# sloisel/MultiGridBarrier.jl

Measured on AMD Instinct MI355X. Metric: Newton iters/sec + wall-clock to converge, 2D P2 p-Laplace L=9, higher is better.
Workload: dtype f64

## Files before the change

include/mgbhip.h:

```cpp
#ifndef MGBHIP_H
#define MGBHIP_H

#include <stdint.h>

#ifdef __cplusplus
extern "C" {
#endif

#define MGBHIP_OK 0
#define MGBHIP_ERR_INVALID 1
#define MGBHIP_ERR_HIP 2
#define MGBHIP_ERR_NOT_SPD 3
#define MGBHIP_ERR_NONFINITE 4
#define MGBHIP_ERR_CONVERGENCE 5

#define MGBHIP_MAX_PIECES 4
#define MGBHIP_MAX_IDX 10
#define MGBHIP_MAX_LIN 4
#define MGBHIP_MAX_ND 13
#define MGBHIP_MAX_NU 4
#define MGBHIP_MAX_OPS 8

#define MGBHIP_KIND_EP 1
#define MGBHIP_KIND_LINEAR 2
// ... 74 lines not shown
    int64_t newton_iterations;
    int64_t f0_evals, f1_evals, f2_evals, factorizations;
    int32_t cap_steps;
    int64_t* its;
    double* ts;
    double* kappas;
    double* times;
    double* c_dot_Dz;
} mgbhip_core_result;

int mgbhip_create(mgbhip_ctx** ctx, int device_id, void* hip_stream );
int mgbhip_destroy(mgbhip_ctx* ctx);
const char* mgbhip_last_error(void);
const char* mgbhip_version(void);

int mgbhip_problem_create(mgbhip_ctx* ctx, const mgbhip_problem_desc* desc,
                          mgbhip_problem* share, mgbhip_problem** out);
int mgbhip_problem_destroy(mgbhip_problem* prob);
int mgbhip_problem_set_box(mgbhip_problem* prob, double b, double R);
int mgbhip_problem_set_barrier_weights(mgbhip_problem* prob, const double* bw );
int64_t mgbhip_level_size(const mgbhip_problem* prob, int32_t level);

int mgbhip_f0(mgbhip_problem* prob, int32_t level, const double* s, const double* c,
              const double* z0, double* value);
int mgbhip_f1(mgbhip_problem* prob, int32_t level, const double* s, const double* c,
              const double* z0, double* grad );
int mgbhip_f2(mgbhip_problem* prob, int32_t level, const double* s, const double* c,
              const double* z0, double* values );
int mgbhip_hessian_pattern(mgbhip_problem* prob, int32_t level, int64_t* nnz,
                           const int32_t** rowptr, const int32_t** colidx);
int mgbhip_solve(mgbhip_problem* prob, int32_t level, const double* g, double* x);
int mgbhip_set_hessian(mgbhip_problem* prob, int32_t level, const double* values );
int mgbhip_solve_newton(mgbhip_problem* prob, int32_t level, const double* g, double* x, double* lambda2);
typedef int (*mgbhip_allreduce_fn)(void* user, double* buf, int64_t count, int32_t op, int32_t on_device);
int mgbhip_problem_set_sharding(mgbhip_problem* prob, int32_t level, int64_t n_iface,
                                const int32_t* iface_cols, const double* own_mask );
int mgbhip_problem_set_collective(mgbhip_problem* prob, mgbhip_allreduce_fn allreduce, void* user,
                                  int32_t accepts_device_ptr);
int mgbhip_newton_direction(mgbhip_problem* prob, int32_t level, const double* s, const double* c,
                            const double* z0, double* x, double* lambda2, int32_t* condensed);
int mgbhip_node_barrier(mgbhip_problem* prob, const double* z, double* F , double* Dz );
int mgbhip_node_slack(mgbhip_problem* prob, const double* z, double* slack );

int mgbhip_mgb_core(mgbhip_problem* prob, double* z , const double* c ,
                    const mgbhip_options* opt, mgbhip_core_result* res);
int mgbhip_matched_t(mgbhip_problem* prob, const double* z, const double* c, double t_default,
                     double* t_out);
void mgbhip_default_options(mgbhip_options* opt, int64_t n_nodes);

typedef struct mgbhip_vec mgbhip_vec;
int mgbhip_vec_alloc(mgbhip_ctx* ctx, int64_t len, mgbhip_vec** out);
int mgbhip_vec_free(mgbhip_vec* v);
int64_t mgbhip_vec_len(const mgbhip_vec* v);
int mgbhip_vec_upload(mgbhip_vec* v, const double* host, int64_t len);
int mgbhip_vec_download(const mgbhip_vec* v, double* host, int64_t len);
int mgbhip_vec_fill(mgbhip_vec* v, double value);
int mgbhip_vec_copy(mgbhip_vec* dst, const mgbhip_vec* src);
int mgbhip_vec_axpy(double alpha, const mgbhip_vec* x, mgbhip_vec* y);
int mgbhip_vec_scale(double alpha, mgbhip_vec* x);
int mgbhip_vec_dot(const mgbhip_vec* a, const mgbhip_vec* b, double* out);
int mgbhip_vec_norm(const mgbhip_vec* a, double* out);
int mgbhip_vec_isfinite(const mgbhip_vec* a, int32_t* all_finite);
int mgbhip_f0_d(mgbhip_problem* prob, int32_t level, const mgbhip_vec* s, const mgbhip_vec* c,
                const mgbhip_vec* z0, double* value);
int mgbhip_f1_d(mgbhip_problem* prob, int32_t level, const mgbhip_vec* s, const mgbhip_vec* c,
                const mgbhip_vec* z0, mgbhip_vec* grad);
int mgbhip_f2_d(mgbhip_problem* prob, int32_t level, const mgbhip_vec* s, const mgbhip_vec* c,
                const mgbhip_vec* z0);
int mgbhip_solve_d(mgbhip_problem* prob, int32_t level, const mgbhip_vec* g, mgbhip_vec* x);
int mgbhip_prolong_add(mgbhip_problem* prob, int32_t level, const mgbhip_vec* s, mgbhip_vec* z);

int mgbhip_stage_ms(mgbhip_problem* prob, const char* stage, double* total_ms, int64_t* launches);
int mgbhip_reset_stage_timers(mgbhip_problem* prob, int enable);
int mgbhip_solver_stats(mgbhip_problem* prob, int32_t level, double* out8);
int mgbhip_solver_chain(mgbhip_problem* prob, int32_t level, double* out8);
enum { MGBHIP_PROJ_NONE = 0, MGBHIP_PROJ_LOOP = 1, MGBHIP_PROJ_STAGED = 2, MGBHIP_PROJ_MFMA = 3, MGBHIP_PROJ_ACCUMULATE = 4 };
int mgbhip_level_plan(mgbhip_problem* prob, int32_t level, int32_t* out16);
enum { MGBHIP_ELEM_F0 = 0, MGBHIP_ELEM_F1 = 1, MGBHIP_ELEM_F2 = 2, MGBHIP_ELEM_NODE_F = 3, MGBHIP_ELEM_NODE_SLACK = 4, MGBHIP_ELEM_F01 = 5 };
enum { MGBHIP_ELEM_KIND_DENSE = 0, MGBHIP_ELEM_KIND_WIDE = 1, MGBHIP_ELEM_KIND_FAST_DEFAULT = 2, MGBHIP_ELEM_KIND_FAST_RUNTIME = 3,
       MGBHIP_ELEM_KIND_CONDENSE = 4, MGBHIP_ELEM_KIND_GENERIC = 5 };
int mgbhip_elem_plan(mgbhip_problem* prob, int32_t mode, int32_t* out16);
int mgbhip_trial_values(mgbhip_problem* prob, int32_t level, const double* x, const double* dir, double step, const double* c,
                        const double* z0, double* y, double* g, double* xn, int32_t* moved, int32_t* finite, int32_t* path);
enum { MGBHIP_LAUNCH_ROW = 16 };
enum { MGBHIP_ASM_NONE = 0, MGBHIP_ASM_GATHER = 1, MGBHIP_ASM_COLUMNS = 2 };
enum { MGBHIP_B0_NA = 0, MGBHIP_B0_GATHER = 1, MGBHIP_B0_DIAG0 = 2, MGBHIP_B0_STEP0 = 3 };
enum { MGBHIP_BWD_NA = 0, MGBHIP_BWD_K8 = 1, MGBHIP_BWD_K16 = 2, MGBHIP_BWD_GENERAL = 3 };
int64_t mgbhip_solver_launches(mgbhip_problem* prob, int32_t level, int32_t* out, int64_t cap);

#define MGBHIP_INTERP_FEM1D 1
#define MGBHIP_INTERP_QK 2
#define MGBHIP_INTERP_P1 3
#define MGBHIP_INTERP_P2 4
#define MGBHIP_INTERP_SPECTRAL1D 5
#define MGBHIP_INTERP_SPECTRAL2D 6
#define MGBHIP_INTERP_P2C 7
int mgbhip_interpolate(mgbhip_ctx* ctx, int32_t family, int32_t d, int32_t k, int32_t p, int64_t N,
                       const double* x, const double* table, int32_t ncomp, const double* z, int64_t M,
                       const double* pts, double* out, int32_t* elem);
int mgbhip_interpolate_grad(mgbhip_ctx* ctx, int32_t family, int32_t d, int32_t k, int32_t p, int64_t N,
                            const double* x, const double* table, int32_t ncomp, const double* z, int64_t M,
                            const double* pts, double* out ,
                            double* grad , int32_t* elem );

typedef struct mgbhip_locator mgbhip_locator;
int mgbhip_locator_create(mgbhip_ctx* ctx, int32_t family, int32_t d, int32_t k, int32_t p, int64_t N,
                          const double* x, const double* table, int64_t M, const double* pts,
                          mgbhip_locator** out);
int mgbhip_locator_elements(const mgbhip_locator* loc, int32_t* elem );
int mgbhip_locator_evaluate(mgbhip_locator* loc, int32_t ncomp, const double* z ,
                            double* out ,
                            double* grad );
int mgbhip_locator_destroy(mgbhip_locator* loc);

typedef struct mgbhip_closest mgbhip_closest;
int mgbhip_closest_create(mgbhip_ctx* ctx, int32_t d, int32_t e, int32_t k, int64_t N, const double* x,
                          const double* nodes, int64_t M, const double* pts, double max_distance,
                          mgbhip_closest** out);
int mgbhip_closest_fetch(const mgbhip_closest* cp, int32_t* elem , double* xi ,
                         double* foot , double* dist , int32_t* flag );
int mgbhip_closest_evaluate(mgbhip_closest* cp, int32_t ncomp, const double* z ,
                            double* out ,
                            double* grad );
int mgbhip_closest_destroy(mgbhip_closest* cp);

enum { MGBHIP_QUAD_VALUE = 0, MGBHIP_QUAD_LP = 1, MGBHIP_QUAD_W1P = 2, MGBHIP_QUAD_ENERGY = 3 };
typedef struct mgbhip_quadrature mgbhip_quadrature;
int mgbhip_quadrature_create(mgbhip_ctx* ctx, int32_t d, int32_t e, int32_t p, int64_t N, const double* x, int32_t Q,
                             const double* wref, const double* phi, const double* dphi, mgbhip_quadrature** out);
int mgbhip_quadrature_points(mgbhip_quadrature* quad, double* points );
int mgbhip_quadrature_weights(mgbhip_quadrature* quad, double* weights );
int mgbhip_quadrature_integrate(mgbhip_quadrature* quad, int32_t kind, double pexp, int32_t ncol,
                                const double* z , const double* minus ,
                                const double* source ,
                                double* per_element , double* totals );
int mgbhip_quadrature_max(mgbhip_quadrature* quad, int32_t kind, int32_t ncol, const double* z ,
                          const double* minus , double* maxima );
int mgbhip_quadrature_plan(int32_t d, int32_t e, int32_t p, int32_t Q, int64_t N, int32_t* out16);
int mgbhip_quadrature_times(const mgbhip_quadrature* quad, double* ms2);
int mgbhip_quadrature_destroy(mgbhip_quadrature* quad);

typedef struct mgbhip_residual mgbhip_residual;
int mgbhip_residual_create(mgbhip_ctx* ctx, int32_t d, int32_t p, int64_t N, const double* x, int32_t Q, const double* wref,
                           const double* phi, const double* dphi, const double* d2phi, mgbhip_residual** out);
int mgbhip_residual_geometry(mgbhip_residual* res, double* points , double* weights ,
                             double* sizes );
int mgbhip_residual_pointwise(mgbhip_residual* res, double pexp, int32_t ncol, const double* z ,
                              const double* source , int32_t at_points, double* r );
int mgbhip_residual_integrate(mgbhip_residual* res, double pexp, int32_t ncol, const double* z ,
                              const double* source , int32_t at_points,
                              double* per_element , double* totals );
int mgbhip_residual_plan(int32_t d, int32_t p, int32_t Q, int64_t N, int32_t* out16);
int mgbhip_residual_times(const mgbhip_residual* res, double* ms2);
int mgbhip_residual_destroy(mgbhip_residual* res);

enum { MGBHIP_FACE_VALUE = 0, MGBHIP_FACE_FLUX = 1 };
typedef struct mgbhip_faces mgbhip_faces;
int mgbhip_faces_create(mgbhip_ctx* ctx, int32_t d, int32_t p, int64_t N, const double* x, const int32_t* t, int32_t F,
                        int32_t Qf, const double* wf, const double* phi, const double* dphi, const double* tangents,
                        const double* normals, const int32_t* corners, int32_t ncode, const int32_t* perm,
                        mgbhip_faces** out, int64_t* nboundary, int64_t* ninterior);
int mgbhip_faces_topology(const mgbhip_faces* faces, int32_t* boundary, int32_t* interior, int32_t* orientation,
                          int32_t* element_faces);
int mgbhip_faces_geometry(mgbhip_faces* faces, int32_t which, double* points, double* normals, double* measures);
int mgbhip_faces_sizes(const mgbhip_faces* faces, double* sizes );
int mgbhip_faces_integrate(mgbhip_faces* faces, int32_t kind, double pexp, int32_t ncol, const double* z ,
// ... 128 lines not shown
```

multigridbarrier.jl_amd/csrc/api.cpp:

```cpp
#include <chrono>
#include <cmath>
#include <cstring>
#include <algorithm>
#include <limits>
#include <memory>
#include <string>

#include "closest.hpp"
#include "contour.hpp"
#include "faces.hpp"
#include "figure.hpp"
#include "interpolate.hpp"
#include "polyline.hpp"
#include "problem.hpp"
#include "quadrature.hpp"
#include "residual.hpp"
#include "raycast.hpp"
#include "stream.hpp"
#include "surface.hpp"
#include "tubes.hpp"
#include "weld.hpp"

using namespace mgbhip;

mgbhip_problem* problem_create(mgbhip_ctx* ctx, const mgbhip_problem_desc* d, mgbhip_problem* share);
int core_run(mgbhip_problem* P, double* z, const double* c, const mgbhip_options* opt, mgbhip_core_result* res);
int matched_t_run(mgbhip_problem* P, const double* z, const double* c, double t_default, double* t_out);
void trial_values_run(mgbhip_problem* P, int level, double step, double* y, int32_t* moved, int32_t* finite, int32_t* path);

#ifdef MGB_STEP_PROBE
namespace mgbhip { void mf_debug_probe(long long* out64); }
#endif

static thread_local std::string g_last_error;

struct DeviceGuard {
    int prev = -1, dev = -1;
    explicit DeviceGuard(int d) : dev(d) {
        if (dev < 0) return;
        if (hipGetDevice(&prev) != hipSuccess) prev = -1;
        if (prev != dev) MGB_HIP_CHECK(hipSetDevice(dev));
    }
    ~DeviceGuard() {
        if (dev >= 0 && prev >= 0 && prev != dev) (void)hipSetDevice(prev);
    }
};
static int dev_of(const mgbhip_ctx* c) { return c ? c->device : -1; }
template <class H>
static int dev_of(const H* h) { return (h && h->ctx) ? h->ctx->device : -1; }

template <class T>
struct Handle {
    mgbhip_ctx* ctx = nullptr;
    T obj;
};
struct mgbhip_locator : Handle<Locator> {};
struct mgbhip_closest : Handle<Closest> {};
struct mgbhip_quadrature : Handle<Quadrature> {};
struct mgbhip_faces : Handle<Faces> {};
struct mgbhip_residual : Handle<Residual> {};
struct mgbhip_contour : Handle<Contour> {};
struct mgbhip_tessellation : Handle<Tessellation> {};
struct mgbhip_weld : Handle<Weld> {};
struct mgbhip_polyline : Handle<Polyline> {};
struct mgbhip_raycast : Handle<RayCaster> {};
struct mgbhip_surface : Handle<Surface> {};
struct mgbhip_tubes : Handle<Tubes> {};
struct mgbhip_stream : Handle<StreamTracer> {};
struct mgbhip_figure : Handle<Figure> {};

#define MGB_API_BEGIN try {
#define MGB_API_BEGIN_ON(h) try { DeviceGuard _guard(dev_of(h));
#define MGB_API_END                                   \
    }                                                 \
    catch (const InvalidArgument& e) {                \
        g_last_error = e.what();                      \
        return MGBHIP_ERR_INVALID;                    \
    }                                                 \
    catch (const HipError& e) {                       \
        g_last_error = e.what();                      \
        return MGBHIP_ERR_HIP;                        \
    }                                                 \
    catch (const std::exception& e) {                 \
        g_last_error = e.what();                      \
        return MGBHIP_ERR_INVALID;                    \
    }

template <class H, class Build>
static void create_handle(mgbhip_ctx* ctx, H** out, Build build) {
    std::unique_ptr<H> h(new H());
    h->ctx = ctx;
    build(h->obj);
    *out = h.release();
}

template <class H>
static int destroy_handle(H* h) {
    MGB_API_BEGIN_ON(h)
    if (!h) return MGBHIP_OK;
    (void)hipStreamSynchronize(h->ctx->stream);
    delete h;
    return MGBHIP_OK;
    MGB_API_END
}

static void check_window(const std::string& who, double t_min, double t_max) {
    MGB_REQUIRE(std::isfinite(t_min) && t_max > t_min, who + ": t_min must be finite and t_max > t_min");
}

static void check_rays(const std::string& who, int64_t R, int dim, const double* origin, const double* dir) {
    for (int64_t i = 0; i < R * dim; ++i)
// ... 273 lines not shown
        for (size_t i = 0; i < m; ++i) acc += g[i] * x[i];
        *lambda2 = acc;
    }
    if (status != MGBHIP_OK) g_last_error = "Cholesky met a non-positive pivot";
    return status;
    MGB_API_END
}

int mgbhip_problem_set_sharding(mgbhip_problem* P, int32_t level, int64_t n_iface, const int32_t* iface_cols, const double* own_mask) {
    MGB_API_BEGIN_ON(P)
    check_level(P, level);
    mgbhip::Level& L = P->levels[level];
    MGB_REQUIRE(!L.solver.analyzed, "sharding must be set before the first solve of the level");
    MGB_REQUIRE(own_mask != nullptr && n_iface >= 0 && n_iface <= L.m && (n_iface == 0 || iface_cols), "bad sharding arguments");
    L.h_iface.assign(iface_cols, iface_cols + n_iface);
    for (int64_t i = 0; i < n_iface; ++i) {
        MGB_REQUIRE(L.h_iface[i] >= 0 && L.h_iface[i] < L.m, "interface column out of range");
        MGB_REQUIRE(i == 0 || L.h_iface[i] > L.h_iface[i - 1], "interface columns must be strictly increasing");
    }
    L.d_iface.upload(L.h_iface, P->stream());
    L.own.upload(own_mask, (size_t)L.m, P->stream());
    MGB_HIP_CHECK(hipStreamSynchronize(P->stream()));
    L.sharded = true;
    return MGBHIP_OK;
    MGB_API_END
}

int mgbhip_problem_set_collective(mgbhip_problem* P, mgbhip_allreduce_fn fn, void* user, int32_t accepts_device_ptr) {
    MGB_API_BEGIN_ON(P)
    P->coll_fn = fn;
    P->coll_user = user;
    P->coll_device = accepts_device_ptr != 0;
    return MGBHIP_OK;
    MGB_API_END
}

int mgbhip_newton_direction(mgbhip_problem* P, int32_t level, const double* s, const double* c, const double* z0, double* x,
                            double* lambda2, int32_t* condensed) {
    MGB_API_BEGIN_ON(P)
    check_level(P, level);
    MGB_REQUIRE(s && c && z0 && x, "null argument");
    hipStream_t st = P->stream();
    const size_t m = (size_t)P->levels[level].m;
    stage_inputs(P, level, s, c, z0);
    P->eval_f1(level, P->d_x.p, P->d_z0.p, P->d_c.p, P->d_g.p);
    P->eval_f2(level, P->d_x.p, P->d_z0.p, P->d_c.p, false, P->d_g.p);
    if (condensed) *condensed = P->levels[level].H.condensed() ? 1 : 0;
    P->factor(level, P->d_g.p, P->d_nv.p);
    P->trisolve_carried(level, P->d_nv.p);
    const int status = P->levels[level].solver.status(st);
    P->d_nv.download(x, m, st);
    if (lambda2) {
        std::vector<double> g(m);
        P->d_g.download(g.data(), m, st);
        MGB_HIP_CHECK(hipStreamSynchronize(st));
        double acc = 0.0;
        for (size_t i = 0; i < m; ++i) acc += g[i] * x[i];
        *lambda2 = acc;
    }
    MGB_HIP_CHECK(hipStreamSynchronize(st));
    if (status != MGBHIP_OK) g_last_error = "Cholesky met a non-positive pivot";
    return status;
    MGB_API_END
}

int mgbhip_trial_values(mgbhip_problem* P, int32_t level, const double* x, const double* dir, double step, const double* c,
                        const double* z0, double* y, double* g, double* xn, int32_t* moved, int32_t* finite, int32_t* path) {
    MGB_API_BEGIN_ON(P)
    check_level(P, level);
    MGB_REQUIRE(x && dir && c && z0 && y && g && xn && moved && finite && path, "null argument");
    MGB_REQUIRE(!P->sharded(), "trial_values: not for sharded problems");
    hipStream_t st = P->stream();
    const size_t m = (size_t)P->levels[level].m;
    stage_inputs(P, level, x, c, z0);
    P->d_nv.upload(dir, m, st);
    trial_values_run(P, level, step, y, moved, finite, path);
    P->d_gn.download(g, m, st);
    P->d_xn.download(xn, m, st);
    MGB_HIP_CHECK(hipStreamSynchronize(st));
    return MGBHIP_OK;
    MGB_API_END
}


static double* vec_scratch(mgbhip_ctx* c, int64_t len) {
    c->vscratch.ensure((size_t)reduce_scratch_doubles(len));
    c->vscal.ensure(8);
    return c->vscratch.p;
}
static void same_ctx(const mgbhip_vec* a, const mgbhip_vec* b) {
    MGB_REQUIRE(a && b, "null vector");
    MGB_REQUIRE(a->ctx == b->ctx, "vectors belong to different contexts");
}

int mgbhip_vec_alloc(mgbhip_ctx* ctx, int64_t len, mgbhip_vec** out) {
    MGB_API_BEGIN_ON(ctx)
    MGB_REQUIRE(ctx && out && len >= 0, "bad argument");
    std::unique_ptr<mgbhip_vec> v(new mgbhip_vec());
    v->ctx = ctx;
    v->len = len;
    v->buf.alloc((size_t)std::max<int64_t>(len, 1));
    v->buf.zero(ctx->stream);
    *out = v.release();
    return MGBHIP_OK;
    MGB_API_END
}

int mgbhip_vec_free(mgbhip_vec* v) {
    MGB_API_BEGIN_ON(v)
    if (!v) return MGBHIP_OK;
    (void)hipStreamSynchronize(v->ctx->stream);
    delete v;
    return MGBHIP_OK;
    MGB_API_END
}

int64_t mgbhip_vec_len(const mgbhip_vec* v) { return v ? v->len : -1; }

int mgbhip_vec_upload(mgbhip_vec* v, const double* host, int64_t len) {
    MGB_API_BEGIN_ON(v)
    MGB_REQUIRE(v && host && len == v->len, "upload: length mismatch");
    v->buf.upload(host, (size_t)len, v->ctx->stream);
    MGB_HIP_CHECK(hipStreamSynchronize(v->ctx->stream));
    return MGBHIP_OK;
    MGB_API_END
}

int mgbhip_vec_download(const mgbhip_vec* v, double* host, int64_t len) {
    MGB_API_BEGIN_ON(v)
    MGB_REQUIRE(v && host && len == v->len, "download: length mismatch");
    v->buf.download(host, (size_t)len, v->ctx->stream);
    MGB_HIP_CHECK(hipStreamSynchronize(v->ctx->stream));
    return MGBHIP_OK;
    MGB_API_END
}

int mgbhip_vec_fill(mgbhip_vec* v, double value) {
    MGB_API_BEGIN_ON(v)
    MGB_REQUIRE(v, "null vector");
    launch_fill(value, v->buf.p, v->len, v->ctx->stream);
    return MGBHIP_OK;
    MGB_API_END
}

int mgbhip_vec_copy(mgbhip_vec* dst, const mgbhip_vec* src) {
    MGB_API_BEGIN_ON(dst)
    same_ctx(dst, src);
    MGB_REQUIRE(dst->len == src->len, "copy: length mismatch");
    if (dst->len) MGB_HIP_CHECK(hipMemcpyAsync(dst->buf.p, src->buf.p, (size_t)dst->len * sizeof(double),
                                               hipMemcpyDeviceToDevice, dst->ctx->stream));
    return MGBHIP_OK;
    MGB_API_END
}

int mgbhip_vec_axpy(double alpha, const mgbhip_vec* x, mgbhip_vec* y) {
    MGB_API_BEGIN_ON(y)
    same_ctx(x, y);
    MGB_REQUIRE(x->len == y->len, "axpy: length mismatch");
    if (y->len) launch_axpy(alpha, x->buf.p, y->buf.p, y->len, y->ctx->stream);
    return MGBHIP_OK;
    MGB_API_END
}

int mgbhip_vec_scale(double alpha, mgbhip_vec* x) {
    MGB_API_BEGIN_ON(x)
    MGB_REQUIRE(x, "null vector");
// ... 1273 lines not shown
```

multigridbarrier.jl_amd/csrc/common.hpp:

```cpp
#pragma once
#include <hip/hip_runtime.h>

#include <cstdint>
#include <cstdio>
#include <map>
#include <stdexcept>
#include <string>
#include <vector>

#include "host_util.hpp"
#include "readback.hpp"

namespace mgbhip {

struct HipError : std::runtime_error {
    using std::runtime_error::runtime_error;
};

#define MGB_HIP_CHECK(expr)                                                                  \
    do {                                                                                     \
        hipError_t _e = (expr);                                                              \
        if (_e != hipSuccess) {                                                              \
            char _buf[512];                                                                  \
            snprintf(_buf, sizeof(_buf), "%s failed: %s (%s:%d)", #expr, hipGetErrorString(_e), \
                     __FILE__, __LINE__);                                                    \
            throw ::mgbhip::HipError(_buf);                                                  \
        }                                                                                    \
    } while (0)

template <typename T>
struct DevBuf {
    T* p = nullptr;
    size_t n = 0;
    DevBuf() = default;
    DevBuf(const DevBuf&) = delete;
    DevBuf& operator=(const DevBuf&) = delete;
    DevBuf(DevBuf&& o) noexcept : p(o.p), n(o.n) { o.p = nullptr; o.n = 0; }
    DevBuf& operator=(DevBuf&& o) noexcept {
        if (this != &o) { release(); p = o.p; n = o.n; o.p = nullptr; o.n = 0; }
        return *this;
    }
    ~DevBuf() { release(); }
    void release() {
        if (p) (void)hipFree(p);
        p = nullptr;
        n = 0;
    }
    void alloc(size_t count) {
        if (count == n && p) return;
        release();
        if (count) MGB_HIP_CHECK(hipMalloc((void**)&p, count * sizeof(T)));
        n = count;
    }
    void ensure(size_t count) {
        if (count > n) alloc(count);
    }
    void upload(const T* h, size_t count, hipStream_t st) {
        ensure(count);
        if (count) MGB_HIP_CHECK(hipMemcpyAsync(p, h, count * sizeof(T), hipMemcpyHostToDevice, st));
    }
    void upload(const std::vector<T>& h, hipStream_t st) { upload(h.data(), h.size(), st); }
    void download(T* h, size_t count, hipStream_t st) const {
        if (count) MGB_HIP_CHECK(hipMemcpyAsync(h, p, count * sizeof(T), hipMemcpyDeviceToHost, st));
    }
    void zero(hipStream_t st, size_t count = (size_t)-1) {
        if (count == (size_t)-1) count = n;
        if (count) MGB_HIP_CHECK(hipMemsetAsync(p, 0, count * sizeof(T), st));
    }
};

struct PinnedBuf {
    double* d = nullptr;
    double* dev = nullptr;
    PinnedBuf() {
        void* p = nullptr;
        if (hipHostMalloc(&p, RB_SLOTS * sizeof(double), hipHostMallocDefault) != hipSuccess)
            throw HipError("hipHostMalloc failed for the scalar read-back block");
        d = static_cast<double*>(p);
        void* dp = nullptr;
        if (hipHostGetDevicePointer(&dp, p, 0) != hipSuccess || dp == nullptr)
            throw HipError("hipHostGetDevicePointer failed for the scalar read-back block");
        dev = static_cast<double*>(dp);
    }
    ~PinnedBuf() { if (d) (void)hipHostFree(d); }
    PinnedBuf(const PinnedBuf&) = delete;
    PinnedBuf& operator=(const PinnedBuf&) = delete;
};

struct StageTimers {
    struct Rec { double ms = 0; int64_t launches = 0; };
    bool enabled = false;
    hipStream_t stream = nullptr;
    std::map<std::string, Rec> recs;
    struct Pending { std::string name; hipEvent_t a, b; };
    std::vector<Pending> pending;
    std::vector<hipEvent_t> pool;

    hipEvent_t get() {
        if (!pool.empty()) { hipEvent_t e = pool.back(); pool.pop_back(); return e; }
        hipEvent_t e;
        MGB_HIP_CHECK(hipEventCreate(&e));
        return e;
    }
    std::vector<size_t> open;
    void begin(const char* name) {
        if (!enabled) return;
        Pending p{name, get(), get()};
        MGB_HIP_CHECK(hipEventRecord(p.a, stream));
        pending.push_back(p);
        open.push_back(pending.size() - 1);
    }
    void end() {
        if (!enabled || open.empty()) return;
        MGB_HIP_CHECK(hipEventRecord(pending[open.back()].b, stream));
        open.pop_back();
        if (open.empty() && pending.size() > 4096) collect();
    }
    void collect() {
        if (!open.empty()) return;
        for (auto& p : pending) {
            MGB_HIP_CHECK(hipEventSynchronize(p.b));
            float ms = 0;
            MGB_HIP_CHECK(hipEventElapsedTime(&ms, p.a, p.b));
            auto& r = recs[p.name];
            r.ms += ms;
            r.launches += 1;
            pool.push_back(p.a);
            pool.push_back(p.b);
        }
        pending.clear();
    }
    void reset(bool en) {
        collect();
        recs.clear();
        enabled = en;
    }
    ~StageTimers() {
        for (auto& p : pending) { (void)hipEventDestroy(p.a); (void)hipEventDestroy(p.b); }
        for (auto e : pool) (void)hipEventDestroy(e);
    }
};

template <int N>
struct CallEvents {
    hipEvent_t ev[N] = {};
    bool timed = false;
    CallEvents() = default;
    CallEvents(const CallEvents&) = delete;
    CallEvents& operator=(const CallEvents&) = delete;
    ~CallEvents() {
        for (hipEvent_t e : ev)
            if (e) (void)hipEventDestroy(e);
    }
    void mark(int i, hipStream_t st) {
        if (!ev[i]) MGB_HIP_CHECK(hipEventCreate(&ev[i]));
        MGB_HIP_CHECK(hipEventRecord(ev[i], st));
    }
    void begin(hipStream_t st) {
        timed = false;
        mark(0, st);
    }
// ... 17 lines not shown
```

multigridbarrier.jl_amd/csrc/driver.cpp:

```cpp
#include <chrono>
#include <cstdio>
#include <cstdlib>
#include <cmath>
#include <cstring>
#include <functional>
#include <limits>

#include "problem.hpp"

using namespace mgbhip;

namespace {

constexpr double EPS = std::numeric_limits<double>::epsilon();

bool debug_on() {
    static const bool on = env_on("MGBHIP_DEBUG");
    return on;
}
#define DBG(...) do { if (debug_on()) { fprintf(stderr, __VA_ARGS__); } } while (0)

struct Stop {
    double lambda_tol;
    double theta;
    int (*fn)(double, double, double, double, double, double, void*) = nullptr;
    void* user = nullptr;
    bool operator()(double ymin, double ynext, double gmin, double gnorm_next, double ndecmin, double ndec) const {
        if (fn) return fn(ymin, ynext, gmin, gnorm_next, ndecmin, ndec, user) != 0;
        const bool exact = (ynext >= ymin) && (gnorm_next >= theta * gmin);
        if (lambda_tol >= 0) return (ndec < lambda_tol) || exact;
        return exact;
    }
};

struct NewtonResult {
    int k = 0;
    bool converged = false;
    double y = 0;
};

struct VecStats { double sumsq, bad; };

VecStats vec_stats(mgbhip_problem* P, int level, const double* d_v, int64_t len) {
    launch_vec_stats(d_v, len, P->d_scratch.p, P->d_scal.p, RB_SUMSQ, P->stream(), P->own_mask(level));
    const double* r = P->read_scalars(RB_SUMSQ, 2);
    return VecStats{r[0], r[1]};
}

double dev_dot(mgbhip_problem* P, int level, const double* a, const double* b, int64_t len) {
    launch_dot(a, b, len, P->d_scratch.p, P->d_scal.p, RB_GDOTV, P->stream(), P->own_mask(level));
    return *P->read_scalars(RB_GDOTV, 1);
}

struct NewtonCtx {
    mgbhip_problem* P;
    int level;
    const double* d_zJ;
    const double* d_c;
    int64_t m;
    double F0(const double* d_s) { return P->eval_f0(level, d_s, d_zJ, d_c); }
    void F1(const double* d_s, double* d_out, double* d_part) { P->eval_f1(level, d_s, d_zJ, d_c, d_out, P->sharded() ? d_part : nullptr); }
    const double* rhs_of_g() const { return P->sharded() ? P->d_gpart.p : P->d_g.p; }
    void F2(const double* d_s) { P->eval_f2(level, d_s, d_zJ, d_c, false, rhs_of_g()); }
};

bool trial_values(NewtonCtx& C, double& ynext, double& gnorm_next, int32_t* moved = nullptr, const double* step = nullptr,
                  bool* restrict_fused_out = nullptr) {
    mgbhip_problem* P = C.P;
    hipStream_t st = P->stream();
    const bool onfly = step && P->can_fuse_step(C.level);
    if (step) {
        ++P->step_stamp;
        if (!onfly) launch_step(P->d_x.p, P->d_nv.p, *step, P->d_xn.p, C.m, P->d_flag.p, P->step_stamp, st);
        P->touch();
    }
    const bool fused = !P->dense;
    static const bool fuse_restrict = !env_on("MGBHIP_NO_FUSED_RESTRICT");
    TrialRestrict fuse;
    TrialPoint point{};
    if (onfly) {
        point = TrialPoint{P->d_x.p, P->d_nv.p, *step};
        fuse = TrialRestrict{P->d_x.p, P->d_nv.p, *step, P->d_xn.p, P->d_flag.p, P->step_stamp};
    }
    const bool restrict_fused = P->eval_f01_launch(C.level, P->d_xn.p, C.d_zJ, C.d_c, P->d_gn.p, P->sharded() ? P->d_gnpart.p : nullptr, fused,
                                                   onfly ? &point : nullptr, (fused && fuse_restrict) ? &fuse : nullptr);
    if (restrict_fused_out) *restrict_fused_out = restrict_fused;
    if (onfly && !restrict_fused) launch_step(P->d_x.p, P->d_nv.p, *step, P->d_xn.p, C.m, P->d_flag.p, P->step_stamp, st);
    const TrialReadback r = P->finish_trial(C.level, P->d_gn.p, fused, restrict_fused);
    if (moved) *moved = r.moved ? 1 : 0;
    ynext = r.value;
    if (!std::isfinite(ynext)) return false;
    if (r.bad != 0.0 || !std::isfinite(r.sumsq)) return false;
    gnorm_next = std::sqrt(r.sumsq);
    return true;
}

bool linesearch_backtracking(NewtonCtx& C, const mgbhip_options& opt, double y, double inc, double& ynext,
                             double& gnorm_next) {
    double s = 1.0;
    bool have = false;
    while (s > 0.0) {
        double yn, gn;
        int32_t moved = 0;
        if (trial_values(C, yn, gn, &moved, &s)) {
            have = true;
            ynext = yn;
            gnorm_next = gn;
            const bool stalled = (moved == 0);
            if (stalled || yn <= y - opt.ls_c1 * inc * s) return true;
        }
        s *= opt.ls_beta;
    }
    return have;
}

bool linesearch_illinois(NewtonCtx& C, const mgbhip_options& opt, double inc, double& ynext, double& gnorm_next) {
    mgbhip_problem* P = C.P;
    hipStream_t st = P->stream();
    struct Reject {};
    auto phi = [&](double sigma) -> double {
        launch_step(P->d_x.p, P->d_nv.p, sigma, P->d_xn.p, C.m, P->d_flag.p, ++P->step_stamp, st);
        P->touch();
        const double f = C.F0(P->d_xn.p);
        if (!std::isfinite(f)) throw Reject();
        C.F1(P->d_xn.p, P->d_gn.p, P->d_gnpart.p);
        const double v = dev_dot(P, C.level, P->d_gn.p, P->d_nv.p, C.m);
        if (!std::isfinite(v)) throw Reject();
        return v;
    };
    double s = 1.0;
    while (s > 0.0) {
        try {
            double a = 0.0, b = s, fa = inc, fb = phi(s), root = b;
            bool done = false;
            if (fa == 0) { root = a; done = true; }
            else if (fa * fb >= 0) { root = b; done = true; }
            for (int it = 0; it < 10000 && !done; ++it) {
                const double c = (a * fb - b * fa) / (fb - fa);
                const double fc = phi(c);
                if (c <= std::fmin(a, b) || c >= std::fmax(a, b) || fc * fa == 0 || fc * fb == 0) { root = c; done = true; break; }
                if (fb * fc < 0) { a = b; fa = fb; } else { fa /= 2; }
                b = c; fb = fc;
            }
            if (!done) throw Reject();
            launch_step(P->d_x.p, P->d_nv.p, root, P->d_xn.p, C.m, P->d_flag.p, ++P->step_stamp, st);
        P->touch();
            double yn, gn;
            if (!trial_values(C, yn, gn)) throw Reject();
            ynext = yn;
            gnorm_next = gn;
            return true;
        } catch (Reject&) {
        }
        s *= opt.ls_beta;
    }
    return false;
}

NewtonResult newton(NewtonCtx& C, const mgbhip_options& opt, const Stop& stop, int maxit) {
    mgbhip_problem* P = C.P;
    hipStream_t st = P->stream();
    NewtonResult R;
    P->d_x.zero(st, (size_t)C.m);
    P->touch();
    static const bool split_start = env_on("MGBHIP_SPLIT_START");
    double y;
    VecStats gs;
    if (!split_start && !P->dense && !P->sharded() && opt.line_search != 1) {
        P->eval_f01_launch(C.level, P->d_x.p, C.d_zJ, C.d_c, P->d_g.p, nullptr, true);
        const TrialReadback r = P->finish_trial(C.level, P->d_g.p, true, false);
        y = r.value;
        if (!std::isfinite(y)) throw InvalidArgument("newton: initial objective value is not finite");
        gs = VecStats{r.sumsq, r.bad};
    } else {
        y = C.F0(P->d_x.p);
        if (!std::isfinite(y)) throw InvalidArgument("newton: initial objective value is not finite");
        if (P->sharded()) { P->d_gpart.ensure((size_t)C.m); P->d_gnpart.ensure((size_t)C.m); }
        C.F1(P->d_x.p, P->d_g.p, P->d_gpart.p);
        gs = vec_stats(P, C.level, P->d_g.p, C.m);
    }
    double ymin = y;
// ... 76 lines not shown

struct StepResult {
    bool converged;
    std::vector<int64_t> its;
};

StepResult mgb_step(mgbhip_problem* P, const double* d_c, const mgbhip_options& opt, bool finalize_now,
                    bool initial_step) {
    const int L = (int)P->levels.size();
    StepResult out;
    out.its.assign(L, 0);
    hipStream_t st = P->stream();
    const Stop sc{opt.stop_lambda_tol, opt.stop_theta, opt.stopping_criterion, opt.user};
    const Stop fin{-1.0, opt.finalize_theta};
    const size_t zn = (size_t)P->nu * P->n;
    auto eta = [&](int j, int J, const Stop& stop, int maxit) -> bool {
        (void)j;
        const int lev = J - 1;
        static const bool snapshot = env_on("MGBHIP_Z_SNAPSHOT");
        if (snapshot) MGB_HIP_CHECK(hipMemcpyAsync(P->d_z0.p, P->d_z.p, zn * sizeof(double), hipMemcpyDeviceToDevice, st));
        NewtonCtx C{P, lev, snapshot ? P->d_z0.p : P->d_z.p, d_c, P->levels[lev].m};
        NewtonResult r = newton(C, opt, stop, maxit);
        out.its[lev] += r.k;
        if (r.converged) {
            const Level& Lv = P->levels[lev];
            StageScope scp(P->ctx->timers, "prolong");
            launch_csr_matvec(Lv.rows, Lv.Rptr.p, Lv.Rcol.p, Lv.Rval.p, P->d_x.p, P->d_z.p, true, false, st);
        }
        return r.converged;
    };
    std::function<bool(int, int)> dac = [&](int j, int J) -> bool {
        const int mn = (initial_step && J - j == 1) ? opt.maxit : opt.max_newton;
        if (eta(j, J, sc, mn)) return true;
        const int jmid = (j + J) / 2;
        if (jmid == j || jmid == J) return false;
        return dac(j, jmid) && dac(jmid, J);
    };
    bool converged = dac(0, L);
    if (finalize_now) {
        const bool foo = eta(L - 1, L, fin, opt.maxit);
        converged = converged && foo;
    }
    out.converged = converged;
    return out;
}

double c_dot_Dz(mgbhip_problem* P, const double* d_c) {
    hipStream_t st = P->stream();
    ElemParams E = P->elem_params(d_c);
    E.z0 = P->d_z.p;
    E.invn = 0.0;
    E.bw = nullptr;
    launch_elem(E, MODE_F0, st);
    launch_reduce_partials(P->d_partials.p, elem_grid(P->p, P->N), P->d_scal.p, st);
    double v;
    P->d_scal.download(&v, 1, st);
    MGB_HIP_CHECK(hipStreamSynchronize(st));
    if (P->sharded()) P->allreduce_host(&v, 1, 0);
    return v;
}

bool slack_feasible(mgbhip_problem* P, std::vector<double>& hbuf) {
    hipStream_t st = P->stream();
    hbuf.resize((size_t)P->n);
    MGB_HIP_CHECK(hipMemcpyAsync(hbuf.data(), P->d_z.p + (size_t)(P->nu - 1) * P->n, (size_t)P->n * sizeof(double),
                                 hipMemcpyDeviceToHost, st));
    MGB_HIP_CHECK(hipStreamSynchronize(st));
    double mx = -INFINITY;
    for (double v : hbuf) mx = std::fmax(mx, v);
    if (P->sharded()) P->allreduce_host(&mx, 1, 1);
    return mx < 0;
}

}

void trial_values_run(mgbhip_problem* P, int level, double step, double* y, int32_t* moved, int32_t* finite, int32_t* path) {
    NewtonCtx C{P, level, P->d_z0.p, P->d_c.p, P->levels[level].m};
    double yn = 0.0, gn = 0.0;
    const bool onfly = P->can_fuse_step(level);
    bool restrict_fused = false;
    *finite = trial_values(C, yn, gn, moved, &step, &restrict_fused) ? 1 : 0;
    *y = yn;
    *path = (onfly ? 1 : 0) | (restrict_fused ? 2 : 0);
}

int core_run(mgbhip_problem* P, double* z, const double* c, const mgbhip_options* optp, mgbhip_core_result* res) {
    const mgbhip_options opt = *optp;
    hipStream_t st = P->stream();
    const size_t zn = (size_t)P->nu * P->n;
    const size_t cn = (size_t)P->n * P->nD;
    const int L = (int)P->levels.size();
    P->prepare_all();
    P->d_z.upload(z, zn, st);
    P->d_c0.upload(c, cn, st);
    P->cnt = Counters();
    auto tb = std::chrono::steady_clock::now();
    auto now = [&] { return std::chrono::duration<double>(std::chrono::steady_clock::now() - tb).count(); };
    double t = opt.t;
    const double target = 1.0 / opt.tol;
    double kappa = opt.kappa;
    const double kappa0 = kappa;
    int k = 1;
    std::vector<double> hbuf;
    double t_first = INFINITY;
    std::vector<double> zhost;
    auto early = [&](double tt) -> bool {
        if (opt.early_stop_fn) {
            zhost.resize(zn);
            P->d_z.download(zhost.data(), zn, st);
            MGB_HIP_CHECK(hipStreamSynchronize(st));
            if (opt.early_stop_fn(zhost.data(), tt, opt.user) != 0) return true;
        }
        if (opt.early_stop != 1) return false;
        if (!slack_feasible(P, hbuf)) return false;
        t_first = std::fmin(t_first, tt);
        return tt >= 2 * t_first;
    };
    auto record = [&](int kk, const std::vector<int64_t>& its, bool add) {
        if (kk - 1 < res->cap_steps && res->its) {
            for (int l = 0; l < L; ++l) {
                if (add) res->its[(size_t)(kk - 1) * L + l] += its[l];
                else res->its[(size_t)(kk - 1) * L + l] = its[l];
            }
        }
    };
    auto setc = [&](double tt) { launch_scale_copy(P->d_c0.p, tt, P->d_c.p, (int64_t)cn, st); };
    res->failure_code = 0;
    res->L = L;
    if (res->times && res->cap_steps > 0) res->times[0] = now();
    setc(t);
    StepResult S = mgb_step(P, P->d_c.p, opt, opt.finalize && t >= target, true);
    if (!S.converged) {
        res->failure_code = 1;
        res->k = 1;
        res->t_final = t;
        res->t_elapsed = now();
        return MGBHIP_ERR_CONVERGENCE;
    }
    record(1, S.its, false);
    auto diag = [&](int kk) {
        if (kk - 1 < res->cap_steps) {
            if (res->ts) res->ts[kk - 1] = t;
            if (res->kappas) res->kappas[kk - 1] = kappa;
            if (res->c_dot_Dz) res->c_dot_Dz[kk - 1] = c_dot_Dz(P, P->d_c0.p);
        }
    };
    diag(1);
    bool stopped_early = false;
    while (t < target && kappa > 1 && k < opt.maxit) {
        if (early(t)) { stopped_early = true; break; }
        ++k;
        if (k - 1 < res->cap_steps && res->its)
            for (int l = 0; l < L; ++l) res->its[(size_t)(k - 1) * L + l] = 0;
        if (res->times && k - 1 < res->cap_steps) res->times[k - 1] = now();
        while (kappa > 1) {
            const double t1 = kappa * t;
            setc(t1);
            P->d_tmp.ensure(zn);
            MGB_HIP_CHECK(hipMemcpyAsync(P->d_tmp.p, P->d_z.p, zn * sizeof(double), hipMemcpyDeviceToDevice, st));
            S = mgb_step(P, P->d_c.p, opt, opt.finalize && t1 >= target, false);
            record(k, S.its, true);
            if (S.converged) {
                int64_t mx = 0;
                for (int64_t v : S.its) mx = std::max(mx, v);
                if ((double)mx <= opt.max_newton * 0.5) kappa = std::fmin(kappa0, kappa * kappa);
                t = t1;
// ... 74 lines not shown
```

multigridbarrier.jl_amd/csrc/elem_kernels.hpp:

```cpp
#pragma once
#include <mutex>
#include <utility>

#include "dense.hpp"
#include "elem_device.hpp"

namespace mgbhip {

namespace {

template <int NY, int MODE>
__global__ __launch_bounds__(256) void elem_kernel(const ElemParams P, const int lgG) {
    extern __shared__ double sh[];
    const int tid = threadIdx.x;
    const int G = 1 << lgG;
    const int EPB = 256 >> lgG;
    const int el = tid >> lgG;
    const int r = tid & (G - 1);
    const int p = P.p;
    const int pp = p * p;
    const int nu = P.nu;
    const int64_t e = (int64_t)blockIdx.x * EPB + el;
    const bool active = (e < P.N) && (r < p);
    const int64_t n = P.n;
    const int64_t node = e * p + r;

    double* zl = sh;
    double* opL = zl + elem_lds_z(256, nu);
    double* YL = opL + elem_lds_ops(P.nstage, EPB, pp);

    {
        const int64_t e0 = (int64_t)blockIdx.x * EPB;
        int64_t lim = (P.N - e0) * pp;
        if (lim > (int64_t)EPB * pp) lim = (int64_t)EPB * pp;
        for (int o = 0; o < P.nstage; ++o) {
            const double* src = P.stage_ptr[o] + e0 * pp;
            double* dst = opL + (size_t)o * EPB * pp;
            for (int i = tid; i < lim; i += 256) dst[i] = src[i];
        }
    }
    if (active) stage_z(P, zl, el, nu, G, r, n, node);
    __syncthreads();

    auto OP = [&](int k, int rr, int cc) -> double {
        const int so = P.D_stage[k];
        if (so >= 0) return opL[((size_t)so * EPB + el) * pp + cc * p + rr];
        return P.ops[P.D_op[k]][e * pp + cc * p + rr];
    };

    double y[NY];
#pragma unroll
    for (int k = 0; k < NY; ++k) {
        double v = 0.0;
        if (active) {
            const int a = P.D_state[k];
            if (P.D_stage[k] == -1) {
                v = zl[(el * nu + a) * G + r];
            } else {
                for (int cc = 0; cc < p; ++cc) v += OP(k, r, cc) * zl[(el * nu + a) * G + cc];
            }
        }
        y[k] = v;
    }

    double F = 0.0;
    double g[NY];
    double H[NY * NY];
    (void)g;
    (void)H;

    if (MODE == MODE_F0 || MODE == MODE_NODE_F) {
        if (active) cone_eval<NY, 0>(P.cone, node, n, y, F, g, H);
        if (MODE == MODE_NODE_F) {
            if (active) {
                P.out_F[node] = F;
                if (P.out_Dz != nullptr) {
#pragma unroll
                    for (int k = 0; k < NY; ++k) P.out_Dz[node + n * k] = y[k];
                }
            }
            return;
        }
        double val = 0.0;
        if (active) {
            const double bar = barrier_f0(P, node, F);
            double lin = 0.0;
#pragma unroll
            for (int k = 0; k < NY; ++k) lin += P.c[node + n * k] * y[k];
            val = bar + P.w[node] * lin;
        }
        __syncthreads();
        const double tot = block_sum_256(val, sh);
        if (tid == 0) P.out_partial[blockIdx.x] = tot;
        return;
    }
// ... 52 lines not shown
            for (int k = 0; k < NY; ++k) {
                double sc = P.bw ? ((bwv == 0.0) ? 0.0 : bwv * g[k]) : P.invn * g[k];
                YL[(el * NY + k) * G + r] = sc + wv * P.c[node + n * k];
            }
        }
        __syncthreads();
        if (active) {
            const int i = r;
            for (int a = 0; a < nu; ++a) {
                double acc = 0.0;
#pragma unroll
                for (int k = 0; k < NY; ++k) {
                    if (P.D_state[k] != a) continue;
                    const double* Yk = YL + (el * NY + k) * G;
                    if (P.D_stage[k] == -1) {
                        acc += Yk[i];
                    } else {
                        for (int rr = 0; rr < p; ++rr) acc += OP(k, rr, i) * Yk[rr];
                    }
                }
                P.out_ret[(int64_t)a * n + node] = acc;
            }
        }
        return;
    }
    if (MODE == MODE_F2) {
        constexpr int NT = NY * (NY + 1) / 2;
        if (active) {
            cone_eval<NY, 2>(P.cone, node, n, y, F, g, H);
            const double bwv = P.bw ? P.bw[node] : 0.0;
#pragma unroll
            for (int k = 0; k < NY; ++k)
#pragma unroll
                for (int k2 = k; k2 < NY; ++k2) {
                    const double h = H[k * NY + k2];
                    const double sc = P.bw ? ((bwv == 0.0) ? 0.0 : bwv * h) : P.invn * h;
                    YL[((size_t)el * NT + tri_index(k, k2, NY)) * G + r] = sc;
                }
        }
        __syncthreads();
        if (active) {
            const int j = r;
            const int NB = nu * (nu + 1) / 2;
            for (int a = 0; a < nu; ++a)
                for (int b = a; b < nu; ++b) {
                    const int blk = a * nu - (a * (a - 1)) / 2 + (b - a);
                    const bool dblk = (P.diag_mask >> blk) & 1;
                    double* out = P.out_hel + P.blk_off[blk] + (dblk ? (e * p + j) - j : (e * p + j) * (int64_t)p);
                    for (int i = dblk ? j : 0; i < (dblk ? j + 1 : p); ++i) {
                        double val = 0.0;
#pragma unroll
                        for (int k = 0; k < NY; ++k) {
                            if (P.D_state[k] != a) continue;
                            const bool idk = P.D_stage[k] == -1;
#pragma unroll
                            for (int k2 = 0; k2 < NY; ++k2) {
                                if (P.D_state[k2] != b) continue;
                                const bool idk2 = P.D_stage[k2] == -1;
                                const int t = (k <= k2) ? tri_index(k, k2, NY) : tri_index(k2, k, NY);
                                const double* Yt = YL + ((size_t)el * NT + t) * G;
                                if (idk && idk2) {
                                    val += (i == j) ? Yt[i] : 0.0;
                                } else if (idk) {
                                    val += Yt[i] * OP(k2, i, j);
                                } else if (idk2) {
                                    val += OP(k, j, i) * Yt[j];
                                } else {
                                    double acc = 0.0;
                                    for (int rr = 0; rr < p; ++rr) acc += OP(k, rr, i) * Yt[rr] * OP(k2, rr, j);
                                    val += acc;
                                }
                            }
                        }
                        out[i] = val;
                    }
                }
        }
        return;
    }
}

template <int MODE>
__global__ __launch_bounds__(256) void elem_wide_kernel(const ElemParams P, const int lgG) {
    extern __shared__ double sh[];
    const int tid = threadIdx.x;
    const int NT_ = blockDim.x;
    const int G = 1 << lgG;
    const int EPB = NT_ >> lgG;
    const int el = tid >> lgG;
    const int r = tid & (G - 1);
    const int p = P.p;
    const int pp = p * p;
    const int nu = P.nu;
    const int nD = P.nD;
    const int64_t e = (int64_t)blockIdx.x * EPB + el;
    const bool active = (e < P.N) && (r < p);
    const int64_t n = P.n;
    const int64_t node = e * p + r;

    double* zl = sh;
    double* opL = zl + elem_lds_z((size_t)NT_, nu);
    double* YL = opL + elem_lds_ops(P.nstage, EPB, pp);
    {
        const int64_t e0 = (int64_t)blockIdx.x * EPB;
        int64_t lim = (P.N - e0) * pp;
        if (lim > (int64_t)EPB * pp) lim = (int64_t)EPB * pp;
        for (int o = 0; o < P.nstage; ++o) {
            const double* src = P.stage_ptr[o] + e0 * pp;
            double* dst = opL + (size_t)o * EPB * pp;
            for (int i = tid; i < lim; i += NT_) dst[i] = src[i];
        }
    }
    if (active) stage_z(P, zl, el, nu, G, r, n, node);
    __syncthreads();

    auto OP = [&](int k, int rr, int cc) -> double {
        const int so = P.D_stage[k];
        if (so >= 0) return opL[((size_t)so * EPB + el) * pp + cc * p + rr];
        return P.ops[P.D_op[k]][e * pp + cc * p + rr];
    };

    double y[WIDE_NY];
#pragma unroll
    for (int k = 0; k < WIDE_NY; ++k) {
        double v = 0.0;
        if (active && k < nD) {
            const int a = P.D_state[k];
            if (P.D_stage[k] == -1) {
                v = zl[(el * nu + a) * G + r];
            } else {
                for (int cc = 0; cc < p; ++cc) v += OP(k, r, cc) * zl[(el * nu + a) * G + cc];
            }
        }
        y[k] = v;
    }
    double F = 0.0;
    double g[WIDE_NY];

    if (MODE == MODE_F0 || MODE == MODE_NODE_F) {
        if (active) cone_eval_wide<0>(P.cone, node, n, nD, y, F, g, nullptr, 0);
        if (MODE == MODE_NODE_F) {
            if (active) {
                P.out_F[node] = F;
                if (P.out_Dz != nullptr)
                    for (int k = 0; k < nD; ++k) P.out_Dz[node + n * k] = y[k];
            }
            return;
        }
        double val = 0.0;
        if (active) {
            const double bar = barrier_f0(P, node, F);
            double lin = 0.0;
#pragma unroll
            for (int k = 0; k < WIDE_NY; ++k) lin += (k < nD) ? P.c[node + n * k] * y[k] : 0.0;
            val = bar + P.w[node] * lin;
        }
        __syncthreads();
        const double tot = block_sum_256(val, sh);
        if (tid == 0) P.out_partial[blockIdx.x] = tot;
        return;
    }
    if (MODE == MODE_NODE_SLACK) {
        if (active) P.out_F[node] = cone_slack<WIDE_NY, WIDE_W>(P.cone, node, n, y);
        return;
    }
    if (MODE == MODE_F1 || MODE == MODE_F01) {
// ... 308 lines not shown
            }
#pragma unroll
            for (int q = 0; q < P; ++q) bj -= Xbeta[q] * t[q];
            if (j == PB) {
                bj -= Pm.leaf_g[ld.interior];
#pragma unroll
                for (int q = 0; q < P; ++q) corner -= Xbeta[q] * Xbeta[q] * Xinv[q];
#pragma unroll
                for (int i = 0; i < P; ++i) Xc[i] = up[i];
                Xs[0] = bj;
                Xs[1] = up[PB];
            }
        }
        __builtin_amdgcn_fence(__ATOMIC_RELEASE, "wavefront");
        __builtin_amdgcn_wave_barrier();
        __builtin_amdgcn_fence(__ATOMIC_ACQUIRE, "wavefront");
        {
            const int m = (int)(ld.packed & 15u);
            const bool pk = Pm.leaf_packed != 0;
            int pos[P];
#pragma unroll
            for (int i = 0; i < P; ++i) pos[i] = (int)((ld.packed >> (4 + 4 * i)) & 15u);
            double d7 = 1.0, bb = 0.0, inv7 = 1.0, f = 0.0, xc[P];
#pragma unroll
            for (int i = 0; i < P; ++i) xc[i] = 0.0;
            if (active) {
                d7 = Xs[1];
                bb = Xs[0];
                inv7 = 1.0 / d7;
#pragma unroll
                for (int i = 0; i < P; ++i) xc[i] = Xc[i];
                f = (j < PB) ? xc[j] * inv7 : 0.0;
                bad = bad || (j == PB && ((d7 == 0.0) || !isfinite(d7)));
            }
            double* Fg = Pm.leaf_arena + ld.F_off;
            double* S = Fg;
            if (pk) {
                __syncthreads();
                S = sh + (size_t)el * 120;
            }
            auto at = [&](int rr, int cc) -> int { return pk ? cc * m - (cc * (cc - 1)) / 2 + (rr - cc) : rr + cc * m; };
            if (active) {
                S[at(j, j)] = ssj;
#pragma unroll
                for (int rr = 0; rr < P; ++rr)
                    if (rr > j) S[at(rr, j)] = 0.0;
                S[at(P, j)] = usc[PB] * inv;
#pragma unroll
                for (int i = 0; i < PB; ++i)
                    if (pos[i] != 15) S[at(pos[i], j)] = usc[i] * inv;
                S[at(m - 1, j)] = beta * inv;
                if (j == PB) {
                    S[at(P, P)] = d7;
#pragma unroll
                    for (int i = 0; i < PB; ++i)
                        if (pos[i] != 15) S[at(pos[i], P)] = xc[i] * inv7;
                    S[at(m - 1, P)] = bb * inv7;
                    S[at(m - 1, m - 1)] = corner - bb * bb * inv7;
                } else if (pos[j] != 15) {
#pragma unroll
                    for (int i = 0; i < PB; ++i)
                        if (pos[i] != 15 && pos[i] >= pos[j]) S[at(pos[i], pos[j])] = up[i] - xc[i] * f;
                    S[at(m - 1, pos[j])] = bj - bb * f;
                }
            }
            if (pk) {
                __builtin_amdgcn_fence(__ATOMIC_RELEASE, "wavefront");
                __builtin_amdgcn_wave_barrier();
                __builtin_amdgcn_fence(__ATOMIC_ACQUIRE, "wavefront");
                if (e < Pm.N) {
                    const LeafDesc l2 = Pm.leaf_desc[e];
                    const int mm = (int)(l2.packed & 15u);
                    double* dstF = Pm.leaf_arena + l2.F_off;
                    for (int t = r; t < mm * (mm + 1) / 2; t += G) dstF[t] = S[t];
                }
            }
        }
        if (bad) atomicOr(Pm.leaf_status, 1);
    }
}

template <int NY, int P, class Sig>
__global__ __launch_bounds__(256) void elem_f01_fast(const ElemParams Pm) {
    constexpr int G = elem_group(P);
    constexpr int EPB = 256 / G;
    constexpr int PP = P * P;
    extern __shared__ double sh[];
    const int tid = threadIdx.x;
    const int el = tid / G;
    const int r = tid % G;
    const int nu = Sig::rt ? Pm.nu : 2;
    auto DST = [&](int k) -> int { return Sig::rt ? Pm.D_state[k] : Sig::state(k); };
    auto DSG = [&](int k) -> int { return Sig::rt ? Pm.D_stage[k] : Sig::stage(k); };
    const int64_t e0 = (int64_t)blockIdx.x * EPB;
    const int64_t e = e0 + el;
    const bool active = (e < Pm.N) && (r < P);
    const int64_t n = Pm.n;
    const int64_t node = e * P + r;

    double* zl = sh;
    double* opL = zl + elem_lds_z(256, nu);
    double* YL = opL + elem_lds_ops(Pm.nstage, EPB, PP);
    {
        int64_t lim = (Pm.N - e0) * PP;
        if (lim > (int64_t)EPB * PP) lim = (int64_t)EPB * PP;
        constexpr int NIT = (EPB * PP + 255) / 256;
        for (int o = 0; o < Pm.nstage; ++o) {
            const double* src = Pm.stage_ptr[o] + e0 * PP;
            double* dst = opL + (size_t)o * EPB * PP;
            copy_unrolled<NIT>(src, dst, lim, tid);
        }
    }
    double ck[NY];
    double wv = 0.0, bwv = 0.0;
    if (active) {
        for (int a = 0; a < nu; ++a) zl[(el * nu + a) * G + r] = z_at(Pm, (int64_t)a * n + node);
#pragma unroll
        for (int k = 0; k < NY; ++k) ck[k] = Pm.c[node + n * k];
        wv = Pm.w[node];
        bwv = Pm.bw ? Pm.bw[node] : 0.0;
    }
    __syncthreads();
    const double* opE = opL + (size_t)el * PP;
    auto OP = [&](int k, int rr, int cc) -> double { return opE[(size_t)DSG(k) * EPB * PP + cc * P + rr]; };
    double y[NY];
#pragma unroll
    for (int k = 0; k < NY; ++k) {
        double v = 0.0;
        if (active) {
            const double* za = zl + (el * nu + DST(k)) * G;
            if (DSG(k) < 0) v = za[r];
            else {
#pragma unroll
                for (int cc = 0; cc < P; ++cc) v += OP(k, r, cc) * za[cc];
            }
        }
        y[k] = v;
    }
    double val = 0.0;
    if (active) {
        double F0v, F, g[NY], H[NY * NY];
        cone_eval<NY, 0>(Pm.cone, node, n, y, F0v, g, H);
        cone_eval<NY, 1>(Pm.cone, node, n, y, F, g, H);
        const double bar = Pm.bw ? ((bwv == 0.0) ? 0.0 : bwv * F0v) : Pm.invn * F0v;
        double lin = 0.0;
#pragma unroll
        for (int k = 0; k < NY; ++k) {
            lin += ck[k] * y[k];
            const double sc = Pm.bw ? ((bwv == 0.0) ? 0.0 : bwv * g[k]) : Pm.invn * g[k];
            YL[(el * NY + k) * G + r] = sc + wv * ck[k];
        }
        val = bar + wv * lin;
    }
    __syncthreads();
    if (active) {
        const int i = r;
        for (int a = 0; a < nu; ++a) {
            double acc = 0.0;
#pragma unroll
            for (int k = 0; k < NY; ++k) {
                if (DST(k) != a) continue;
                const double* Yk = YL + (el * NY + k) * G;
                if (DSG(k) < 0) {
                    acc += Yk[i];
                } else {
#pragma unroll
// ... 124 lines not shown
```

multigridbarrier.jl_amd/csrc/kernels.hpp:

```cpp
#pragma once
#include "common.hpp"
#include "cone.hpp"
#include "elem_layout.hpp"
#include "panel_layout.hpp"

namespace mgbhip {

struct LeafDesc {
    int64_t F_off;
    int32_t interior;
    uint32_t packed;
};

struct ElemParams {
    int32_t p, nu, nD, nstage;
    int32_t ymask;
    int64_t N, n;
    const double* ops[MGBHIP_MAX_OPS];
    const double* stage_ptr[MGBHIP_MAX_OPS];
    int32_t D_state[MGBHIP_MAX_ND];
    int32_t D_op[MGBHIP_MAX_ND];
    int32_t D_stage[MGBHIP_MAX_ND];
    const double* w;
    const double* c;
    const double* z0;
    const double* bw;
    double invn;
    ConeDev cone;
    double* out_partial;
    double* out_ret;
    double* out_hel;
    double* out_F;
    double* out_Dz;
    int32_t diag_mask;
    int64_t blk_off[MGBHIP_MAX_NU * (MGBHIP_MAX_NU + 1) / 2];
    double* dn_Dz;
    double* dn_Y;
    const LeafDesc* leaf_desc;
    double* leaf_arena;
    const double* leaf_g;
    int64_t leaf_slack0;
    int32_t* leaf_status;
    int32_t leaf_packed;
    const int32_t* zsel;
    const double* zs;
    double* zout;
    const double* zx;
    double zalpha;
    int32_t wide;
};
static_assert(sizeof(ElemParams) <= 4096 - 64, "ElemParams must stay well inside the kernel argument limit");

bool launch_elem_f2_condense(const ElemParams& P, hipStream_t st);

int64_t elem_grid(int p, int64_t N);
inline size_t elem_lds_bytes(const ElemParams& P, int mode) {
    return elem_lds_bytes(elem_threads(P.wide != 0, mode), P.p, P.nu, P.nD, P.nstage, mode);
}
inline bool elem_default_signature(const ElemParams& P) {
    const int NY = P.nD;
    if (P.nu != 2 || P.ymask != (((1 << NY) - 1) & ~1)) return false;
    for (int k = 0; k < NY; ++k) {
        if (P.D_state[k] != (k == NY - 1 ? 1 : 0)) return false;
        if (P.D_stage[k] != ((k == 0 || k == NY - 1) ? -1 : k - 1)) return false;
    }
    return true;
}
inline int elem_unstaged_rows(const ElemParams& P) {
    int cnt = 0;
    for (int k = 0; k < P.nD; ++k) cnt += P.D_stage[k] == -2;
    return cnt;
}
inline ElemPlan elem_plan_of(const ElemParams& P, int mode, bool condensing) {
    return elem_decide(P.p, P.nu, P.nD, P.nstage, P.wide != 0, P.p > 64, elem_unstaged_rows(P) == 0, elem_default_signature(P), mode,
                       condensing, P.N);
}
void launch_elem(const ElemParams& P, int mode, hipStream_t st);

void launch_reduce_partials(const double* partials, int64_t count, double* out, hipStream_t st);
void launch_vec_stats(const double* v, int64_t n, double* scratch, double* block, int32_t slot, hipStream_t st,
                      const double* mask = nullptr);
void launch_dot(const double* a, const double* b, int64_t n, double* scratch, double* block, int32_t slot, hipStream_t st,
                const double* mask = nullptr);
void launch_restrict_trial(int64_t rows, const int32_t* ptr, const int32_t* col, const double* val, const double* ret, double* g,
                            double* scratch, const double* x, const double* nn, double s, double* xn, int32_t* moved, int32_t stamp,
                            hipStream_t st);
void launch_publish(const double* src, int n, double* host_block, int host_lo, double seq, hipStream_t st);
void launch_dir_finish(const double* v, const double* g, int64_t n, double* scratch, double* scal, int32_t* status2, double* host,
                       hipStream_t st, const double* mask = nullptr, double seq = 0.0);
void launch_trial_finish(const double* g, int64_t n, double* scratch, const double* f0_partials, int64_t f0_count, double* scal,
                         int32_t* moved, double* host, hipStream_t st, const double* mask = nullptr, double seq = 0.0,
                         bool partials_ready = false);
void launch_index_gather(const double* v, const int32_t* idx, int64_t cnt, double* out, hipStream_t st);
void launch_index_scatter(const double* in, const int32_t* idx, int64_t cnt, double* v, hipStream_t st);
int64_t reduce_scratch_doubles(int64_t n);

void launch_csr_matvec(int64_t rows, const int32_t* ptr, const int32_t* col, const double* val,
                       const double* x, double* y, bool add, bool long_rows, hipStream_t st);
int csr_chunks(int64_t max_row_len);
void launch_csr_matvec_chunked(int64_t rows, const int32_t* ptr, const int32_t* col, const double* val,
                               const double* x, double* y, double* scratch, int nchunk, hipStream_t st);
void launch_prolong(int64_t rows, const int32_t* ptr, const int32_t* col, const double* val, const double* s,
                    const double* z0, double* zfull, hipStream_t st);
void launch_step(const double* x, const double* n, double s, double* xn, int64_t len, int32_t* moved, int32_t stamp,
                 hipStream_t st);
void launch_scale_copy(const double* src, double alpha, double* dst, int64_t len, hipStream_t st);
void launch_border_tail(const double* g, double* tail, int64_t m, hipStream_t st, double* x_one = nullptr);
void launch_axpy(double alpha, const double* x, double* y, int64_t len, hipStream_t st);
void launch_fill(double value, double* y, int64_t len, hipStream_t st);

void launch_gather_shared(int64_t nshared, const int32_t* sh_q, const int32_t* cptr, const int32_t* cidx, const double* slab,
                          double* out, hipStream_t st);
void launch_gather_assemble(int64_t nnz, const int32_t* cptr, const int32_t* cidx, const double* slab,
                            double* Hval, bool long_lists, hipStream_t st, int32_t chunk = 0, int32_t nchunk = 0,
                            double* part = nullptr, const int32_t* qmap = nullptr, int64_t nq = 0);

struct PanelParams {
    int32_t p, nu;
    int64_t N;
    const int32_t* ecol_ptr;
    const double* panels;
    const int32_t* eoff;
    const double* hel;
    double* slab;
    int32_t cmax;
    int32_t upper_only;
    const int32_t* spos;
};
bool launch_panel_project_mfma(const PanelParams& P, hipStream_t st);
void launch_invert_lists(const int32_t* cidx, int64_t total, int32_t* spos, hipStream_t st);
void launch_panel_project(const PanelParams& P, hipStream_t st);
void launch_panel_accumulate(const PanelParams& P, const int32_t* ecols, int32_t m, int32_t nstream, int32_t nsplit,
                             int32_t chunk, int32_t ctmax, double* partial, double* H, hipStream_t st);
void launch_panel_project_staged(const PanelParams& P, int32_t ctmax, hipStream_t st);

}
```

multigridbarrier.jl_amd/csrc/problem.cpp:

```cpp
#include "problem.hpp"
#include "assembly_plan.hpp"
#include "plan_device.hpp"
#include "dense.hpp"

#include <algorithm>
#include <cmath>
#include <cstdio>
#include <atomic>
#include <exception>
#include <cstdlib>
#include <string>
#include <thread>
#include <cstring>
#include <numeric>

using namespace mgbhip;



static void upload_csr(const mgbhip_csr& R, Level& L, hipStream_t st) {
    MGB_REQUIRE(R.rows >= 0 && R.cols >= 0 && R.rowptr && (R.rowptr[R.rows] == 0 || (R.colidx && R.values)),
                "bad prolongation CSR");
    MGB_REQUIRE(R.rows < INT32_MAX && R.cols < INT32_MAX, "prolongation too large for 32-bit indices");
    L.rows = R.rows;
// ... 365 lines not shown
        if (L.acc) dense_pattern(m, L.hHptr, L.hHcol);
        else host_pattern(S, C, L.hHptr, L.hHcol);
        L.nnz = (int64_t)L.hHcol.size();
        L.Hptr.upload(L.hHptr, st);
        L.Hcol.upload(L.hHcol, st);
        if (!L.acc) {
            const HostLists lists = host_lists(S, C, L.hHptr, L.hHcol);
            L.long_lists = lists.long_lists;
            L.list_total = lists.total;
            L.cptr.upload(lists.cptr, st);
            L.cidx.upload(lists.cidx.data(), lists.cidx.size(), st);
            if (lists.cidx.empty()) L.cidx.alloc(1);
            MGB_HIP_CHECK(hipStreamSynchronize(st));
        }
    }
    L.Hval.alloc((size_t)(L.nnz + L.m + 1));
    if (!L.acc && L.long_lists && L.nnz > 0) {
        std::vector<int32_t> hc((size_t)L.nnz + 1);
        L.cptr.download(hc.data(), hc.size(), st);
        MGB_HIP_CHECK(hipStreamSynchronize(st));
        const GatherChunks G = decide_gather_chunks(hc.data(), L.nnz);
        if (G.gather_nchunk > 0) {
            L.gather_chunk = G.gather_chunk;
            L.gather_nchunk = G.gather_nchunk;
            L.gather_part.alloc(2 * (size_t)L.nnz * (size_t)L.gather_nchunk);
        }
    }
    if (!selection && !L.acc && L.nnz > 0) {
        static const bool row_major = env_on("MGBHIP_UPPER_ROW_MAJOR");
        const std::vector<int32_t> up = upper_positions(L.hHptr, L.hHcol, m, row_major);
        L.nup = (int64_t)up.size();
        L.upq.upload(up, st);
        MGB_HIP_CHECK(hipStreamSynchronize(st));
    }
    if (!selection) {
        const std::vector<double> panels = element_panels(S, C);
        L.panels.upload(panels.data(), panels.size(), st);
        if (panels.empty()) L.panels.alloc(1);
        L.slab.alloc((size_t)std::max<int64_t>(L.slab_doubles, 1));
        static const bool no_sorted = env_on("MGBHIP_NO_SORTED_SLAB");
        if (!L.acc && L.nnz > 0 && L.slab_doubles > 0 && !no_sorted) {
            if (L.list_total == L.slab_doubles) {
                L.spos.alloc((size_t)L.slab_doubles);
                launch_invert_lists(L.cidx.p, L.slab_doubles, L.spos.p, st);
                L.sorted_slab = true;
            }
        }
        if (L.acc) L.acc_copies.alloc((size_t)L.acc_waves * (size_t)A.tri);
        MGB_HIP_CHECK(hipStreamSynchronize(st));
    }
    MGB_HIP_CHECK(hipStreamSynchronize(st));
    L.planned = true;
}


ElemParams mgbhip_problem::elem_params(const double* d_cc) const {
    ElemParams E;
    std::memset(&E, 0, sizeof(E));
    E.p = p; E.nu = nu; E.nD = nD; E.nstage = nstage; E.N = N; E.n = n;
    E.wide = wide ? 1 : 0;
    E.ymask = 0;
    for (int k = 0; k < cone.npieces; ++k)
        for (int c = 0; c < cone.pc[k].ni; ++c) E.ymask |= 1 << cone.pc[k].idx[c];
    if (cone.feasibility)
        for (int k = cone.NC - 1; k < nD; ++k) E.ymask |= 1 << k;
    for (size_t o = 0; o < store->ops.size() && o < MGBHIP_MAX_OPS; ++o) E.ops[o] = store->ops[o].p;
    for (int o = 0; o < nstage; ++o) E.stage_ptr[o] = stage_ptr[o];
    for (int k = 0; k < MGBHIP_MAX_ND; ++k) { E.D_state[k] = D_state[k]; E.D_op[k] = D_op[k]; E.D_stage[k] = D_stage[k]; }
    E.w = store->w.p;
    E.c = d_cc;
    E.bw = has_bw ? bw.p : nullptr;
    E.invn = 1.0 / (double)n;
    E.cone = cone;
    E.out_partial = d_partials.p;
    E.out_ret = d_ret.p;
    E.out_hel = d_hel.p;
    E.out_F = d_nodeF.p;
    E.out_Dz = nullptr;
    E.dn_Dz = d_dnDz.p;
    E.dn_Y = d_dnY.p;
    return E;
}

bool mgbhip_problem::bind_point(ElemParams& E, int level, const double* d_s, const double* d_zz, const TrialPoint* trial) {
    const Level& L = levels[level];
    const PointKey here{zstamp, level, d_s, d_zz};
    MGB_REQUIRE(!trial || (L.R_unit && !dense && !(zf == here)), "a trial point is given only after touch(), on a selection level");
    E.z0 = d_zz;
    if (d_s == nullptr) return false;
    if (zf == here) {
    } else if (L.R_unit && !dense) {
        E.zsel = L.Rsel.p;
        E.zs = d_s;
        if (trial) { E.zs = trial->x; E.zx = trial->dir; E.zalpha = trial->alpha; }
        E.zout = d_zfull.p;
        return true;
    } else if (L.R_long) {
        MGB_HIP_CHECK(hipMemcpyAsync(d_zfull.p, d_zz, sizeof(double) * (size_t)L.rows, hipMemcpyDeviceToDevice, stream()));
        launch_csr_matvec(L.rows, L.Rptr.p, L.Rcol.p, L.Rval.p, d_s, d_zfull.p, true, true, stream());
    } else {
        launch_prolong(L.rows, L.Rptr.p, L.Rcol.p, L.Rval.p, d_s, d_zz, d_zfull.p, stream());
    }
    zf = here;
    E.z0 = d_zfull.p;
    return false;
}

void mgbhip_problem::launch_elem_at(ElemParams& E, int mode, int level, const double* d_s, const double* d_zz, const TrialPoint* trial) {
    const bool writes_zfull = bind_point(E, level, d_s, d_zz, trial);
    launch_elem(E, mode, stream());
    if (writes_zfull) zf = PointKey{zstamp, level, d_s, d_zz};
}

const char* mgbhip_problem::stage_name(Stage s, int level) const {
    static const char* const names[][2] = {{"f0", "f0_coarse"}, {"f1", "f1_coarse"}, {"f01", "f01_coarse"}, {"f2", "f2_coarse"},
                                           {"assemble", "assemble_coarse"}};
    return names[s][level + 1 == (int)levels.size() ? 0 : 1];
}

void mgbhip_problem::eval_f0_launch(int level, const double* d_s, const double* d_zz, const double* d_cc) {
    hipStream_t st = stream();
    StageScope sc(ctx->timers, stage_name(STAGE_F0, level));
    ElemParams E = elem_params(d_cc);
    launch_elem_at(E, MODE_F0, level, d_s, d_zz);
    launch_reduce_partials(d_partials.p, elem_grid(p, N), d_scal.p, st);
    cnt.f0++;
}

double mgbhip_problem::eval_f0(int level, const double* d_s, const double* d_zz, const double* d_cc) {
    eval_f0_launch(level, d_s, d_zz, d_cc);
    return *read_scalars(RB_VALUE, 1);
}

void mgbhip_problem::allreduce_host(double* h, int64_t count, int op) {
    MGB_REQUIRE(coll_fn != nullptr, "no collective installed");
    if (coll_fn(coll_user, h, count, op, 0) != 0) throw mgbhip::InvalidArgument("the caller's allreduce failed");
}

void mgbhip_problem::allreduce_device(double* d, int64_t count, int op) {
    MGB_REQUIRE(coll_fn != nullptr, "no collective installed");
    hipStream_t st = stream();
    if (coll_device) {
        MGB_HIP_CHECK(hipStreamSynchronize(st));
        if (coll_fn(coll_user, d, count, op, 1) != 0) throw mgbhip::InvalidArgument("the caller's allreduce failed");
        return;
    }
    coll_host.resize((size_t)count);
    MGB_HIP_CHECK(hipMemcpyAsync(coll_host.data(), d, sizeof(double) * (size_t)count, hipMemcpyDeviceToHost, st));
    MGB_HIP_CHECK(hipStreamSynchronize(st));
    allreduce_host(coll_host.data(), count, op);
    MGB_HIP_CHECK(hipMemcpyAsync(d, coll_host.data(), sizeof(double) * (size_t)count, hipMemcpyHostToDevice, st));
    MGB_HIP_CHECK(hipStreamSynchronize(st));
}

void mgbhip_problem::reduce_interface(int level, double* d_g, double* d_part) {
    Level& L = levels[level];
    if (!L.sharded) return;
    hipStream_t st = stream();
    if (d_part) MGB_HIP_CHECK(hipMemcpyAsync(d_part, d_g, sizeof(double) * (size_t)L.m, hipMemcpyDeviceToDevice, st));
    const int64_t ni = (int64_t)L.h_iface.size();
    if (ni == 0) return;
    L.iface_buf.ensure((size_t)ni);
    launch_index_gather(d_g, L.d_iface.p, ni, L.iface_buf.p, st);
    allreduce_device(L.iface_buf.p, ni, 0);
    launch_index_scatter(L.iface_buf.p, L.d_iface.p, ni, d_g, st);
}

bool mgbhip_problem::restrict_ret(int level, double* d_gout, const TrialRestrict* fuse) {
    hipStream_t st = stream();
    const Level& L = levels[level];
    StageScope sc(ctx->timers, "restrict");
    if (fuse && L.T_chunks == 0 && !L.T_long && !sharded()) {
        launch_restrict_trial(L.m, L.Tptr.p, L.Tcol.p, L.Tval.p, d_ret.p, d_gout, d_scratch.p, fuse->x, fuse->n, fuse->s,
                              fuse->xn, fuse->moved, fuse->stamp, st);
        return true;
    }
    if (L.T_chunks > 0)
        launch_csr_matvec_chunked(L.m, L.Tptr.p, L.Tcol.p, L.Tval.p, d_ret.p, d_gout, d_tchunk.p, L.T_chunks, st);
    else
        launch_csr_matvec(L.m, L.Tptr.p, L.Tcol.p, L.Tval.p, d_ret.p, d_gout, false, L.T_long, st);
    return false;
}

void mgbhip_problem::eval_f1(int level, const double* d_s, const double* d_zz, const double* d_cc, double* d_gout, double* d_part) {
    {
        StageScope sc(ctx->timers, stage_name(STAGE_F1, level));
        ElemParams E = elem_params(d_cc);
        launch_elem_at(E, MODE_F1, level, d_s, d_zz);
    }
    restrict_ret(level, d_gout);
    if (levels[level].sharded) reduce_interface(level, d_gout, d_part);
    cnt.f1++;
}

bool mgbhip_problem::eval_f01_launch(int level, const double* d_s, const double* d_zz, const double* d_cc, double* d_gout,
                                     double* d_part, bool defer_f0_sum, const TrialPoint* trial, const TrialRestrict* fuse) {
    MGB_REQUIRE(!trial || can_fuse_step(level), "a trial point is given only on a level whose element kernel forms it on the fly");
    if (dense) {
        eval_f0_launch(level, d_s, d_zz, d_cc);
        eval_f1(level, d_s, d_zz, d_cc, d_gout, d_part);
        return false;
    }
    hipStream_t st = stream();
    {
        StageScope sc(ctx->timers, stage_name(STAGE_F01, level));
        ElemParams E = elem_params(d_cc);
        launch_elem_at(E, MODE_F01, level, d_s, d_zz, trial);
        if (!defer_f0_sum) launch_reduce_partials(d_partials.p, elem_grid(p, N), d_scal.p, st);
    }
    const bool fused = restrict_ret(level, d_gout, fuse);
    if (levels[level].sharded) reduce_interface(level, d_gout, d_part);
    cnt.f0++;
    cnt.f1++;
    return fused;
}

bool mgbhip_problem::try_enable_condensed(int level) {
    Level& L = levels[level];
    static const bool off = env_on("MGBHIP_NO_CONDENSE");
    if (off || dense || !L.selection || !L.direct || nu != 2 || p != 7 || L.hRptr.empty()) return false;
    if (!L.solver.analyzed || !L.solver.has_direct_map()) return false;
    const int64_t slack0 = L.m - n;
    if (slack0 < 0 || L.rows != 2 * n) return false;
    std::vector<int32_t> ucol((size_t)n, -1);
    for (int64_t node = 0; node < n; ++node) {
        const int32_t b = L.hRptr[node], e = L.hRptr[node + 1];
        if (e - b > 1) return false;
        if (e - b == 1) ucol[(size_t)node] = L.hRcol[b];
        const int64_t rs = n + node;
        if (L.hRptr[rs + 1] - L.hRptr[rs] != 1 || (int64_t)L.hRcol[L.hRptr[rs]] != slack0 + node) return false;
    }
    const bool ok = L.solver.enable_condensed(N, p, ucol.data(), slack0, L.nnz, hel_cap + L.nshared, stream());
    if (debug_level() >= 2)
        fprintf(stderr, "[mgbhip] level %d: condensed leaves %s\n", level, ok ? "enabled" : "not applicable");
    return ok;
}

void mgbhip_problem::eval_f2(int level, const double* d_s, const double* d_zz, const double* d_cc, bool materialize,
                             const double* rhs) {
    ensure_plan(level);
    hipStream_t st = stream();
    Level& L = levels[level];
    int E_ymask = 0;
    if (L.condense && !materialize && rhs != nullptr && L.selection && L.direct && !dense) {
        StageScope sc(ctx->timers, stage_name(STAGE_F2, level));
        ElemParams E = elem_params(d_cc);
        const bool writes_zfull = bind_point(E, level, d_s, d_zz);
        E.leaf_desc = L.solver.leaf_desc();
        E.leaf_arena = L.solver.arena();
        E.leaf_g = rhs;
        E.leaf_slack0 = L.m - n;
        E.leaf_status = L.solver.leaf_status();
        E.leaf_packed = L.solver.leaves_packed() ? 1 : 0;
        if (!L.solver.leaf_flag_zero()) MGB_HIP_CHECK(hipMemsetAsync(E.leaf_status, 0, sizeof(int32_t), st));
        L.solver.leaf_flag_used();
        if (launch_elem_f2_condense(E, st)) {
            if (writes_zfull) zf = PointKey{zstamp, level, d_s, d_zz};
            L.H.written_condensed(hel_owner, level, rhs);
            cnt.f2++;
            return;
        }
    }
    L.proj_kernel = MGBHIP_PROJ_NONE;
    {
        StageScope sc(ctx->timers, stage_name(STAGE_F2, level));
        ElemParams E = elem_params(d_cc);
        E_ymask = E.ymask;
        E.diag_mask = (L.selection && !dense) ? diag_mask_sel : 0;
        hel_layout(nu, N, p, E.diag_mask, E.blk_off);
        launch_elem_at(E, MODE_F2, level, d_s, d_zz);
    }
    {
        StageScope sc(ctx->timers, stage_name(STAGE_ASSEMBLE, level));
        if (dense) {
            int klo = nD, khi = -1;
            for (int k = 0; k < nD; ++k)
                if ((E_ymask >> k) & 1) { klo = std::min(klo, k); khi = std::max(khi, k); }
            const int64_t ld = (int64_t)nD * n;
            if (khi < klo) {
                MGB_HIP_CHECK(hipMemsetAsync(L.Hval.p, 0, sizeof(double) * (size_t)L.nnz, st));
            } else {
                launch_dense_weight(nD, klo, khi, n, L.m, ld, L.denseDR.p, d_dnY.p, L.denseW.p, st);
                launch_dense_gemm_tn((int)L.m, (int)L.m, (int)((khi - klo + 1) * n), L.denseDR.p + (int64_t)klo * n, ld,
                                     nullptr, L.denseW.p + (int64_t)klo * n, ld, L.Hval.p, L.m, false, true, st);
            }
        } else if (L.selection && L.direct && !materialize) {
            launch_gather_shared(L.nshared, L.sh_q.p, L.cptr.p, L.cidx.p, d_hel.p, d_hel.p + hel_cap, st);
        } else if (L.selection) {
            launch_gather_assemble(L.nnz, L.cptr.p, L.cidx.p, d_hel.p, L.Hval.p, L.long_lists, st, L.gather_chunk, L.gather_nchunk, L.gather_part.p);
        } else {
            PanelParams PP;
            PP.p = p; PP.nu = nu; PP.N = N;
            PP.ecol_ptr = L.ecol_ptr.p; PP.panels = L.panels.p; PP.eoff = L.eoff.p;
            PP.hel = d_hel.p; PP.slab = L.slab.p; PP.cmax = L.cmax; PP.spos = nullptr;
            static const bool full_h = env_on("MGBHIP_FULL_COARSE_H");
            const bool upper = !materialize && rhs != nullptr && L.nup > 0 && !L.acc && !full_h;
            PP.upper_only = upper ? 1 : 0;
            if (L.acc) {
                L.proj_kernel = MGBHIP_PROJ_ACCUMULATE;
                launch_panel_accumulate(PP, L.ecols.p, (int32_t)L.m, L.acc_waves, L.acc_split, L.acc_chunk, L.acc_ctmax,
                                        L.acc_copies.p, L.Hval.p, st);
            } else {
                PP.spos = L.sorted_slab ? L.spos.p : nullptr;
                if (launch_panel_project_mfma(PP, st)) {
                    L.proj_kernel = MGBHIP_PROJ_MFMA;
                } else if (panel_accumulate_lds(p, nu, L.acc_ctmax) <= 40 * 1024) {
                    L.proj_kernel = MGBHIP_PROJ_STAGED;
                    launch_panel_project_staged(PP, L.acc_ctmax, st);
                } else {
                    L.proj_kernel = MGBHIP_PROJ_LOOP;
                    launch_panel_project(PP, st);
                }
                launch_gather_assemble(L.nnz, L.cptr.p, L.sorted_slab ? nullptr : L.cidx.p, L.slab.p, L.Hval.p, L.long_lists, st, L.gather_chunk,
                                       L.gather_nchunk, L.gather_part.p, upper ? L.upq.p : nullptr, upper ? L.nup : 0);
            }
        }
    }
    if (L.selection && L.direct && !materialize && !dense) L.H.written_to_slab(hel_owner, level);
    else L.H.written_to_csr(hel_owner);
    cnt.f2++;
}

void mgbhip_problem::wait_results(double seq) {
    static const bool poll = !env_on("MGBHIP_NO_POLL");
    hipStream_t st = stream();
    if (poll && seq != 0.0) {
        volatile const double* stamp = pin.d + RB_STAMP;
        const Stopwatch sw;
        for (int spins = 0;; ++spins) {
            if (__atomic_load_n(reinterpret_cast<const volatile uint64_t*>(stamp), __ATOMIC_ACQUIRE) ==
                *reinterpret_cast<const uint64_t*>(&seq))
                return;
            if ((spins & 1023) == 1023 && sw.seconds() > 1e-3)
                break;
        }
    }
    MGB_HIP_CHECK(hipStreamSynchronize(st));
}

const double* mgbhip_problem::read_scalars(int lo, int n) {
    const double seq = next_seq();
    launch_publish(d_scal.p + lo, n, pin.dev, lo, seq, stream());
    wait_results(seq);
    if (sharded()) allreduce_host(pin.d + lo, n, 0);
    return pin.d + lo;
}

TrialReadback mgbhip_problem::finish_trial(int level, const double* d_grad, bool f0_partials, bool partials_ready) {
    const double seq = next_seq();
    launch_trial_finish(d_grad, levels[level].m, d_scratch.p, f0_partials ? d_partials.p : nullptr, elem_grid(p, N), d_scal.p,
                        d_flag.p, pin.dev, stream(), own_mask(level), seq, partials_ready);
    wait_results(seq);
    TrialReadback r = decode_trial(pin.d, step_stamp);
    if (sharded()) {
        double s[RB_SHARD];
        pack_trial(r, s);
        allreduce_host(s, RB_SHARD, 0);
        r = unpack_trial(s);
    }
    return r;
}

DirReadback mgbhip_problem::finish_direction(int level, bool leaf_before, int* status) {
    MfSolver& solver = levels[level].solver;
    const double seq = next_seq();
    launch_dir_finish(d_nv.p, d_g.p, levels[level].m, d_scratch.p, d_scal.p, solver.status_flags_rw(), pin.dev, stream(),
                      own_mask(level), seq);
    solver.flags_cleared();
    wait_results(seq);
    DirReadback r = decode_direction(pin.d);
    const int32_t flags2[2] = {r.pivot ? 1 : 0, (leaf_before || r.leaf) ? 1 : 0};
    *status = MfSolver::status_from(flags2, solver.factored_condensed);
    if (sharded()) {
        double s[RB_SHARD];
        pack_direction(r, *status != MGBHIP_OK, s);
        allreduce_host(s, RB_SHARD, 0);
        *status = unpack_direction(s, r) ? MGBHIP_ERR_NOT_SPD : MGBHIP_OK;
    }
    return r;
}

bool mgbhip_problem::can_fuse_step(int level) const {
    static const bool off = env_on("MGBHIP_NO_FUSED_STEP");
    return !off && !dense && !sharded() && levels[level].R_unit;
}

void mgbhip_problem::ensure_analysis(int level) {
    Level& L = levels[level];
    if (L.solver.analyzed) return;
    hipStream_t st = stream();
    const Stopwatch sw;
    std::vector<double> cen;
    if (!hx.empty() && xdim > 0 && !L.hRptr.empty()) {
        cen.assign((size_t)L.m * xdim, 0.0);
        std::vector<double> wsum((size_t)L.m, 0.0);
        for (int64_t r = 0; r < L.rows; ++r) {
            const int64_t node = r % n;
            for (int32_t q = L.hRptr[r]; q < L.hRptr[r + 1]; ++q) {
                const double a = std::fabs(L.hRval[q]);
                const int32_t j = L.hRcol[q];
                wsum[j] += a;
                for (int d = 0; d < xdim; ++d) cen[(size_t)j * xdim + d] += a * hx[(size_t)d * n + node];
            }
        }
        for (int64_t j = 0; j < L.m; ++j)
            for (int d = 0; d < xdim; ++d) cen[(size_t)j * xdim + d] = wsum[j] > 0 ? cen[(size_t)j * xdim + d] / wsum[j] : 0.0;
    }
    const bool leaves = L.selection && L.direct && !dense && nu == 2 && p == 7;
    if (L.sharded) {
        mgbhip_problem* self = this;
        L.solver.iface_reduce = [self](double* d, int64_t cnt2) { self->allreduce_device(d, cnt2, 0); };
    }
    L.solver.analyze(L.m, L.hHptr.data(), L.hHcol.data(), st, cen.empty() ? nullptr : cen.data(), xdim, leaves,
                     L.sharded ? L.h_iface.data() : nullptr, L.sharded ? (int64_t)L.h_iface.size() : 0);
    if (debug_level() >= 2)
        fprintf(stderr, "[mgbhip] symbolic analysis level %d (m=%lld, nnz=%lld): %.2f s\n", level, (long long)L.m,
                (long long)L.nnz, sw.seconds());
}

void mgbhip_problem::prepare_all() {
    if (prepared) return;
    prepared = true;
    static const bool off = env_on("MGBHIP_LAZY_PLANS");
    if (off || dense || sharded() || levels.size() < 2) return;
    const int Ln = (int)levels.size();
    const Stopwatch prep_sw;
    std::vector<std::exception_ptr> errors((size_t)Ln);
    std::atomic<int> next{Ln - 1};
    auto worker = [&] {
        (void)hipSetDevice(ctx->device);
        for (int l = next.fetch_sub(1); l >= 0; l = next.fetch_sub(1)) {
            try {
                Level& L = levels[l];
                if (L.sharded) continue;
                ensure_plan(l);
                if (L.m < 1) continue;
// ... 97 lines not shown
```

multigridbarrier.jl_amd/csrc/problem.hpp:

```cpp
#pragma once
#include <mutex>
#include <memory>
#include <string>
#include <vector>

#include "../../include/mgbhip.h"
#include "common.hpp"
#include "hessian_state.hpp"
#include "kernels.hpp"
#include "mf_solver.hpp"

struct mgbhip_ctx {
    int device = 0;
    hipStream_t stream = nullptr;
    bool own_stream = false;
    mgbhip::StageTimers timers;
    mgbhip::DevBuf<double> vscratch, vscal;
};

struct mgbhip_vec {
    mgbhip_ctx* ctx = nullptr;
    mgbhip::DevBuf<double> buf;
    int64_t len = 0;
};

namespace mgbhip {

struct OpStore {
    std::vector<DevBuf<double>> ops;
    std::vector<bool> identity;
    DevBuf<double> w;
};

struct Level {
    int64_t rows = 0, m = 0;
    std::vector<int32_t> hRptr, hRcol;
    std::vector<double> hRval;
    DevBuf<int32_t> Rptr, Rcol, Tptr, Tcol;
    DevBuf<double> Rval, Tval;
    bool T_long = false, R_long = false;
    int32_t max_row = 0, max_col = 0;
    bool R_unit = false;
    DevBuf<int32_t> Rsel;
    int32_t T_chunks = 0;
    bool planned = false;
    bool selection = false;
    bool acc = false;
    int32_t acc_waves = 0, acc_ctmax = 0;
    int32_t acc_split = 1, acc_chunk = 0;
    DevBuf<double> acc_copies;
    std::vector<int32_t> hHptr, hHcol;
    DevBuf<int32_t> Hptr, Hcol, cptr, cidx, ecol_ptr, ecols, eoff;
    DevBuf<int32_t> spos;
    bool sorted_slab = false;
    DevBuf<double> Hval, panels, slab;
    int64_t slab_doubles = 0;
    int32_t cmax = 1;
    bool long_lists = false;
    int64_t list_total = 0;
    int32_t proj_kernel = 0;
    int32_t gather_chunk = 0, gather_nchunk = 0;
    DevBuf<double> gather_part;
    DevBuf<int32_t> upq;
    int64_t nup = 0;
    int64_t nnz = 0;
    DevBuf<double> denseDR, denseW;
    MfSolver solver;
    HessianState H;
    bool direct = false;
    int64_t nshared = 0;
    DevBuf<int32_t> sh_q;
    std::vector<int32_t> h_vmap;
    bool sharded = false;
    std::vector<int32_t> h_iface;
    DevBuf<int32_t> d_iface;
    DevBuf<double> own, iface_buf;
    bool condense_tried = false, condense = false;
};

struct TrialPoint { const double* x; const double* dir; double alpha; };

struct TrialRestrict { const double* x = nullptr; const double* n = nullptr; double s = 0.0;
                       double* xn = nullptr; int32_t* moved = nullptr; int32_t stamp = 0; };

struct Counters {
    int64_t f0 = 0, f1 = 0, f2 = 0, factor = 0, newton = 0;
    double solve_seconds = 0;
};

}

struct mgbhip_problem {
    mgbhip_ctx* ctx = nullptr;
    int32_t p = 0, nu = 0, nD = 0;
    int64_t N = 0, n = 0;
    int32_t diag_mask_sel = 0;
    bool dense = false;
    bool wide = false;
    std::shared_ptr<mgbhip::OpStore> store;
    int32_t D_state[MGBHIP_MAX_ND], D_op[MGBHIP_MAX_ND], D_stage[MGBHIP_MAX_ND];
    int32_t nstage = 0;
    const double* stage_ptr[MGBHIP_MAX_OPS];
    mgbhip::ConeDev cone;
    std::vector<mgbhip::DevBuf<double>> cone_grids;
    mgbhip::DevBuf<double> bw;
    bool has_bw = false;
    std::vector<mgbhip::Level> levels;
    std::vector<double> hx;
    int32_t xdim = 0;
    mgbhip::DevBuf<double> d_z, d_z0, d_zfull, d_c, d_ret, d_hel, d_partials, d_scal, d_scratch, d_nodeF, d_nodeDz, d_dnDz, d_dnY, d_tchunk;
    mgbhip::DevBuf<double> d_x, d_g, d_nv, d_xn, d_gn, d_tmp, d_c0;
    mgbhip::DevBuf<int32_t> d_flag;
    int32_t step_stamp = 0;
    mgbhip::PinnedBuf pin;
    mgbhip::Counters cnt;
    int64_t zstamp = 0;
    struct PointKey {
        int64_t stamp = -1; int level = -1; const double* s = nullptr; const double* z = nullptr;
        bool operator==(const PointKey& o) const { return stamp == o.stamp && level == o.level && s == o.s && z == o.z; }
    } zf;
    void touch() { ++zstamp; }
    mgbhip_allreduce_fn coll_fn = nullptr;
    void* coll_user = nullptr;
    bool coll_device = false;
    bool sharded() const { return coll_fn != nullptr; }
    std::vector<double> coll_host;
    void allreduce_host(double* h, int64_t count, int op);
    void allreduce_device(double* d, int64_t count, int op);
    void reduce_interface(int level, double* d_g, double* d_part);
    const double* own_mask(int level) const { return levels[level].sharded ? levels[level].own.p : nullptr; }
    mgbhip::DevBuf<double> d_gpart, d_gnpart;

    mgbhip::ElemParams elem_params(const double* d_cc) const;
    bool bind_point(mgbhip::ElemParams& E, int level, const double* d_s, const double* d_zz, const mgbhip::TrialPoint* trial = nullptr);
    void launch_elem_at(mgbhip::ElemParams& E, int mode, int level, const double* d_s, const double* d_zz,
                        const mgbhip::TrialPoint* trial = nullptr);
    enum Stage { STAGE_F0, STAGE_F1, STAGE_F01, STAGE_F2, STAGE_ASSEMBLE };
    const char* stage_name(Stage s, int level) const;
    bool restrict_ret(int level, double* d_gout, const mgbhip::TrialRestrict* fuse = nullptr);
    hipStream_t stream() const { return ctx->stream; }
    void ensure_plan(int level);
    void ensure_analysis(int level);
    void ensure_direct(int level);
    void prepare_all();
    double next_seq() { return ++result_seq; }
    void wait_results(double seq);
    bool can_fuse_step(int level) const;
    const double* read_scalars(int lo, int n);
    mgbhip::TrialReadback finish_trial(int level, const double* d_grad, bool f0_partials, bool partials_ready);
    mgbhip::DirReadback finish_direction(int level, bool leaf_before, int* status);
    double result_seq = 0.0;
    std::mutex shared_mutex;
    bool prepared = false;
    void ensure_plan_dense(int level);
    double eval_f0(int level, const double* d_s, const double* d_zz, const double* d_cc);
    void eval_f0_launch(int level, const double* d_s, const double* d_zz, const double* d_cc);
    void eval_f1(int level, const double* d_s, const double* d_zz, const double* d_cc, double* d_gout, double* d_part = nullptr);
    bool eval_f01_launch(int level, const double* d_s, const double* d_zz, const double* d_cc, double* d_gout, double* d_part = nullptr,
                         bool defer_f0_sum = false, const mgbhip::TrialPoint* trial = nullptr, const mgbhip::TrialRestrict* fuse = nullptr);
    void eval_f2(int level, const double* d_s, const double* d_zz, const double* d_cc, bool materialize = true,
                 const double* rhs = nullptr);
    bool try_enable_condensed(int level);
    int64_t hel_cap = 0;
    mgbhip::SlabOwner hel_owner;
    void factor(int level, const double* rhs = nullptr, double* carried_out = nullptr);
    void trisolve(int level, const double* d_g, double* d_xout);
    void trisolve_carried(int level, double* d_xout_np1);
    bool lu_fallback(int level, const double* d_g, double* d_xout);
    mgbhip::DevBuf<double> d_lu;
    mgbhip::DevBuf<int32_t> d_lustat;
    int64_t lu_fallbacks = 0;
};
```

multigridbarrier.jl_amd/csrc/readback.hpp:

```cpp
#pragma once
#include <cstdint>

namespace mgbhip {

enum : int32_t {
    RB_VALUE = 0,
    RB_AUX = 1,
    RB_SUMSQ = 2,
    RB_BAD = 3,
    RB_MOVED = 4,
    RB_GDOTV = 4,
    RB_PIVOT = 5,
    RB_LEAF = 6,
    RB_STAMP = 15,
    RB_SLOTS = 16
};
constexpr int32_t RB_TRIAL_LO = RB_VALUE, RB_TRIAL_N = RB_MOVED + 1 - RB_TRIAL_LO;
constexpr int32_t RB_DIR_LO = RB_SUMSQ, RB_DIR_N = RB_LEAF + 1 - RB_DIR_LO;
static_assert(RB_TRIAL_LO + RB_TRIAL_N <= RB_STAMP && RB_DIR_LO + RB_DIR_N <= RB_STAMP, "a read-back layout reaches the stamp");
static_assert(RB_AUX < RB_STAMP && RB_STAMP < RB_SLOTS, "the stamp is the block's last slot");

struct FinishJob { const double* src; int64_t count; int32_t out; };
struct FinishParams {
    FinishJob job[4];
    int32_t njobs;
    double* out;
    int32_t* ints;
    int32_t nints, ints_out, reset;
    double* host;
    int32_t host_lo, host_n;
    double seq;
};

inline FinishParams finish_plain(const double* partials, int64_t count, int32_t njobs, double* block, int32_t slot) {
    FinishParams F{};
    for (int32_t k = 0; k < njobs; ++k) F.job[k] = FinishJob{partials + k * count, count, slot + k};
    F.njobs = njobs;
    F.out = block;
    return F;
}

inline FinishParams finish_trial_params(const double* f0_partials, int64_t f0_count, const double* partials, int64_t count,
                                        double* block, int32_t* moved, double* host, double seq) {
    FinishParams F{};
    int32_t nj = 0;
    if (f0_partials) F.job[nj++] = FinishJob{f0_partials, f0_count, RB_VALUE};
    F.job[nj++] = FinishJob{partials, count, RB_SUMSQ};
    F.job[nj++] = FinishJob{partials + count, count, RB_BAD};
    F.njobs = nj;
    F.out = block;
    F.ints = moved; F.nints = 1; F.ints_out = RB_MOVED; F.reset = 0;
    F.host = host; F.host_lo = RB_TRIAL_LO; F.host_n = RB_TRIAL_N;
    F.seq = seq;
    return F;
}

inline FinishParams finish_direction_params(const double* partials, int64_t count, double* block, int32_t* status2, double* host,
                                            double seq) {
    FinishParams F{};
    F.job[0] = FinishJob{partials, count, RB_SUMSQ};
    F.job[1] = FinishJob{partials + count, count, RB_BAD};
    F.job[2] = FinishJob{partials + 2 * count, count, RB_GDOTV};
    F.njobs = 3;
    F.out = block;
    F.ints = status2; F.nints = 2; F.ints_out = RB_PIVOT; F.reset = 1;
    F.host = host; F.host_lo = RB_DIR_LO; F.host_n = RB_DIR_N;
    F.seq = seq;
    return F;
}
static_assert(RB_LEAF == RB_PIVOT + 1, "the two status flags are one pair of ints");

struct TrialReadback { double value, sumsq, bad; bool moved; };
struct DirReadback { double sumsq, bad, gdotv; bool pivot, leaf; };

inline TrialReadback decode_trial(const double* block, int32_t stamp) {
    return TrialReadback{block[RB_VALUE], block[RB_SUMSQ], block[RB_BAD], block[RB_MOVED] == (double)stamp};
}
inline DirReadback decode_direction(const double* block) {
    return DirReadback{block[RB_SUMSQ], block[RB_BAD], block[RB_GDOTV], block[RB_PIVOT] != 0.0, block[RB_LEAF] != 0.0};
}

constexpr int RB_SHARD = 4;
inline void pack_trial(const TrialReadback& r, double* s) {
    s[0] = r.value; s[1] = r.moved ? 1.0 : 0.0; s[2] = r.sumsq; s[3] = r.bad;
}
inline TrialReadback unpack_trial(const double* s) { return TrialReadback{s[0], s[2], s[3], s[1] != 0.0}; }
inline void pack_direction(const DirReadback& r, bool failed, double* s) {
    s[0] = r.sumsq; s[1] = r.bad; s[2] = r.gdotv; s[3] = failed ? 1.0 : 0.0;
}
inline bool unpack_direction(const double* s, DirReadback& r) {
    r.sumsq = s[0]; r.bad = s[1]; r.gdotv = s[2];
    return s[3] != 0.0;
}

}
```

multigridbarrier.jl_amd/csrc/reduce_kernels.hpp:

```cpp
#pragma once
#include <hip/hip_runtime.h>

#include "dsum.hpp"
#include "kernels.hpp"

namespace mgbhip {

namespace {


__global__ __launch_bounds__(256) void reduce_partials_kernel(const double* __restrict__ partials, int64_t count,
                                                              double* __restrict__ out) {
    __shared__ double red[256];
    const int tid = threadIdx.x;
    double s = 0.0;
    for (int64_t i = tid; i < count; i += 256) s += partials[i];
    red[tid] = s;
    __syncthreads();
    for (int off = 128; off > 0; off >>= 1) {
        if (tid < off) red[tid] += red[tid + off];
        __syncthreads();
    }
    if (tid == 0) out[0] = red[0];
}

template <int MODE>
__global__ __launch_bounds__(256) void block_reduce_kernel(const double* __restrict__ a, const double* __restrict__ b,
                                                           int64_t n, double* __restrict__ partials,
                                                           const double* __restrict__ mask) {
    __shared__ double red[256];
    __shared__ double red2[256];
    const int tid = threadIdx.x;
    double s = 0.0, bad = 0.0;
    for (int64_t i = (int64_t)blockIdx.x * 256 + tid; i < n; i += (int64_t)gridDim.x * 256) {
        const double v = a[i];
        const double w = mask ? mask[i] : 1.0;
        if (MODE == 0) s += mask ? w * (v * b[i]) : v * b[i];
        else {
            s += mask ? w * (v * v) : v * v;
            bad += isfinite(v) ? 0.0 : 1.0;
        }
    }
    red[tid] = s;
    red2[tid] = bad;
    __syncthreads();
    for (int off = 128; off > 0; off >>= 1) {
        if (tid < off) { red[tid] += red[tid + off]; red2[tid] += red2[tid + off]; }
        __syncthreads();
    }
    if (tid == 0) {
        partials[blockIdx.x] = red[0];
        if (MODE == 1) partials[gridDim.x + blockIdx.x] = red2[0];
    }
}

__global__ __launch_bounds__(256) void restrict_trial_kernel(int64_t rows, const int32_t* __restrict__ ptr, const int32_t* __restrict__ col,
                                                             const double* __restrict__ val, const double* __restrict__ ret,
                                                             double* __restrict__ g, double* __restrict__ partials,
                                                             const double* __restrict__ x, const double* __restrict__ nn, double s,
                                                             double* __restrict__ xn, int32_t* __restrict__ moved, int32_t stamp) {
    __shared__ double red[256];
    __shared__ double red2[256];
    __shared__ int any_moved;
    const int tid = threadIdx.x;
    if (tid == 0) any_moved = 0;
    __syncthreads();
    double ss = 0.0, bad = 0.0;
    bool m = false;
    for (int64_t i = (int64_t)blockIdx.x * 256 + tid; i < rows; i += (int64_t)gridDim.x * 256) {
        double acc = 0.0;
        for (int32_t q = ptr[i]; q < ptr[i + 1]; ++q) acc += val[q] * ret[col[q]];
        g[i] = acc;
        ss += acc * acc;
        bad += isfinite(acc) ? 0.0 : 1.0;
        if (xn) {
            const double xi = x[i];
            const double v = __builtin_fma(-s, nn[i], xi);
            xn[i] = v;
            m = m || (v != xi);
        }
    }
    red[tid] = ss;
    red2[tid] = bad;
    if (m) any_moved = 1;
    __syncthreads();
    for (int off = 128; off > 0; off >>= 1) {
        if (tid < off) { red[tid] += red[tid + off]; red2[tid] += red2[tid + off]; }
        __syncthreads();
    }
    if (tid == 0) {
        partials[blockIdx.x] = red[0];
        partials[gridDim.x + blockIdx.x] = red2[0];
        if (any_moved) *moved = stamp;
    }
}

__global__ __launch_bounds__(256) void dir_stats_kernel(const double* __restrict__ v, const double* __restrict__ g, int64_t n,
                                                        double* __restrict__ partials, const double* __restrict__ mask) {
    __shared__ double red[3][256];
    const int tid = threadIdx.x;
    double s = 0.0, bad = 0.0, d = 0.0;
    for (int64_t i = (int64_t)blockIdx.x * 256 + tid; i < n; i += (int64_t)gridDim.x * 256) {
        const double x = v[i];
        const double w = mask ? mask[i] : 1.0;
        s += mask ? w * (x * x) : x * x;
        bad += isfinite(x) ? 0.0 : 1.0;
        d += mask ? w * (g[i] * x) : g[i] * x;
    }
    red[0][tid] = s; red[1][tid] = bad; red[2][tid] = d;
    __syncthreads();
    for (int off = 128; off > 0; off >>= 1) {
        if (tid < off) {
            red[0][tid] += red[0][tid + off];
            red[1][tid] += red[1][tid + off];
            red[2][tid] += red[2][tid + off];
        }
        __syncthreads();
    }
    if (tid == 0) {
        partials[blockIdx.x] = red[0][0];
        partials[gridDim.x + blockIdx.x] = red[1][0];
        partials[2 * gridDim.x + blockIdx.x] = red[2][0];
    }
}

constexpr int FINISH_LOADS_IN_FLIGHT = 8;
template <int U>
__global__ __launch_bounds__(256) void finish_kernel(const FinishParams P) {
    __shared__ double red[4][256];
    __shared__ double res[RB_SLOTS];
    const int tid = threadIdx.x;
    if (tid < P.nints) {
        res[P.ints_out + tid] = (double)P.ints[tid];
        if (P.reset) P.ints[tid] = 0;
    }
    int64_t cnt[4], cmax = 0;
#pragma unroll
    for (int o = 0; o < 4; ++o) {
        cnt[o] = o < P.njobs ? P.job[o].count : 0;
        cmax = cnt[o] > cmax ? cnt[o] : cmax;
    }
    double s[4] = {0.0, 0.0, 0.0, 0.0};
    for (int64_t base = 0; base < cmax; base += 256 * U) {
        double v[4][U];
#pragma unroll
        for (int o = 0; o < 4; ++o) {
            const double* __restrict__ src = P.job[o].src;
            if (base < cnt[o]) {
#pragma unroll
                for (int u = 0; u < U; ++u) {
                    const int64_t i = base + u * 256 + tid;
                    v[o][u] = src[i < cnt[o] ? i : cnt[o] - 1];
                }
            } else {
#pragma unroll
                for (int u = 0; u < U; ++u) v[o][u] = 0.0;
            }
        }
#pragma unroll
        for (int o = 0; o < 4; ++o) {
#pragma unroll
            for (int u = 0; u < U; ++u) {
                const int64_t i = base + u * 256 + tid;
                if (i < cnt[o]) s[o] += v[o][u];
            }
        }
    }
#pragma unroll
    for (int o = 0; o < 4; ++o) red[o][tid] = s[o];
    __syncthreads();
    for (int off = 128; off > 0; off >>= 1) {
        if (tid < off) {
#pragma unroll
            for (int o = 0; o < 4; ++o) red[o][tid] += red[o][tid + off];
        }
        __syncthreads();
    }
    if (tid == 0) {
#pragma unroll
        for (int o = 0; o < 4; ++o)
            if (o < P.njobs) res[P.job[o].out] = red[o][0];
    }
    __syncthreads();
    if (tid < RB_SLOTS) {
        bool mine = false;
        for (int o = 0; o < P.njobs; ++o) mine = mine || (P.job[o].out == tid);
        if (tid >= P.ints_out && tid < P.ints_out + P.nints) mine = true;
        if (mine) P.out[tid] = res[tid];
        if (P.host && tid >= P.host_lo && tid < P.host_lo + P.host_n) P.host[tid] = mine ? res[tid] : P.out[tid];
    }
    if (P.host && P.seq != 0.0) {
        __threadfence_system();
        __syncthreads();
        if (tid == 0) {
            __hip_atomic_store(P.host + RB_STAMP, P.seq, __ATOMIC_RELEASE, __HIP_MEMORY_SCOPE_SYSTEM);
        }
    }
}

__global__ __launch_bounds__(256) void finish_serial_kernel(const FinishParams P) {
    __shared__ double red[256];
    __shared__ double res[RB_SLOTS];
    const int tid = threadIdx.x;
    if (tid < P.nints) {
        res[P.ints_out + tid] = (double)P.ints[tid];
        if (P.reset) P.ints[tid] = 0;
    }
    for (int o = 0; o < P.njobs; ++o) {
        const double* __restrict__ src = P.job[o].src;
        const int64_t cnt = P.job[o].count;
        double s = 0.0;
        for (int64_t i = tid; i < cnt; i += 256) s += src[i];
        red[tid] = s;
        __syncthreads();
        for (int off = 128; off > 0; off >>= 1) {
            if (tid < off) red[tid] += red[tid + off];
            __syncthreads();
        }
        if (tid == 0) res[P.job[o].out] = red[0];
        __syncthreads();
    }
    __syncthreads();
    if (tid < RB_SLOTS) {
        bool mine = false;
        for (int o = 0; o < P.njobs; ++o) mine = mine || (P.job[o].out == tid);
        if (tid >= P.ints_out && tid < P.ints_out + P.nints) mine = true;
        if (mine) P.out[tid] = res[tid];
        if (P.host && tid >= P.host_lo && tid < P.host_lo + P.host_n) P.host[tid] = mine ? res[tid] : P.out[tid];
    }
    if (P.host && P.seq != 0.0) {
        __threadfence_system();
        __syncthreads();
        if (tid == 0) {
            __hip_atomic_store(P.host + RB_STAMP, P.seq, __ATOMIC_RELEASE, __HIP_MEMORY_SCOPE_SYSTEM);
        }
    }
}

}

void launch_reduce_partials(const double* partials, int64_t count, double* out, hipStream_t st) {
    hipLaunchKernelGGL(reduce_partials_kernel, dim3(1), dim3(256), 0, st, partials, count, out);
    MGB_HIP_CHECK(hipGetLastError());
}

static int reduce_blocks(int64_t n);

int64_t reduce_scratch_doubles(int64_t n) { return 3 * (int64_t)reduce_blocks(n); }

static void launch_finish(const FinishParams& F, hipStream_t st) {
    static const bool serial = env_on("MGBHIP_FINISH_SERIAL");
    if (serial) hipLaunchKernelGGL(finish_serial_kernel, dim3(1), dim3(256), 0, st, F);
    else hipLaunchKernelGGL(finish_kernel<FINISH_LOADS_IN_FLIGHT>, dim3(1), dim3(256), 0, st, F);
    MGB_HIP_CHECK(hipGetLastError());
}

void launch_vec_stats(const double* v, int64_t n, double* scratch, double* block, int32_t slot, hipStream_t st, const double* mask) {
    const int nb = reduce_blocks(n);
    hipLaunchKernelGGL(block_reduce_kernel<1>, dim3(nb), dim3(256), 0, st, v, (const double*)nullptr, n, scratch, mask);
    launch_finish(finish_plain(scratch, nb, 2, block, slot), st);
}

void launch_dot(const double* a, const double* b, int64_t n, double* scratch, double* block, int32_t slot, hipStream_t st,
                const double* mask) {
    const int nb = reduce_blocks(n);
    hipLaunchKernelGGL(block_reduce_kernel<0>, dim3(nb), dim3(256), 0, st, a, b, n, scratch, mask);
    launch_finish(finish_plain(scratch, nb, 1, block, slot), st);
}

__global__ void publish_kernel(const double* __restrict__ src, int n, double* __restrict__ host, double* __restrict__ stamp, double seq) {
    const int tid = threadIdx.x;
    if (tid < n) host[tid] = src[tid];
    __threadfence_system();
    __syncthreads();
    if (tid == 0) __hip_atomic_store(stamp, seq, __ATOMIC_RELEASE, __HIP_MEMORY_SCOPE_SYSTEM);
}

void launch_publish(const double* src, int n, double* host_block, int host_lo, double seq, hipStream_t st) {
    hipLaunchKernelGGL(publish_kernel, dim3(1), dim3(64), 0, st, src, n, host_block + host_lo, host_block + RB_STAMP, seq);
    MGB_HIP_CHECK(hipGetLastError());
}

void launch_dir_finish(const double* v, const double* g, int64_t n, double* scratch, double* scal, int32_t* status2, double* host,
                       hipStream_t st, const double* mask, double seq) {
    const int nb = reduce_blocks(n);
    hipLaunchKernelGGL(dir_stats_kernel, dim3(nb), dim3(256), 0, st, v, g, n, scratch, mask);
    launch_finish(finish_direction_params(scratch, nb, scal, status2, host, seq), st);
}

void launch_trial_finish(const double* g, int64_t n, double* scratch, const double* f0_partials, int64_t f0_count, double* scal,
                         int32_t* moved, double* host, hipStream_t st, const double* mask, double seq, bool partials_ready) {
    const int nb = reduce_blocks(n);
    if (!partials_ready) hipLaunchKernelGGL(block_reduce_kernel<1>, dim3(nb), dim3(256), 0, st, g, (const double*)nullptr, n, scratch, mask);
    launch_finish(finish_trial_params(f0_partials, f0_count, scratch, nb, scal, moved, host, seq), st);
}

void launch_restrict_trial(int64_t rows, const int32_t* ptr, const int32_t* col, const double* val, const double* ret, double* g,
                            double* scratch, const double* x, const double* nn, double s, double* xn, int32_t* moved, int32_t stamp,
                            hipStream_t st) {
    if (rows == 0) return;
    const int nb = reduce_blocks(rows);
    hipLaunchKernelGGL(restrict_trial_kernel, dim3(nb), dim3(256), 0, st, rows, ptr, col, val, ret, g, scratch, x, nn, s, xn, moved, stamp);
    MGB_HIP_CHECK(hipGetLastError());
}

}
```

multigridbarrier.jl_amd/csrc/vector_kernels.hpp:

```cpp
#pragma once
#include "reduce_kernels.hpp"

namespace mgbhip {

namespace {


template <bool ADD>
__global__ __launch_bounds__(256) void csr_matvec_row_kernel(int64_t rows, const int32_t* __restrict__ ptr,
                                                             const int32_t* __restrict__ col,
                                                             const double* __restrict__ val,
                                                             const double* __restrict__ x, double* __restrict__ y) {
    const int64_t i = (int64_t)blockIdx.x * 256 + threadIdx.x;
    if (i >= rows) return;
    double s = 0.0;
    for (int32_t q = ptr[i]; q < ptr[i + 1]; ++q) s += val[q] * x[col[q]];
    y[i] = ADD ? y[i] + s : s;
}

template <bool ADD>
__global__ __launch_bounds__(256) void csr_matvec_wave_kernel(int64_t rows, const int32_t* __restrict__ ptr,
                                                              const int32_t* __restrict__ col,
                                                              const double* __restrict__ val,
                                                              const double* __restrict__ x, double* __restrict__ y) {
    const int lane = threadIdx.x & 63;
    const int64_t i = (int64_t)blockIdx.x * 4 + (threadIdx.x >> 6);
    if (i >= rows) return;
    DSum a;
    for (int32_t q = ptr[i] + lane; q < ptr[i + 1]; q += 64) a.add(val[q] * x[col[q]]);
    dsum_wave_reduce(a);
    if (lane == 0) y[i] = ADD ? y[i] + a.value() : a.value();
}

constexpr int CHUNK = 4096;
__global__ __launch_bounds__(256) void csr_matvec_chunk_kernel(const int32_t* __restrict__ ptr,
                                                               const int32_t* __restrict__ col,
                                                               const double* __restrict__ val,
                                                               const double* __restrict__ x,
                                                               double* __restrict__ partial, int nchunk) {
    __shared__ double red[256];
    const int row = blockIdx.y, ch = blockIdx.x, tid = threadIdx.x;
    const int32_t q0 = ptr[row] + ch * CHUNK;
    const int32_t q1 = min(ptr[row + 1], q0 + CHUNK);
    __shared__ double redc[256];
    DSum a;
    for (int32_t q = q0 + tid; q < q1; q += 256) a.add(val[q] * x[col[q]]);
    red[tid] = a.s;
    redc[tid] = a.c;
    __syncthreads();
    for (int off = 128; off > 0; off >>= 1) {
        if (tid < off) {
            DSum b;
            b.s = red[tid]; b.c = redc[tid];
            b.merge(red[tid + off], redc[tid + off]);
            red[tid] = b.s; redc[tid] = b.c;
        }
        __syncthreads();
    }
    if (tid == 0) {
        partial[2 * ((int64_t)row * nchunk + ch)] = red[0];
        partial[2 * ((int64_t)row * nchunk + ch) + 1] = redc[0];
    }
}

__global__ __launch_bounds__(256) void csr_matvec_chunk_sum_kernel(int64_t rows, const double* __restrict__ partial,
                                                                   int nchunk, double* __restrict__ y) {
    const int lane = threadIdx.x & 63;
    const int64_t i = (int64_t)blockIdx.x * 4 + (threadIdx.x >> 6);
    if (i >= rows) return;
    DSum a;
    for (int c = lane; c < nchunk; c += 64) a.merge(partial[2 * (i * nchunk + c)], partial[2 * (i * nchunk + c) + 1]);
    dsum_wave_reduce(a);
    if (lane == 0) y[i] = a.value();
}

__global__ __launch_bounds__(256) void prolong_kernel(int64_t rows, const int32_t* __restrict__ ptr,
                                                      const int32_t* __restrict__ col,
                                                      const double* __restrict__ val,
                                                      const double* __restrict__ s, const double* __restrict__ z0,
                                                      double* __restrict__ zfull) {
    const int64_t i = (int64_t)blockIdx.x * 256 + threadIdx.x;
    if (i >= rows) return;
    double v = z0[i];
    for (int32_t q = ptr[i]; q < ptr[i + 1]; ++q) v += val[q] * s[col[q]];
    zfull[i] = v;
}

__global__ __launch_bounds__(256) void step_kernel(const double* __restrict__ x, const double* __restrict__ nn,
                                                   double s, double* __restrict__ xn, int64_t len,
                                                   int32_t* __restrict__ moved, int32_t stamp) {
    const int64_t i = (int64_t)blockIdx.x * 256 + threadIdx.x;
    bool m = false;
    if (i < len) {
        const double xi = x[i];
        const double v = __builtin_fma(-s, nn[i], xi);
        xn[i] = v;
        m = (v != xi);
    }
    __shared__ int any_moved;
    if (threadIdx.x == 0) any_moved = 0;
    __syncthreads();
    if (m) any_moved = 1;
    __syncthreads();
    if (threadIdx.x == 0 && any_moved) *moved = stamp;
}

__global__ __launch_bounds__(256) void scale_copy_kernel(const double* __restrict__ src, double alpha,
                                                         double* __restrict__ dst, int64_t len) {
    const int64_t i = (int64_t)blockIdx.x * 256 + threadIdx.x;
    if (i < len) dst[i] = alpha * src[i];
}

__global__ __launch_bounds__(256) void border_tail_kernel(const double* __restrict__ g, double* __restrict__ tail, int64_t m,
                                                          double* __restrict__ x_one) {
    const int64_t i = (int64_t)blockIdx.x * 256 + threadIdx.x;
    if (i < m) tail[i] = -1.0 * g[i];
    else if (i == m) {
        tail[i] = -1.0;
        if (x_one) *x_one = 1.0;
    }
}

__global__ __launch_bounds__(256) void axpy_kernel(double alpha, const double* __restrict__ x,
                                                   double* __restrict__ y, int64_t len) {
    const int64_t i = (int64_t)blockIdx.x * 256 + threadIdx.x;
    if (i < len) y[i] += alpha * x[i];
}

__global__ __launch_bounds__(256) void fill_kernel(double value, double* __restrict__ y, int64_t len) {
    const int64_t i = (int64_t)blockIdx.x * 256 + threadIdx.x;
    if (i < len) y[i] = value;
}

}

__global__ __launch_bounds__(256) void index_gather_kernel(const double* __restrict__ v, const int32_t* __restrict__ idx,
                                                           int64_t cnt, double* __restrict__ out) {
    const int64_t i = (int64_t)blockIdx.x * 256 + threadIdx.x;
    if (i < cnt) out[i] = v[idx[i]];
}
__global__ __launch_bounds__(256) void index_scatter_kernel(const double* __restrict__ in, const int32_t* __restrict__ idx,
                                                            int64_t cnt, double* __restrict__ v) {
    const int64_t i = (int64_t)blockIdx.x * 256 + threadIdx.x;
    if (i < cnt) v[idx[i]] = in[i];
}
void launch_index_gather(const double* v, const int32_t* idx, int64_t cnt, double* out, hipStream_t st) {
    if (cnt == 0) return;
    hipLaunchKernelGGL(index_gather_kernel, dim3((unsigned)((cnt + 255) / 256)), dim3(256), 0, st, v, idx, cnt, out);
    MGB_HIP_CHECK(hipGetLastError());
}
void launch_index_scatter(const double* in, const int32_t* idx, int64_t cnt, double* v, hipStream_t st) {
    if (cnt == 0) return;
    hipLaunchKernelGGL(index_scatter_kernel, dim3((unsigned)((cnt + 255) / 256)), dim3(256), 0, st, in, idx, cnt, v);
    MGB_HIP_CHECK(hipGetLastError());
}

void launch_csr_matvec(int64_t rows, const int32_t* ptr, const int32_t* col, const double* val,
                       const double* x, double* y, bool add, bool long_rows, hipStream_t st) {
    if (rows == 0) return;
    if (long_rows) {
        const dim3 grid((unsigned)((rows + 3) / 4));
        if (add) hipLaunchKernelGGL(csr_matvec_wave_kernel<true>, grid, dim3(256), 0, st, rows, ptr, col, val, x, y);
        else hipLaunchKernelGGL(csr_matvec_wave_kernel<false>, grid, dim3(256), 0, st, rows, ptr, col, val, x, y);
    } else {
        const dim3 grid((unsigned)((rows + 255) / 256));
        if (add) hipLaunchKernelGGL(csr_matvec_row_kernel<true>, grid, dim3(256), 0, st, rows, ptr, col, val, x, y);
        else hipLaunchKernelGGL(csr_matvec_row_kernel<false>, grid, dim3(256), 0, st, rows, ptr, col, val, x, y);
    }
    MGB_HIP_CHECK(hipGetLastError());
}

int csr_chunks(int64_t max_row_len) { return (int)((max_row_len + CHUNK - 1) / CHUNK); }

void launch_csr_matvec_chunked(int64_t rows, const int32_t* ptr, const int32_t* col, const double* val,
                               const double* x, double* y, double* scratch, int nchunk, hipStream_t st) {
    if (rows == 0) return;
    hipLaunchKernelGGL(csr_matvec_chunk_kernel, dim3((unsigned)nchunk, (unsigned)rows), dim3(256), 0, st, ptr, col, val, x,
                       scratch, nchunk);
    hipLaunchKernelGGL(csr_matvec_chunk_sum_kernel, dim3((unsigned)((rows + 3) / 4)), dim3(256), 0, st, rows, scratch,
                       nchunk, y);
    MGB_HIP_CHECK(hipGetLastError());
}

void launch_prolong(int64_t rows, const int32_t* ptr, const int32_t* col, const double* val, const double* s,
                    const double* z0, double* zfull, hipStream_t st) {
    if (rows == 0) return;
    hipLaunchKernelGGL(prolong_kernel, dim3((unsigned)((rows + 255) / 256)), dim3(256), 0, st, rows, ptr, col, val, s,
                       z0, zfull);
    MGB_HIP_CHECK(hipGetLastError());
}

void launch_step(const double* x, const double* n, double s, double* xn, int64_t len, int32_t* moved, int32_t stamp,
                 hipStream_t st) {
    if (len == 0) return;
    hipLaunchKernelGGL(step_kernel, dim3((unsigned)((len + 255) / 256)), dim3(256), 0, st, x, n, s, xn, len, moved, stamp);
    MGB_HIP_CHECK(hipGetLastError());
}

void launch_scale_copy(const double* src, double alpha, double* dst, int64_t len, hipStream_t st) {
    if (len == 0) return;
    hipLaunchKernelGGL(scale_copy_kernel, dim3((unsigned)((len + 255) / 256)), dim3(256), 0, st, src, alpha, dst, len);
    MGB_HIP_CHECK(hipGetLastError());
}

void launch_border_tail(const double* g, double* tail, int64_t m, hipStream_t st, double* x_one) {
    hipLaunchKernelGGL(border_tail_kernel, dim3((unsigned)((m + 1 + 255) / 256)), dim3(256), 0, st, g, tail, m, x_one);
    MGB_HIP_CHECK(hipGetLastError());
}

void launch_axpy(double alpha, const double* x, double* y, int64_t len, hipStream_t st) {
    if (len == 0) return;
    hipLaunchKernelGGL(axpy_kernel, dim3((unsigned)((len + 255) / 256)), dim3(256), 0, st, alpha, x, y, len);
    MGB_HIP_CHECK(hipGetLastError());
}

void launch_fill(double value, double* y, int64_t len, hipStream_t st) {
    if (len == 0) return;
    hipLaunchKernelGGL(fill_kernel, dim3((unsigned)((len + 255) / 256)), dim3(256), 0, st, value, y, len);
    MGB_HIP_CHECK(hipGetLastError());
}

}
```

multigridbarrier.jl_amd/device.py:

```python
from __future__ import annotations

import ctypes as C
import os
import weakref
from typing import List, Optional

import numpy as np
import scipy.sparse as sp

from .blockmatrices import BlockColumn, BlockDiag
from .convex import KIND_EP, KIND_LINEAR, Convex
from .multigrid import AMG
from .problem import MGBProblem

MAX_PIECES, MAX_IDX, MAX_ND, MAX_NU, MAX_OPS = 4, 10, 13, 4, 8
MAX_LIN = 4
OK, ERR_INVALID, ERR_HIP, ERR_NOT_SPD, ERR_NONFINITE, ERR_CONVERGENCE = range(6)


class Device:
    """reference: src/device.jl:18"""


class CPUDevice(Device):
    """Marker only: the native CPU path is the reference itself (src/device.jl:25)."""


class HIPDevice(Device):
    """The MI355X backend (the reference's `CUDADevice` slot, src/device.jl:32)."""


_DEFAULT = [HIPDevice]


def default_device():
    return _DEFAULT[0]


def default_device_set(D):
    _DEFAULT[0] = D
    return D



_dp = C.POINTER(C.c_double)
_ip = C.POINTER(C.c_int32)


class _Piece(C.Structure):
    _fields_ = [("kind", C.c_int32), ("ni", C.c_int32), ("nc", C.c_int32), ("idx", C.c_int32 * MAX_IDX),
                ("A", _dp), ("b", _dp), ("p", _dp), ("mu", _dp), ("p_const", C.c_double),
                ("mu_const", C.c_double), ("select", _dp)]


class _Cone(C.Structure):
    _fields_ = [("npieces", C.c_int32), ("pieces", _Piece * MAX_PIECES), ("feasibility", C.c_int32),
                ("NC", C.c_int32)]


class _CSR(C.Structure):
    _fields_ = [("rows", C.c_int64), ("cols", C.c_int64), ("rowptr", _ip), ("colidx", _ip), ("values", _dp)]


class _Desc(C.Structure):
    _fields_ = [("p", C.c_int32), ("N", C.c_int64), ("nu", C.c_int32), ("nD", C.c_int32), ("n_ops", C.c_int32),
                ("ops", _dp * MAX_OPS), ("D_state", C.c_int32 * MAX_ND), ("D_op", C.c_int32 * MAX_ND),
                ("w", _dp), ("L", C.c_int32), ("R", C.POINTER(_CSR)), ("cone", _Cone),
                ("barrier_weights", _dp), ("x", _dp), ("dim", C.c_int32)]


class Options(C.Structure):
    _fields_ = [("tol", C.c_double), ("t", C.c_double), ("kappa", C.c_double), ("maxit", C.c_int32),
                ("max_newton", C.c_int32), ("ls_beta", C.c_double), ("ls_c1", C.c_double),
                ("line_search", C.c_int32), ("stop_lambda_tol", C.c_double), ("stop_theta", C.c_double),
                ("finalize", C.c_int32), ("finalize_theta", C.c_double), ("early_stop", C.c_int32),
                ("stopping_criterion", C.c_void_p), ("early_stop_fn", C.c_void_p), ("user", C.c_void_p)]


STOP_FN = C.CFUNCTYPE(C.c_int, C.c_double, C.c_double, C.c_double, C.c_double, C.c_double, C.c_double, C.c_void_p)
EARLY_FN = C.CFUNCTYPE(C.c_int, C.POINTER(C.c_double), C.c_double, C.c_void_p)
ALLREDUCE_FN = C.CFUNCTYPE(C.c_int, C.c_void_p, C.c_void_p, C.c_int64, C.c_int32, C.c_int32)


class _CoreResult(C.Structure):
    _fields_ = [("k", C.c_int32), ("L", C.c_int32), ("failure_code", C.c_int32), ("t_final", C.c_double),
                ("t_elapsed", C.c_double), ("solve_seconds", C.c_double), ("newton_iterations", C.c_int64),
                ("f0_evals", C.c_int64), ("f1_evals", C.c_int64), ("f2_evals", C.c_int64),
                ("factorizations", C.c_int64), ("cap_steps", C.c_int32), ("its", C.POINTER(C.c_int64)),
                ("ts", _dp), ("kappas", _dp), ("times", _dp), ("c_dot_Dz", _dp)]


EXPORTS = [
    "mgbhip_create", "mgbhip_destroy", "mgbhip_last_error", "mgbhip_version", "mgbhip_problem_create",
    "mgbhip_problem_destroy", "mgbhip_problem_set_box", "mgbhip_problem_set_barrier_weights",
    "mgbhip_level_size", "mgbhip_f0", "mgbhip_f1", "mgbhip_f2", "mgbhip_hessian_pattern", "mgbhip_solve",
    "mgbhip_set_hessian", "mgbhip_solve_newton", "mgbhip_newton_direction", "mgbhip_problem_set_sharding",
    "mgbhip_problem_set_collective",
    "mgbhip_node_barrier", "mgbhip_node_slack", "mgbhip_mgb_core", "mgbhip_matched_t",
    "mgbhip_default_options", "mgbhip_stage_ms", "mgbhip_reset_stage_timers", "mgbhip_solver_stats", "mgbhip_solver_chain",
    "mgbhip_vec_alloc", "mgbhip_vec_free", "mgbhip_vec_len", "mgbhip_vec_upload", "mgbhip_vec_download",
    "mgbhip_vec_fill", "mgbhip_vec_copy", "mgbhip_vec_axpy", "mgbhip_vec_scale", "mgbhip_vec_dot",
    "mgbhip_vec_norm", "mgbhip_vec_isfinite", "mgbhip_f0_d", "mgbhip_f1_d", "mgbhip_f2_d", "mgbhip_solve_d",
    "mgbhip_prolong_add", "mgbhip_level_plan", "mgbhip_elem_plan", "mgbhip_trial_values", "mgbhip_solver_launches", "mgbhip_interpolate", "mgbhip_interpolate_grad",
    "mgbhip_locator_create", "mgbhip_locator_elements", "mgbhip_locator_evaluate", "mgbhip_locator_destroy",
    "mgbhip_closest_create", "mgbhip_closest_fetch", "mgbhip_closest_evaluate", "mgbhip_closest_destroy",
    "mgbhip_quadrature_create", "mgbhip_quadrature_points", "mgbhip_quadrature_weights", "mgbhip_quadrature_integrate",
    "mgbhip_quadrature_max", "mgbhip_quadrature_plan", "mgbhip_quadrature_times", "mgbhip_quadrature_destroy",
    "mgbhip_residual_create", "mgbhip_residual_geometry", "mgbhip_residual_pointwise", "mgbhip_residual_integrate",
    "mgbhip_residual_plan", "mgbhip_residual_times", "mgbhip_residual_destroy",
    "mgbhip_faces_create", "mgbhip_faces_topology", "mgbhip_faces_geometry", "mgbhip_faces_sizes", "mgbhip_faces_integrate",
    "mgbhip_faces_jumps", "mgbhip_faces_indicator", "mgbhip_faces_plan", "mgbhip_faces_times", "mgbhip_faces_destroy",
    "mgbhip_contour_create", "mgbhip_contour_fetch", "mgbhip_contour_destroy", "mgbhip_contour_create_embedded",
    "mgbhip_tessellate_create", "mgbhip_tessellate_fetch", "mgbhip_tessellate_destroy",
    "mgbhip_weld_create", "mgbhip_weld_fetch", "mgbhip_weld_rounds", "mgbhip_weld_destroy",
    "mgbhip_polyline_create", "mgbhip_polyline_fetch", "mgbhip_polyline_rounds", "mgbhip_polyline_destroy",
    "mgbhip_polyline_sample",
    "mgbhip_raycast_create", "mgbhip_raycast_offsets", "mgbhip_raycast_samples", "mgbhip_raycast_lengths",
    "mgbhip_raycast_integrate", "mgbhip_raycast_render", "mgbhip_raycast_destroy", "mgbhip_raycast_render_layers",
    "mgbhip_surface_create", "mgbhip_surface_trace", "mgbhip_surface_shade", "mgbhip_surface_destroy",
    "mgbhip_stream_create", "mgbhip_stream_set_field", "mgbhip_stream_trace", "mgbhip_stream_destroy",
    "mgbhip_tubes_create", "mgbhip_tubes_trace", "mgbhip_tubes_shade", "mgbhip_tubes_destroy",
    "mgbhip_figure_create", "mgbhip_figure_render", "mgbhip_figure_render_rgba8", "mgbhip_figure_counts",
    "mgbhip_figure_destroy",
]


def library_path() -> str:
    here = os.path.dirname(os.path.abspath(__file__))
    return os.environ.get("MGBHIP_LIB") or os.path.join(here, "lib", "libmgbhip.so")


_LIB = None


def load_library():
    global _LIB
    if _LIB is not None:
        return _LIB
    path = library_path()
    if not os.path.exists(path):
        raise RuntimeError(f"{path} not found: build it with `make -C multigridbarrier.jl_amd/csrc` "
                           "(or __graft_entry__.build()); this package has no CPU fallback")
    lib = C.CDLL(path)
    lib.mgbhip_last_error.restype = C.c_char_p
    lib.mgbhip_version.restype = C.c_char_p
    lib.mgbhip_level_size.restype = C.c_int64
    lib.mgbhip_level_size.argtypes = [C.c_void_p, C.c_int32]
    lib.mgbhip_create.argtypes = [C.POINTER(C.c_void_p), C.c_int, C.c_void_p]
    lib.mgbhip_destroy.argtypes = [C.c_void_p]
    lib.mgbhip_problem_create.argtypes = [C.c_void_p, C.POINTER(_Desc), C.c_void_p, C.POINTER(C.c_void_p)]
    lib.mgbhip_problem_destroy.argtypes = [C.c_void_p]
    lib.mgbhip_problem_set_box.argtypes = [C.c_void_p, C.c_double, C.c_double]
    lib.mgbhip_problem_set_barrier_weights.argtypes = [C.c_void_p, _dp]
    for name in ("mgbhip_f0", "mgbhip_f1", "mgbhip_f2"):
        getattr(lib, name).argtypes = [C.c_void_p, C.c_int32, _dp, _dp, _dp, _dp]
    lib.mgbhip_hessian_pattern.argtypes = [C.c_void_p, C.c_int32, C.POINTER(C.c_int64), C.POINTER(_ip), C.POINTER(_ip)]
    lib.mgbhip_solve.argtypes = [C.c_void_p, C.c_int32, _dp, _dp]
    lib.mgbhip_set_hessian.argtypes = [C.c_void_p, C.c_int32, _dp]
    lib.mgbhip_solve_newton.argtypes = [C.c_void_p, C.c_int32, _dp, _dp, _dp]
    lib.mgbhip_newton_direction.argtypes = [C.c_void_p, C.c_int32, _dp, _dp, _dp, _dp, _dp, _ip]
    lib.mgbhip_problem_set_sharding.argtypes = [C.c_void_p, C.c_int32, C.c_int64, _ip, _dp]
    lib.mgbhip_problem_set_collective.argtypes = [C.c_void_p, C.c_void_p, C.c_void_p, C.c_int32]
    lib.mgbhip_node_barrier.argtypes = [C.c_void_p, _dp, _dp, _dp]
    lib.mgbhip_node_slack.argtypes = [C.c_void_p, _dp, _dp]
    lib.mgbhip_mgb_core.argtypes = [C.c_void_p, _dp, _dp, C.POINTER(Options), C.POINTER(_CoreResult)]
    lib.mgbhip_matched_t.argtypes = [C.c_void_p, _dp, _dp, C.c_double, _dp]
    lib.mgbhip_default_options.argtypes = [C.POINTER(Options), C.c_int64]
    lib.mgbhip_default_options.restype = None
    lib.mgbhip_stage_ms.argtypes = [C.c_void_p, C.c_char_p, _dp, C.POINTER(C.c_int64)]
    lib.mgbhip_reset_stage_timers.argtypes = [C.c_void_p, C.c_int]
    lib.mgbhip_solver_stats.argtypes = [C.c_void_p, C.c_int32, _dp]
    lib.mgbhip_solver_chain.argtypes = [C.c_void_p, C.c_int32, _dp]
    lib.mgbhip_level_plan.argtypes = [C.c_void_p, C.c_int32, _ip]
    lib.mgbhip_elem_plan.argtypes = [C.c_void_p, C.c_int32, _ip]
    lib.mgbhip_trial_values.argtypes = [C.c_void_p, C.c_int32, _dp, _dp, C.c_double, _dp, _dp, _dp, _dp, _dp, _ip, _ip, _ip]
    lib.mgbhip_solver_launches.argtypes = [C.c_void_p, C.c_int32, _ip, C.c_int64]
    lib.mgbhip_solver_launches.restype = C.c_int64
    vp = C.c_void_p
    lib.mgbhip_vec_alloc.argtypes = [vp, C.c_int64, C.POINTER(vp)]
    lib.mgbhip_vec_free.argtypes = [vp]
    lib.mgbhip_vec_len.argtypes = [vp]
    lib.mgbhip_vec_len.restype = C.c_int64
    lib.mgbhip_vec_upload.argtypes = [vp, _dp, C.c_int64]
    lib.mgbhip_vec_download.argtypes = [vp, _dp, C.c_int64]
    lib.mgbhip_vec_fill.argtypes = [vp, C.c_double]
    lib.mgbhip_vec_copy.argtypes = [vp, vp]
    lib.mgbhip_vec_axpy.argtypes = [C.c_double, vp, vp]
    lib.mgbhip_vec_scale.argtypes = [C.c_double, vp]
    lib.mgbhip_vec_dot.argtypes = [vp, vp, _dp]
    lib.mgbhip_vec_norm.argtypes = [vp, _dp]
    lib.mgbhip_vec_isfinite.argtypes = [vp, C.POINTER(C.c_int32)]
    lib.mgbhip_f0_d.argtypes = [vp, C.c_int32, vp, vp, vp, _dp]
    lib.mgbhip_f1_d.argtypes = [vp, C.c_int32, vp, vp, vp, vp]
    lib.mgbhip_f2_d.argtypes = [vp, C.c_int32, vp, vp, vp]
    lib.mgbhip_solve_d.argtypes = [vp, C.c_int32, vp, vp]
    lib.mgbhip_prolong_add.argtypes = [vp, C.c_int32, vp, vp]
    lib.mgbhip_interpolate.argtypes = [vp, C.c_int32, C.c_int32, C.c_int32, C.c_int32, C.c_int64, _dp, _dp, C.c_int32,
                                       _dp, C.c_int64, _dp, _dp, _ip]
    lib.mgbhip_interpolate_grad.argtypes = [vp, C.c_int32, C.c_int32, C.c_int32, C.c_int32, C.c_int64, _dp, _dp,
                                            C.c_int32, _dp, C.c_int64, _dp, _dp, _dp, _ip]
    lib.mgbhip_locator_create.argtypes = [vp, C.c_int32, C.c_int32, C.c_int32, C.c_int32, C.c_int64, _dp, _dp, C.c_int64,
                                          _dp, C.POINTER(vp)]
    lib.mgbhip_locator_elements.argtypes = [vp, _ip]
    lib.mgbhip_locator_evaluate.argtypes = [vp, C.c_int32, _dp, _dp, _dp]
    lib.mgbhip_locator_destroy.argtypes = [vp]
    lib.mgbhip_closest_create.argtypes = [vp, C.c_int32, C.c_int32, C.c_int32, C.c_int64, _dp, _dp, C.c_int64, _dp, C.c_double,
                                          C.POINTER(vp)]
    lib.mgbhip_closest_fetch.argtypes = [vp, _ip, _dp, _dp, _dp, _ip]
    lib.mgbhip_closest_evaluate.argtypes = [vp, C.c_int32, _dp, _dp, _dp]
    lib.mgbhip_closest_destroy.argtypes = [vp]
    lib.mgbhip_quadrature_create.argtypes = [vp, C.c_int32, C.c_int32, C.c_int32, C.c_int64, _dp, C.c_int32, _dp, _dp, _dp,
                                             C.POINTER(vp)]
    lib.mgbhip_quadrature_points.argtypes = [vp, _dp]
    lib.mgbhip_quadrature_weights.argtypes = [vp, _dp]
    lib.mgbhip_quadrature_integrate.argtypes = [vp, C.c_int32, C.c_double, C.c_int32, _dp, _dp, _dp, _dp, _dp]
    lib.mgbhip_quadrature_max.argtypes = [vp, C.c_int32, C.c_int32, _dp, _dp, _dp]
    lib.mgbhip_quadrature_plan.argtypes = [C.c_int32, C.c_int32, C.c_int32, C.c_int32, C.c_int64, _ip]
    lib.mgbhip_quadrature_times.argtypes = [vp, _dp]
    lib.mgbhip_quadrature_destroy.argtypes = [vp]
    lib.mgbhip_residual_create.argtypes = [vp, C.c_int32, C.c_int32, C.c_int64, _dp, C.c_int32, _dp, _dp, _dp, _dp,
                                           C.POINTER(C.c_void_p)]
    lib.mgbhip_residual_geometry.argtypes = [vp, _dp, _dp, _dp]
    lib.mgbhip_residual_pointwise.argtypes = [vp, C.c_double, C.c_int32, _dp, _dp, C.c_int32, _dp]
    lib.mgbhip_residual_integrate.argtypes = [vp, C.c_double, C.c_int32, _dp, _dp, C.c_int32, _dp, _dp]
    lib.mgbhip_residual_plan.argtypes = [C.c_int32, C.c_int32, C.c_int32, C.c_int64, _ip]
    lib.mgbhip_residual_times.argtypes = [vp, _dp]
    lib.mgbhip_residual_destroy.argtypes = [vp]
    lib.mgbhip_faces_create.argtypes = [vp, C.c_int32, C.c_int32, C.c_int64, _dp, _ip, C.c_int32, C.c_int32, _dp, _dp, _dp, _dp,
                                        _dp, _ip, C.c_int32, _ip, C.POINTER(vp), C.POINTER(C.c_int64), C.POINTER(C.c_int64)]
    lib.mgbhip_faces_topology.argtypes = [vp, _ip, _ip, _ip, _ip]
    lib.mgbhip_faces_geometry.argtypes = [vp, C.c_int32, _dp, _dp, _dp]
    lib.mgbhip_faces_sizes.argtypes = [vp, _dp]
    lib.mgbhip_faces_integrate.argtypes = [vp, C.c_int32, C.c_double, C.c_int32, _dp, _dp, _dp, _dp]
    lib.mgbhip_faces_jumps.argtypes = [vp, C.c_int32, C.c_double, C.c_int32, _dp, _dp]
    lib.mgbhip_faces_indicator.argtypes = [vp, C.c_double, C.c_int32, _dp, _dp, _dp]
    lib.mgbhip_faces_plan.argtypes = [C.c_int32, C.c_int32, C.c_int32, C.c_int32, C.c_int32, C.c_int64, _ip]
    lib.mgbhip_faces_times.argtypes = [vp, _dp]
    lib.mgbhip_faces_destroy.argtypes = [vp]
    lib.mgbhip_contour_create.argtypes = [vp, C.c_int32, C.c_int32, C.c_int32, C.c_int32, C.c_int64, _dp, _dp, C.c_int32,
                                          _dp, C.c_int32, _dp, C.c_int32, C.POINTER(vp), C.POINTER(C.c_int64)]
    lib.mgbhip_contour_create_embedded.argtypes = [vp, C.c_int32, C.c_int32, C.c_int32, C.c_int32, C.c_int32, C.c_int64, _dp,
                                                   _dp, C.c_int32, _dp, C.c_int32, _dp, C.c_int32, C.POINTER(vp),
                                                   C.POINTER(C.c_int64)]
    lib.mgbhip_tessellate_create.argtypes = [vp, C.c_int32, C.c_int32, C.c_int32, C.c_int32, C.c_int32, C.c_int64, _dp, _dp,
                                             C.c_int32, _dp, C.c_int32, C.POINTER(vp), C.POINTER(C.c_int64)]
    lib.mgbhip_tessellate_fetch.argtypes = [vp, _dp, _ip, _dp]
    lib.mgbhip_tessellate_destroy.argtypes = [vp]
    lib.mgbhip_contour_fetch.argtypes = [vp, _dp, _ip, _ip, _dp]
    lib.mgbhip_contour_destroy.argtypes = [vp]
    lib.mgbhip_weld_create.argtypes = [vp, C.c_int64, C.c_int32, C.c_int32, _dp, _ip, C.c_double, C.c_int32, C.POINTER(vp),
                                       C.POINTER(C.c_int64), C.POINTER(C.c_int64)]
    lib.mgbhip_weld_fetch.argtypes = [vp, _ip, _ip, _ip, _dp]
    lib.mgbhip_weld_rounds.argtypes = [vp, _ip, _ip]
    lib.mgbhip_weld_destroy.argtypes = [vp]
    _lp = C.POINTER(C.c_int64)
    lib.mgbhip_polyline_create.argtypes = [vp, C.c_int64, C.c_int32, _dp, C.c_int64, _ip, C.POINTER(vp), _lp, _lp, _lp]
    lib.mgbhip_polyline_fetch.argtypes = [vp, _lp, _ip, _ip, C.POINTER(C.c_uint8), _dp, _dp]
    lib.mgbhip_polyline_rounds.argtypes = [vp, _ip, _ip]
# ... 397 lines not shown
        its = np.zeros((L, cap_steps), dtype=np.int64, order="F")
        ts, kappas, times, cdz = (np.zeros(cap_steps) for _ in range(4))
        r = _CoreResult()
        r.cap_steps = cap_steps
        r.its = its.ctypes.data_as(C.POINTER(C.c_int64))
        r.ts, r.kappas, r.times, r.c_dot_Dz = _ptr(ts), _ptr(kappas), _ptr(times), _ptr(cdz)
        status = self.lib.mgbhip_mgb_core(self.handle, _ptr(z), _ptr(c), C.byref(opt), C.byref(r))
        if status not in (OK, ERR_CONVERGENCE):
            _check(self.lib, status)
        k = min(r.k, cap_steps)
        diag = dict(its=its[:, :k].copy(), ts=ts[:k].copy(), kappas=kappas[:k].copy(), times=times[:k].copy(),
                    c_dot_Dz=cdz[:k].copy(), t_elapsed=r.t_elapsed, t_final=r.t_final,
                    solve_seconds=r.solve_seconds, newton_iterations=int(r.newton_iterations),
                    f0_evals=int(r.f0_evals), f1_evals=int(r.f1_evals), f2_evals=int(r.f2_evals),
                    factorizations=int(r.factorizations), failure_code=int(r.failure_code), k=int(r.k))
        return status, z, diag

    def matched_t(self, z, c, t_default: float) -> float:
        z = _f64(z)
        c = np.asfortranarray(c, dtype=np.float64)
        out = C.c_double()
        _check(self.lib, self.lib.mgbhip_matched_t(self.handle, _ptr(z), _ptr(c), float(t_default), C.cast(C.byref(out), _dp)))
        return out.value

    def reset_stage_timers(self, enable: bool = True):
        _check(self.lib, self.lib.mgbhip_reset_stage_timers(self.handle, 1 if enable else 0))

    def stage_ms(self, stage: str):
        ms, cnt = C.c_double(), C.c_int64()
        _check(self.lib, self.lib.mgbhip_stage_ms(self.handle, stage.encode(), C.cast(C.byref(ms), _dp), C.byref(cnt)))
        return ms.value, cnt.value

    def solver_stats(self, level: int) -> dict:
        out = np.zeros(8)
        _check(self.lib, self.lib.mgbhip_solver_stats(self.handle, level, _ptr(out)))
        keys = ("fronts", "max_front", "arena_doubles", "factor_flops", "peeled", "tree_levels", "nnz", "unknowns")
        return dict(zip(keys, out.tolist()))

    def solver_chain(self, level: int) -> dict:
        out = np.zeros(8)
        _check(self.lib, self.lib.mgbhip_solver_chain(self.handle, level, _ptr(out)))
        keys = ("pivot_blocks_on_critical_path", "large_front_tree_levels", "launches_per_factorization",
                "launches_per_backward_sweep", "arena_doubles", "factor_flops", "extra_trailing_doubles", "reserved")
        return dict(zip(keys, out.tolist()))

    PLAN_KEYS = ("R_unit", "R_long", "T_long", "T_chunks", "selection", "acc", "acc_split", "long_lists", "gather_chunk",
                 "gather_nchunk", "projection", "max_row", "max_col", "cmax", "mean_list", "planned")
    PROJECTION = ("none", "loop", "staged", "mfma", "accumulate")

    def level_plan(self, level: int) -> dict:
        out = (C.c_int32 * 16)()
        _check(self.lib, self.lib.mgbhip_level_plan(self.handle, level, out))
        d = dict(zip(self.PLAN_KEYS, (int(v) for v in out)))
        d["projection"] = self.PROJECTION[d["projection"]]
        d["direct"] = bool(d["selection"] & 2)
        d["selection"] = bool(d["selection"] & 1)
        for k in ("R_unit", "R_long", "T_long", "acc", "long_lists", "planned"):
            d[k] = bool(d[k])
        return d

    ELEM_MODES = ("f0", "f1", "f2", "node_F", "node_slack", "f01")
    ELEM_KINDS = ("dense", "wide", "fast_default", "fast_runtime", "condense", "generic")

    def elem_plan(self, mode) -> dict:
        mode = self.ELEM_MODES.index(mode) if isinstance(mode, str) else int(mode)
        out = (C.c_int32 * 16)()
        _check(self.lib, self.lib.mgbhip_elem_plan(self.handle, mode, out))
        keys = ("kind", "NY", "P", "threads", "G", "EPB", "grid", "lds", "nstage", "unstaged", "ymask", "newton_kind")
        d = dict(zip(keys, (int(v) for v in out)))
        d["kind"], d["newton_kind"] = self.ELEM_KINDS[d["kind"]], self.ELEM_KINDS[d["newton_kind"]]
        return d

    def trial_values(self, level: int, x, direction, step: float, c, z0) -> dict:
        x, direction, c, z0 = _f64(x), _f64(direction), np.asfortranarray(c, dtype=np.float64), _f64(z0)
        m = self.level_sizes[level]
        g, xn = np.empty(m), np.empty(m)
        y, moved, finite, path = C.c_double(), C.c_int32(), C.c_int32(), C.c_int32()
        _check(self.lib, self.lib.mgbhip_trial_values(self.handle, level, _ptr(x), _ptr(direction), float(step), _ptr(c), _ptr(z0),
                                                      C.cast(C.byref(y), _dp), _ptr(g), _ptr(xn), C.byref(moved), C.byref(finite),
                                                      C.byref(path)))
        return dict(y=y.value, g=g, xn=xn, moved=int(moved.value), finite=int(finite.value), on_the_fly=bool(path.value & 1),
                    fused_restrict=bool(path.value & 2))

    LAUNCH_KEYS = ("level", "first", "count", "cls", "max_m", "max_k", "max_child", "tiny", "wave", "inv", "iface", "packed",
                   "assembly", "block0", "backward")
    ASSEMBLY = ("none", "gather", "columns")
    BLOCK0 = ("n/a", "gather", "diag0", "step0")
    BACKWARD = ("n/a", "k8", "k16", "general")

    @classmethod
    def launch_rows(cls, raw) -> list:
        rows = []
        for r in np.asarray(raw, dtype=np.int64).reshape(-1, 16):
            d = dict(zip(cls.LAUNCH_KEYS, (int(v) for v in r)))
            for k in ("tiny", "wave", "inv", "iface", "packed"):
                d[k] = bool(d[k])
            d["assembly"], d["block0"], d["backward"] = cls.ASSEMBLY[d["assembly"]], cls.BLOCK0[d["block0"]], cls.BACKWARD[d["backward"]]
            rows.append(d)
        return rows

    def solver_launches(self, level: int) -> list:
        n = self.lib.mgbhip_solver_launches(self.handle, level, None, 0)
        if n < 0:
            _check(self.lib, int(-n))
        out = (C.c_int32 * (16 * max(int(n), 1)))()
        n = self.lib.mgbhip_solver_launches(self.handle, level, out, n)
        if n < 0:
            _check(self.lib, int(-n))
        return self.launch_rows(np.frombuffer(out, dtype=np.int32)[:16 * int(n)])

    def close(self):
        if self.handle:
            self.lib.mgbhip_problem_destroy(self.handle)
            self.handle = None

    def __del__(self):
        try:
            self.close()
        except Exception:
            pass


def dense_as_block(M: AMG) -> AMG:
    if isinstance(M.D_fine[0], BlockColumn):
        return M
    n = M.w.size
    geom = M.geometry
    ops = {k: BlockDiag(np.asarray(v, dtype=np.float64).reshape(n, n, 1)) for k, v in geom.operators.items()}
    from dataclasses import replace
    g2 = replace(geom, operators=ops)
    nu = len(M.state_names)
    D_fine = [BlockColumn(ops[name], state, nu) for (state, name) in M.D_spec]
    return AMG(geometry=g2, x=M.x, w=M.w, R_fine=M.R_fine, D_fine=D_fine, state_names=M.state_names, D_spec=M.D_spec)


class DeviceMGBProblem:

    def __init__(self, prob: MGBProblem, device_id: int = 0, stream: Optional[int] = None, shards=None, collective=None,
                 accepts_device_ptr: bool = False):
        self.prob = prob
        self.ctx = HipContext(device_id, stream)
        self.M1 = dense_as_block(prob.M[0])
        self.main = DeviceProblem(self.ctx, self.M1, prob.Q)
        self._feas = None
        self._shards, self._collective, self._coll_dev = shards, collective, accepts_device_ptr
        if shards is not None:
            self.main.set_sharding(shards[0], collective, accepts_device_ptr)

    @property
    def feasibility(self) -> DeviceProblem:
        if self._feas is None:
            M2 = dense_as_block(self.prob.M[1])
            self._feas = DeviceProblem(self.ctx, M2, self.prob.Q, feasibility=True, NC=self.main.nD + 1,
                                       share=self.main)
            if self._shards is not None:
                self._feas.set_sharding(self._shards[1], self._collective, self._coll_dev)
        return self._feas

    def close(self):
        if self._feas is not None:
            self._feas.close()
        self.main.close()
        self.ctx.close()


def native_to_device(D, prob: MGBProblem, **kw) -> DeviceMGBProblem:
# ... 14 lines not shown
```

Baseline: 716.6.

## Speculatively queue next backtracking line-search trial gated on a device verdict

Adds a speculative line search. While the host waits for the current trial's readback, the next backtracking trial (smaller step) is already enqueued. Every kernel in that trial is gated on a device-side verdict word, so it exits early when the previous trial was accepted. This hides host round-trip latency between trials, using double-buffered pinned readback blocks. The cost is extra launches (mostly empty when gated) and more complex state save/restore. It is enabled only on levels with few trial launches.

```diff
diff --git a/include/mgbhip.h b/include/mgbhip.h
--- a/include/mgbhip.h
+++ b/include/mgbhip.h
@@ -180,6 +180,10 @@
 int mgbhip_elem_plan(mgbhip_problem* prob, int32_t mode, int32_t* out16);
 int mgbhip_trial_values(mgbhip_problem* prob, int32_t level, const double* x, const double* dir, double step, const double* c,
                         const double* z0, double* y, double* g, double* xn, int32_t* moved, int32_t* finite, int32_t* path);
+int mgbhip_linesearch(mgbhip_problem* prob, int32_t level, const double* x, const double* dir, const double* c, const double* z0,
+                      double y, double inc, double ls_c1, double ls_beta, double* out8, double* g, double* xn, double* zfull,
+                      double* blocks48);
+int mgbhip_trial_counters(mgbhip_problem* prob, int64_t* out8);
 enum { MGBHIP_LAUNCH_ROW = 16 };
 enum { MGBHIP_ASM_NONE = 0, MGBHIP_ASM_GATHER = 1, MGBHIP_ASM_COLUMNS = 2 };
 enum { MGBHIP_B0_NA = 0, MGBHIP_B0_GATHER = 1, MGBHIP_B0_DIAG0 = 2, MGBHIP_B0_STEP0 = 3 };
diff --git a/multigridbarrier.jl_amd/csrc/api.cpp b/multigridbarrier.jl_amd/csrc/api.cpp
--- a/multigridbarrier.jl_amd/csrc/api.cpp
+++ b/multigridbarrier.jl_amd/csrc/api.cpp
@@ -27,6 +27,7 @@
 int core_run(mgbhip_problem* P, double* z, const double* c, const mgbhip_options* opt, mgbhip_core_result* res);
 int matched_t_run(mgbhip_problem* P, const double* z, const double* c, double t_default, double* t_out);
 void trial_values_run(mgbhip_problem* P, int level, double step, double* y, int32_t* moved, int32_t* finite, int32_t* path);
+bool linesearch_run(mgbhip_problem* P, int level, double y, double inc, double ls_c1, double ls_beta, double* ynext, double* gnorm_next);
 
 #ifdef MGB_STEP_PROBE
 namespace mgbhip { void mf_debug_probe(long long* out64); }
@@ -466,6 +467,41 @@
     MGB_API_END
 }
 
+int mgbhip_linesearch(mgbhip_problem* P, int32_t level, const double* x, const double* dir, const double* c, const double* z0,
+                      double y, double inc, double ls_c1, double ls_beta, double* out8, double* g, double* xn, double* zfull,
+                      double* blocks48) {
+    MGB_API_BEGIN_ON(P)
+    check_level(P, level);
+    MGB_REQUIRE(x && dir && c && z0 && out8 && g && xn && zfull && blocks48, "null argument");
+    MGB_REQUIRE(!P->sharded(), "linesearch: not for sharded problems");
+    hipStream_t st = P->stream();
+    const size_t m = (size_t)P->levels[level].m;
+    stage_inputs(P, level, x, c, z0);
+    P->d_nv.upload(dir, m, st);
+    for (int i = 0; i < 8; ++i) out8[i] = 0.0;
+    out8[0] = linesearch_run(P, level, y, inc, ls_c1, ls_beta, &out8[1], &out8[2]) ? 1.0 : 0.0;
+    const mgbhip_problem::PointKey at_xn{P->zstamp, level, P->d_xn.p, P->d_z0.p};
+    out8[3] = (P->zf == at_xn) ? 1.0 : 0.0;
+    out8[4] = (double)P->last_trial_block;
+    P->d_gn.download(g, m, st);
+    P->d_xn.download(xn, m, st);
+    P->d_zfull.download(zfull, (size_t)P->nu * P->n, st);
+    P->d_scal.download(blocks48, RB_SLOTS, st);
+    MGB_HIP_CHECK(hipStreamSynchronize(st));
+    for (int b = 0; b < PinnedBuf::BLOCKS; ++b)
+        for (int i = 0; i < RB_SLOTS; ++i) blocks48[(b + 1) * RB_SLOTS + i] = P->pin.host_block(b)[i];
+    return MGBHIP_OK;
+    MGB_API_END
+}
+
+int mgbhip_trial_counters(mgbhip_problem* P, int64_t* out8) {
+    MGB_API_BEGIN_ON(P)
+    MGB_REQUIRE(P != nullptr && out8 != nullptr, "null argument");
+    out8[0] = P->cnt.spec_queued; out8[1] = P->cnt.spec_ran; out8[2] = P->cnt.spec_skipped; out8[3] = P->cnt.plain_trials;
+    out8[4] = P->cnt.f0; out8[5] = P->cnt.f1; out8[6] = P->step_stamp; out8[7] = (int64_t)P->result_seq;
+    return MGBHIP_OK;
+    MGB_API_END
+}
 
 static double* vec_scratch(mgbhip_ctx* c, int64_t len) {
     c->vscratch.ensure((size_t)reduce_scratch_doubles(len));
diff --git a/multigridbarrier.jl_amd/csrc/common.hpp b/multigridbarrier.jl_amd/csrc/common.hpp
--- a/multigridbarrier.jl_amd/csrc/common.hpp
+++ b/multigridbarrier.jl_amd/csrc/common.hpp
@@ -72,11 +72,15 @@
 struct PinnedBuf {
     double* d = nullptr;
     double* dev = nullptr;
+    static constexpr int BLOCKS = 2;
+    double* host_block(int b) const { return d + (size_t)b * RB_SLOTS; }
+    double* dev_block(int b) const { return dev + (size_t)b * RB_SLOTS; }
     PinnedBuf() {
         void* p = nullptr;
-        if (hipHostMalloc(&p, RB_SLOTS * sizeof(double), hipHostMallocDefault) != hipSuccess)
+        if (hipHostMalloc(&p, BLOCKS * RB_SLOTS * sizeof(double), hipHostMallocDefault) != hipSuccess)
             throw HipError("hipHostMalloc failed for the scalar read-back block");
         d = static_cast<double*>(p);
+        for (int i = 0; i < BLOCKS * RB_SLOTS; ++i) d[i] = 0.0;
         void* dp = nullptr;
         if (hipHostGetDevicePointer(&dp, p, 0) != hipSuccess || dp == nullptr)
             throw HipError("hipHostGetDevicePointer failed for the scalar read-back block");
diff --git a/multigridbarrier.jl_amd/csrc/driver.cpp b/multigridbarrier.jl_amd/csrc/driver.cpp
--- a/multigridbarrier.jl_amd/csrc/driver.cpp
+++ b/multigridbarrier.jl_amd/csrc/driver.cpp
@@ -64,18 +64,32 @@
     void F2(const double* d_s) { P->eval_f2(level, d_s, d_zJ, d_c, false, rhs_of_g()); }
 };
 
-bool trial_values(NewtonCtx& C, double& ynext, double& gnorm_next, int32_t* moved = nullptr, const double* step = nullptr,
-                  bool* restrict_fused_out = nullptr) {
+bool fuse_restrict_on() {
+    static const bool on = !env_on("MGBHIP_NO_FUSED_RESTRICT");
+    return on;
+}
+
+int trial_launch_count(const mgbhip_problem* P, int level) {
+    const Level& L = P->levels[level];
+    const bool onfly = P->can_fuse_step(level);
+    int n = 2;
+    if (!onfly) n += 1 + (L.R_unit ? 0 : (L.R_long ? 2 : 1));
+    if (fuse_restrict_on() && L.T_chunks == 0 && !L.T_long) n += 1;
+    else n += (L.T_chunks > 0 ? 2 : 1) + 1 + (onfly ? 1 : 0);
+    return n;
+}
+
+bool trial_launch(NewtonCtx& C, const double* step, Gate gate = {}) {
     mgbhip_problem* P = C.P;
     hipStream_t st = P->stream();
     const bool onfly = step && P->can_fuse_step(C.level);
     if (step) {
         ++P->step_stamp;
-        if (!onfly) launch_step(P->d_x.p, P->d_nv.p, *step, P->d_xn.p, C.m, P->d_flag.p, P->step_stamp, st);
+        if (!onfly) launch_step(P->d_x.p, P->d_nv.p, *step, P->d_xn.p, C.m, P->d_flag.p, P->step_stamp, st, gate);
         P->touch();
     }
     const bool fused = !P->dense;
-    static const bool fuse_restrict = !env_on("MGBHIP_NO_FUSED_RESTRICT");
+    const bool fuse_restrict = fuse_restrict_on();
     TrialRestrict fuse;
     TrialPoint point{};
     if (onfly) {
@@ -83,10 +97,18 @@
         fuse = TrialRestrict{P->d_x.p, P->d_nv.p, *step, P->d_xn.p, P->d_flag.p, P->step_stamp};
     }
     const bool restrict_fused = P->eval_f01_launch(C.level, P->d_xn.p, C.d_zJ, C.d_c, P->d_gn.p, P->sharded() ? P->d_gnpart.p : nullptr, fused,
-                                                   onfly ? &point : nullptr, (fused && fuse_restrict) ? &fuse : nullptr);
+                                                   onfly ? &point : nullptr, (fused && fuse_restrict) ? &fuse : nullptr, gate);
+    if (onfly && !restrict_fused) launch_step(P->d_x.p, P->d_nv.p, *step, P->d_xn.p, C.m, P->d_flag.p, P->step_stamp, st, gate);
+    return restrict_fused;
+}
+
+bool trial_values(NewtonCtx& C, double& ynext, double& gnorm_next, int32_t* moved = nullptr, const double* step = nullptr,
+                  bool* restrict_fused_out = nullptr) {
+    mgbhip_problem* P = C.P;
+    const bool restrict_fused = trial_launch(C, step);
     if (restrict_fused_out) *restrict_fused_out = restrict_fused;
-    if (onfly && !restrict_fused) launch_step(P->d_x.p, P->d_nv.p, *step, P->d_xn.p, C.m, P->d_flag.p, P->step_stamp, st);
-    const TrialReadback r = P->finish_trial(C.level, P->d_gn.p, fused, restrict_fused);
+    const TrialReadback r = P->finish_trial(C.level, P->d_gn.p, !P->dense, restrict_fused);
+    ++P->cnt.plain_trials;
     if (moved) *moved = r.moved ? 1 : 0;
     ynext = r.value;
     if (!std::isfinite(ynext)) return false;
@@ -95,8 +117,59 @@
     return true;
 }
 
+constexpr int SPECULATE_MAX_LAUNCHES = 4;
+bool speculates(const mgbhip_problem* P, int level) {
+    static const bool off = env_on("MGBHIP_NO_SPECULATIVE_TRIAL");
+    static const bool all_levels = env_on("MGBHIP_SPECULATE_ALL_LEVELS");
+    if (off || P->dense || P->sharded() || P->ctx->timers.enabled) return false;
+    return all_levels || trial_launch_count(P, level) <= SPECULATE_MAX_LAUNCHES;
+}
+
+bool linesearch_speculative(NewtonCtx& C, const mgbhip_options& opt, double y, double inc, double& ynext, double& gnorm_next) {
+    mgbhip_problem* P = C.P;
+    struct Queued { double s, thr, seq; int32_t stamp; int block; };
+    auto enqueue = [&](double s, int block, const int32_t* gate_word, int32_t expect) {
+        const double thr = y - opt.ls_c1 * inc * s;
+        const Gate gate{gate_word, expect};
+        const bool restrict_fused = trial_launch(C, &s, gate);
+        const TrialVerdict verdict{P->verdict_word(), P->step_stamp, thr};
+        const double seq = P->enqueue_trial_finish(C.level, P->d_gn.p, true, restrict_fused, gate, &verdict, block);
+        return Queued{s, thr, seq, P->step_stamp, block};
+    };
+    Queued cur = enqueue(1.0, 0, nullptr, 0);
+    bool have = false;
+    for (;;) {
+        const double s_next = cur.s * opt.ls_beta;
+        const bool spec = s_next > 0.0;
+        Queued nxt{};
+        mgbhip_problem::TrialState after{};
+        if (spec) {
+            const mgbhip_problem::TrialState before = P->trial_state();
+            nxt = enqueue(s_next, cur.block ^ 1, P->verdict_word(), cur.stamp);
+            after = P->trial_state();
+            P->set_trial_state(before);
+            ++P->cnt.spec_queued;
+        }
+        const TrialReadback r = P->wait_trial(cur.seq, cur.stamp, cur.block);
+        if (trial_accepts(r.value, r.sumsq, r.bad, false, 0.0)) {
+            have = true;
+            ynext = r.value;
+            gnorm_next = std::sqrt(r.sumsq);
+        }
+        if (trial_accepts(r.value, r.sumsq, r.bad, r.moved, cur.thr)) {
+            if (spec) ++P->cnt.spec_skipped;
+            return true;
+        }
+        if (!spec) return have;
+        P->set_trial_state(after);
+        ++P->cnt.spec_ran;
+        cur = nxt;
+    }
+}
+
 bool linesearch_backtracking(NewtonCtx& C, const mgbhip_options& opt, double y, double inc, double& ynext,
                              double& gnorm_next) {
+    if (speculates(C.P, C.level)) return linesearch_speculative(C, opt, y, inc, ynext, gnorm_next);
     double s = 1.0;
     bool have = false;
     while (s > 0.0) {
@@ -339,6 +412,14 @@
     *finite = trial_values(C, yn, gn, moved, &step, &restrict_fused) ? 1 : 0;
     *y = yn;
     *path = (onfly ? 1 : 0) | (restrict_fused ? 2 : 0);
+}
+
+bool linesearch_run(mgbhip_problem* P, int level, double y, double inc, double ls_c1, double ls_beta, double* ynext, double* gnorm_next) {
+    NewtonCtx C{P, level, P->d_z0.p, P->d_c.p, P->levels[level].m};
+    mgbhip_options opt{};
+    opt.ls_c1 = ls_c1;
+    opt.ls_beta = ls_beta;
+    return linesearch_backtracking(C, opt, y, inc, *ynext, *gnorm_next);
 }
 
 int core_run(mgbhip_problem* P, double* z, const double* c, const mgbhip_options* optp, mgbhip_core_result* res) {
diff --git a/multigridbarrier.jl_amd/csrc/elem_kernels.hpp b/multigridbarrier.jl_amd/csrc/elem_kernels.hpp
--- a/multigridbarrier.jl_amd/csrc/elem_kernels.hpp
+++ b/multigridbarrier.jl_amd/csrc/elem_kernels.hpp
@@ -11,6 +11,7 @@
 
 template <int NY, int MODE>
 __global__ __launch_bounds__(256) void elem_kernel(const ElemParams P, const int lgG) {
+    if (MODE == MODE_F01 && gate_shut(P.gate, P.gate_expect)) return;
     extern __shared__ double sh[];
     const int tid = threadIdx.x;
     const int G = 1 << lgG;
@@ -229,6 +230,7 @@
 
 template <int MODE>
 __global__ __launch_bounds__(256) void elem_wide_kernel(const ElemParams P, const int lgG) {
+    if (MODE == MODE_F01 && gate_shut(P.gate, P.gate_expect)) return;
     extern __shared__ double sh[];
     const int tid = threadIdx.x;
     const int NT_ = blockDim.x;
@@ -703,6 +705,7 @@
 
 template <int NY, int P, class Sig>
 __global__ __launch_bounds__(256) void elem_f01_fast(const ElemParams Pm) {
+    if (gate_shut(Pm.gate, Pm.gate_expect)) return;
     constexpr int G = elem_group(P);
     constexpr int EPB = 256 / G;
     constexpr int PP = P * P;
diff --git a/multigridbarrier.jl_amd/csrc/kernels.hpp b/multigridbarrier.jl_amd/csrc/kernels.hpp
--- a/multigridbarrier.jl_amd/csrc/kernels.hpp
+++ b/multigridbarrier.jl_amd/csrc/kernels.hpp
@@ -48,6 +48,8 @@
     const double* zx;
     double zalpha;
     int32_t wide;
+    const int32_t* gate;
+    int32_t gate_expect;
 };
 static_assert(sizeof(ElemParams) <= 4096 - 64, "ElemParams must stay well inside the kernel argument limit");
 
@@ -84,26 +86,27 @@
                 const double* mask = nullptr);
 void launch_restrict_trial(int64_t rows, const int32_t* ptr, const int32_t* col, const double* val, const double* ret, double* g,
                             double* scratch, const double* x, const double* nn, double s, double* xn, int32_t* moved, int32_t stamp,
-                            hipStream_t st);
+                            hipStream_t st, Gate gate = {});
 void launch_publish(const double* src, int n, double* host_block, int host_lo, double seq, hipStream_t st);
 void launch_dir_finish(const double* v, const double* g, int64_t n, double* scratch, double* scal, int32_t* status2, double* host,
                        hipStream_t st, const double* mask = nullptr, double seq = 0.0);
 void launch_trial_finish(const double* g, int64_t n, double* scratch, const double* f0_partials, int64_t f0_count, double* scal,
                          int32_t* moved, double* host, hipStream_t st, const double* mask = nullptr, double seq = 0.0,
-                         bool partials_ready = false);
+                         bool partials_ready = false, Gate gate = {}, const TrialVerdict* verdict = nullptr);
 void launch_index_gather(const double* v, const int32_t* idx, int64_t cnt, double* out, hipStream_t st);
 void launch_index_scatter(const double* in, const int32_t* idx, int64_t cnt, double* v, hipStream_t st);
 int64_t reduce_scratch_doubles(int64_t n);
 
 void launch_csr_matvec(int64_t rows, const int32_t* ptr, const int32_t* col, const double* val,
-                       const double* x, double* y, bool add, bool long_rows, hipStream_t st);
+                       const double* x, double* y, bool add, bool long_rows, hipStream_t st, Gate gate = {});
 int csr_chunks(int64_t max_row_len);
 void launch_csr_matvec_chunked(int64_t rows, const int32_t* ptr, const int32_t* col, const double* val,
-                               const double* x, double* y, double* scratch, int nchunk, hipStream_t st);
+                               const double* x, double* y, double* scratch, int nchunk, hipStream_t st, Gate gate = {});
 void launch_prolong(int64_t rows, const int32_t* ptr, const int32_t* col, const double* val, const double* s,
-                    const double* z0, double* zfull, hipStream_t st);
+                    const double* z0, double* zfull, hipStream_t st, Gate gate = {});
 void launch_step(const double* x, const double* n, double s, double* xn, int64_t len, int32_t* moved, int32_t stamp,
-                 hipStream_t st);
+                 hipStream_t st, Gate gate = {});
+void launch_gated_copy(const double* src, double* dst, int64_t len, hipStream_t st, Gate gate);
 void launch_scale_copy(const double* src, double alpha, double* dst, int64_t len, hipStream_t st);
 void launch_border_tail(const double* g, double* tail, int64_t m, hipStream_t st, double* x_one = nullptr);
 void launch_axpy(double alpha, const double* x, double* y, int64_t len, hipStream_t st);
diff --git a/multigridbarrier.jl_amd/csrc/problem.cpp b/multigridbarrier.jl_amd/csrc/problem.cpp
--- a/multigridbarrier.jl_amd/csrc/problem.cpp
+++ b/multigridbarrier.jl_amd/csrc/problem.cpp
@@ -471,7 +471,7 @@
     return E;
 }
 
-bool mgbhip_problem::bind_point(ElemParams& E, int level, const double* d_s, const double* d_zz, const TrialPoint* trial) {
+bool mgbhip_problem::bind_point(ElemParams& E, int level, const double* d_s, const double* d_zz, const TrialPoint* trial, Gate gate) {
     const Level& L = levels[level];
     const PointKey here{zstamp, level, d_s, d_zz};
     MGB_REQUIRE(!trial || (L.R_unit && !dense && !(zf == here)), "a trial point is given only after touch(), on a selection level");
@@ -485,18 +485,23 @@
         E.zout = d_zfull.p;
         return true;
     } else if (L.R_long) {
-        MGB_HIP_CHECK(hipMemcpyAsync(d_zfull.p, d_zz, sizeof(double) * (size_t)L.rows, hipMemcpyDeviceToDevice, stream()));
-        launch_csr_matvec(L.rows, L.Rptr.p, L.Rcol.p, L.Rval.p, d_s, d_zfull.p, true, true, stream());
+        if (gate.word) launch_gated_copy(d_zz, d_zfull.p, L.rows, stream(), gate);
+        else MGB_HIP_CHECK(hipMemcpyAsync(d_zfull.p, d_zz, sizeof(double) * (size_t)L.rows, hipMemcpyDeviceToDevice, stream()));
+        launch_csr_matvec(L.rows, L.Rptr.p, L.Rcol.p, L.Rval.p, d_s, d_zfull.p, true, true, stream(), gate);
     } else {
-        launch_prolong(L.rows, L.Rptr.p, L.Rcol.p, L.Rval.p, d_s, d_zz, d_zfull.p, stream());
+        launch_prolong(L.rows, L.Rptr.p, L.Rcol.p, L.Rval.p, d_s, d_zz, d_zfull.p, stream(), gate);
     }
     zf = here;
     E.z0 = d_zfull.p;
     return false;
 }
 
-void mgbhip_problem::launch_elem_at(ElemParams& E, int mode, int level, const double* d_s, const double* d_zz, const TrialPoint* trial) {
-    const bool writes_zfull = bind_point(E, level, d_s, d_zz, trial);
+void mgbhip_problem::launch_elem_at(ElemParams& E, int mode, int level, const double* d_s, const double* d_zz, const TrialPoint* trial,
+                                    Gate gate) {
+    MGB_REQUIRE(gate.word == nullptr || mode == MODE_F01, "only the line-search trial's element kernels read a gate");
+    const bool writes_zfull = bind_point(E, level, d_s, d_zz, trial, gate);
+    E.gate = gate.word;
+    E.gate_expect = gate.expect;
     launch_elem(E, mode, stream());
     if (writes_zfull) zf = PointKey{zstamp, level, d_s, d_zz};
 }
@@ -555,19 +560,19 @@
     launch_index_scatter(L.iface_buf.p, L.d_iface.p, ni, d_g, st);
 }
 
-bool mgbhip_problem::restrict_ret(int level, double* d_gout, const TrialRestrict* fuse) {
+bool mgbhip_problem::restrict_ret(int level, double* d_gout, const TrialRestrict* fuse, Gate gate) {
     hipStream_t st = stream();
     const Level& L = levels[level];
     StageScope sc(ctx->timers, "restrict");
     if (fuse && L.T_chunks == 0 && !L.T_long && !sharded()) {
         launch_restrict_trial(L.m, L.Tptr.p, L.Tcol.p, L.Tval.p, d_ret.p, d_gout, d_scratch.p, fuse->x, fuse->n, fuse->s,
-                              fuse->xn, fuse->moved, fuse->stamp, st);
+                              fuse->xn, fuse->moved, fuse->stamp, st, gate);
         return true;
     }
     if (L.T_chunks > 0)
-        launch_csr_matvec_chunked(L.m, L.Tptr.p, L.Tcol.p, L.Tval.p, d_ret.p, d_gout, d_tchunk.p, L.T_chunks, st);
+        launch_csr_matvec_chunked(L.m, L.Tptr.p, L.Tcol.p, L.Tval.p, d_ret.p, d_gout, d_tchunk.p, L.T_chunks, st, gate);
     else
-        launch_csr_matvec(L.m, L.Tptr.p, L.Tcol.p, L.Tval.p, d_ret.p, d_gout, false, L.T_long, st);
+        launch_csr_matvec(L.m, L.Tptr.p, L.Tcol.p, L.Tval.p, d_ret.p, d_gout, false, L.T_long, st, gate);
     return false;
 }
 
@@ -583,8 +588,9 @@
 }
 
 bool mgbhip_problem::eval_f01_launch(int level, const double* d_s, const double* d_zz, const double* d_cc, double* d_gout,
-                                     double* d_part, bool defer_f0_sum, const TrialPoint* trial, const TrialRestrict* fuse) {
+                                     double* d_part, bool defer_f0_sum, const TrialPoint* trial, const TrialRestrict* fuse, Gate gate) {
     MGB_REQUIRE(!trial || can_fuse_step(level), "a trial point is given only on a level whose element kernel forms it on the fly");
+    MGB_REQUIRE(gate.word == nullptr || (!dense && !sharded() && defer_f0_sum), "a gated trial: fused path of an unsharded problem only");
     if (dense) {
         eval_f0_launch(level, d_s, d_zz, d_cc);
         eval_f1(level, d_s, d_zz, d_cc, d_gout, d_part);
@@ -594,10 +600,10 @@
     {
         StageScope sc(ctx->timers, stage_name(STAGE_F01, level));
         ElemParams E = elem_params(d_cc);
-        launch_elem_at(E, MODE_F01, level, d_s, d_zz, trial);
+        launch_elem_at(E, MODE_F01, level, d_s, d_zz, trial, gate);
         if (!defer_f0_sum) launch_reduce_partials(d_partials.p, elem_grid(p, N), d_scal.p, st);
     }
-    const bool fused = restrict_ret(level, d_gout, fuse);
+    const bool fused = restrict_ret(level, d_gout, fuse, gate);
     if (levels[level].sharded) reduce_interface(level, d_gout, d_part);
     cnt.f0++;
     cnt.f1++;
@@ -710,11 +716,11 @@
     cnt.f2++;
 }
 
-void mgbhip_problem::wait_results(double seq) {
+void mgbhip_problem::wait_results(double seq, int block) {
     static const bool poll = !env_on("MGBHIP_NO_POLL");
     hipStream_t st = stream();
     if (poll && seq != 0.0) {
-        volatile const double* stamp = pin.d + RB_STAMP;
+        volatile const double* stamp = pin.host_block(block) + RB_STAMP;
         const Stopwatch sw;
         for (int spins = 0;; ++spins) {
             if (__atomic_load_n(reinterpret_cast<const volatile uint64_t*>(stamp), __ATOMIC_ACQUIRE) ==
@@ -735,12 +741,23 @@
     return pin.d + lo;
 }
 
-TrialReadback mgbhip_problem::finish_trial(int level, const double* d_grad, bool f0_partials, bool partials_ready) {
+double mgbhip_problem::enqueue_trial_finish(int level, const double* d_grad, bool f0_partials, bool partials_ready, Gate gate,
+                                            const TrialVerdict* verdict, int block) {
     const double seq = next_seq();
     launch_trial_finish(d_grad, levels[level].m, d_scratch.p, f0_partials ? d_partials.p : nullptr, elem_grid(p, N), d_scal.p,
-                        d_flag.p, pin.dev, stream(), own_mask(level), seq, partials_ready);
-    wait_results(seq);
-    TrialReadback r = decode_trial(pin.d, step_stamp);
+                        d_flag.p, pin.dev_block(block), stream(), own_mask(level), seq, partials_ready, gate, verdict);
+    return seq;
+}
+
+TrialReadback mgbhip_problem::wait_trial(double seq, int32_t stamp, int block) {
+    wait_results(seq, block);
+    last_trial_block = block;
+    return decode_trial(pin.host_block(block), stamp);
+}
+
+TrialReadback mgbhip_problem::finish_trial(int level, const double* d_grad, bool f0_partials, bool partials_ready) {
+    const double seq = enqueue_trial_finish(level, d_grad, f0_partials, partials_ready);
+    TrialReadback r = wait_trial(seq, step_stamp);
     if (sharded()) {
         double s[RB_SHARD];
         pack_trial(r, s);
diff --git a/multigridbarrier.jl_amd/csrc/problem.hpp b/multigridbarrier.jl_amd/csrc/problem.hpp
--- a/multigridbarrier.jl_amd/csrc/problem.hpp
+++ b/multigridbarrier.jl_amd/csrc/problem.hpp
@@ -86,6 +86,7 @@
 struct Counters {
     int64_t f0 = 0, f1 = 0, f2 = 0, factor = 0, newton = 0;
     double solve_seconds = 0;
+    int64_t spec_queued = 0, spec_ran = 0, spec_skipped = 0, plain_trials = 0;
 };
 
 }
@@ -120,6 +121,12 @@
         bool operator==(const PointKey& o) const { return stamp == o.stamp && level == o.level && s == o.s && z == o.z; }
     } zf;
     void touch() { ++zstamp; }
+    struct TrialState { int64_t zstamp; PointKey zf; int32_t step_stamp; double result_seq; int64_t f0, f1; };
+    TrialState trial_state() const { return TrialState{zstamp, zf, step_stamp, result_seq, cnt.f0, cnt.f1}; }
+    void set_trial_state(const TrialState& t) {
+        zstamp = t.zstamp; zf = t.zf; step_stamp = t.step_stamp; result_seq = t.result_seq; cnt.f0 = t.f0; cnt.f1 = t.f1;
+    }
+    int32_t* verdict_word() const { return d_flag.p + 1; }
     mgbhip_allreduce_fn coll_fn = nullptr;
     void* coll_user = nullptr;
     bool coll_device = false;
@@ -132,24 +139,29 @@
     mgbhip::DevBuf<double> d_gpart, d_gnpart;
 
     mgbhip::ElemParams elem_params(const double* d_cc) const;
-    bool bind_point(mgbhip::ElemParams& E, int level, const double* d_s, const double* d_zz, const mgbhip::TrialPoint* trial = nullptr);
+    bool bind_point(mgbhip::ElemParams& E, int level, const double* d_s, const double* d_zz, const mgbhip::TrialPoint* trial = nullptr,
+                    mgbhip::Gate gate = {});
     void launch_elem_at(mgbhip::ElemParams& E, int mode, int level, const double* d_s, const double* d_zz,
-                        const mgbhip::TrialPoint* trial = nullptr);
+                        const mgbhip::TrialPoint* trial = nullptr, mgbhip::Gate gate = {});
     enum Stage { STAGE_F0, STAGE_F1, STAGE_F01, STAGE_F2, STAGE_ASSEMBLE };
     const char* stage_name(Stage s, int level) const;
-    bool restrict_ret(int level, double* d_gout, const mgbhip::TrialRestrict* fuse = nullptr);
+    bool restrict_ret(int level, double* d_gout, const mgbhip::TrialRestrict* fuse = nullptr, mgbhip::Gate gate = {});
     hipStream_t stream() const { return ctx->stream; }
     void ensure_plan(int level);
     void ensure_analysis(int level);
     void ensure_direct(int level);
     void prepare_all();
     double next_seq() { return ++result_seq; }
-    void wait_results(double seq);
+    void wait_results(double seq, int block = 0);
     bool can_fuse_step(int level) const;
     const double* read_scalars(int lo, int n);
     mgbhip::TrialReadback finish_trial(int level, const double* d_grad, bool f0_partials, bool partials_ready);
+    double enqueue_trial_finish(int level, const double* d_grad, bool f0_partials, bool partials_ready, mgbhip::Gate gate = {},
+                                const mgbhip::TrialVerdict* verdict = nullptr, int block = 0);
+    mgbhip::TrialReadback wait_trial(double seq, int32_t stamp, int block = 0);
     mgbhip::DirReadback finish_direction(int level, bool leaf_before, int* status);
     double result_seq = 0.0;
+    int32_t last_trial_block = 0;
     std::mutex shared_mutex;
     bool prepared = false;
     void ensure_plan_dense(int level);
@@ -157,7 +169,8 @@
     void eval_f0_launch(int level, const double* d_s, const double* d_zz, const double* d_cc);
     void eval_f1(int level, const double* d_s, const double* d_zz, const double* d_cc, double* d_gout, double* d_part = nullptr);
     bool eval_f01_launch(int level, const double* d_s, const double* d_zz, const double* d_cc, double* d_gout, double* d_part = nullptr,
-                         bool defer_f0_sum = false, const mgbhip::TrialPoint* trial = nullptr, const mgbhip::TrialRestrict* fuse = nullptr);
+                         bool defer_f0_sum = false, const mgbhip::TrialPoint* trial = nullptr, const mgbhip::TrialRestrict* fuse = nullptr,
+                         mgbhip::Gate gate = {});
     void eval_f2(int level, const double* d_s, const double* d_zz, const double* d_cc, bool materialize = true,
                  const double* rhs = nullptr);
     bool try_enable_condensed(int level);
diff --git a/multigridbarrier.jl_amd/csrc/readback.hpp b/multigridbarrier.jl_amd/csrc/readback.hpp
--- a/multigridbarrier.jl_amd/csrc/readback.hpp
+++ b/multigridbarrier.jl_amd/csrc/readback.hpp
@@ -1,5 +1,11 @@
 #pragma once
 #include <cstdint>
+
+#if defined(__HIPCC__)
+#define MGB_HOST_DEVICE __host__ __device__
+#else
+#define MGB_HOST_DEVICE
+#endif
 
 namespace mgbhip {
 
@@ -30,7 +36,20 @@
     double* host;
     int32_t host_lo, host_n;
     double seq;
+    const int32_t* gate;
+    int32_t expect;
+    int32_t stamp;
+    int32_t* verdict;
+    double thr;
 };
+
+struct Gate { const int32_t* word = nullptr; int32_t expect = 0; };
+struct TrialVerdict { int32_t* word; int32_t stamp; double thr; };
+MGB_HOST_DEVICE inline bool gate_shut(const int32_t* word, int32_t expect) { return word != nullptr && *word != expect; }
+
+MGB_HOST_DEVICE inline bool trial_accepts(double value, double sumsq, double bad, bool moved, double thr) {
+    return __builtin_isfinite(value) && bad == 0.0 && __builtin_isfinite(sumsq) && (!moved || value <= thr);
+}
 
 inline FinishParams finish_plain(const double* partials, int64_t count, int32_t njobs, double* block, int32_t slot) {
     FinishParams F{};
@@ -73,8 +92,9 @@
 struct TrialReadback { double value, sumsq, bad; bool moved; };
 struct DirReadback { double sumsq, bad, gdotv; bool pivot, leaf; };
 
+MGB_HOST_DEVICE inline bool trial_moved(double moved_slot, int32_t stamp) { return moved_slot == (double)stamp; }
 inline TrialReadback decode_trial(const double* block, int32_t stamp) {
-    return TrialReadback{block[RB_VALUE], block[RB_SUMSQ], block[RB_BAD], block[RB_MOVED] == (double)stamp};
+    return TrialReadback{block[RB_VALUE], block[RB_SUMSQ], block[RB_BAD], trial_moved(block[RB_MOVED], stamp)};
 }
 inline DirReadback decode_direction(const double* block) {
     return DirReadback{block[RB_SUMSQ], block[RB_BAD], block[RB_GDOTV], block[RB_PIVOT] != 0.0, block[RB_LEAF] != 0.0};
diff --git a/multigridbarrier.jl_amd/csrc/reduce_kernels.hpp b/multigridbarrier.jl_amd/csrc/reduce_kernels.hpp
--- a/multigridbarrier.jl_amd/csrc/reduce_kernels.hpp
+++ b/multigridbarrier.jl_amd/csrc/reduce_kernels.hpp
@@ -27,7 +27,8 @@
 template <int MODE>
 __global__ __launch_bounds__(256) void block_reduce_kernel(const double* __restrict__ a, const double* __restrict__ b,
                                                            int64_t n, double* __restrict__ partials,
-                                                           const double* __restrict__ mask) {
+                                                           const double* __restrict__ mask, const int32_t* gate, int32_t expect) {
+    if (gate_shut(gate, expect)) return;
     __shared__ double red[256];
     __shared__ double red2[256];
     const int tid = threadIdx.x;
@@ -58,7 +59,9 @@
                                                              const double* __restrict__ val, const double* __restrict__ ret,
                                                              double* __restrict__ g, double* __restrict__ partials,
                                                              const double* __restrict__ x, const double* __restrict__ nn, double s,
-                                                             double* __restrict__ xn, int32_t* __restrict__ moved, int32_t stamp) {
+                                                             double* __restrict__ xn, int32_t* __restrict__ moved, int32_t stamp,
+                                                             const int32_t* gate, int32_t expect) {
+    if (gate_shut(gate, expect)) return;
     __shared__ double red[256];
     __shared__ double red2[256];
     __shared__ int any_moved;
@@ -124,9 +127,19 @@
     }
 }
 
+__device__ __forceinline__ void finish_verdict(const FinishParams& P, const double* res, int tid) {
+    if (P.verdict == nullptr || tid != 0) return;
+    bool summed = false;
+    for (int o = 0; o < P.njobs; ++o) summed = summed || (P.job[o].out == RB_VALUE);
+    const double value = summed ? res[RB_VALUE] : P.out[RB_VALUE];
+    const bool ok = trial_accepts(value, res[RB_SUMSQ], res[RB_BAD], trial_moved(res[RB_MOVED], P.stamp), P.thr);
+    *P.verdict = ok ? 0 : P.stamp;
+}
+
 constexpr int FINISH_LOADS_IN_FLIGHT = 8;
 template <int U>
 __global__ __launch_bounds__(256) void finish_kernel(const FinishParams P) {
+    if (gate_shut(P.gate, P.expect)) return;
     __shared__ double red[4][256];
     __shared__ double res[RB_SLOTS];
     const int tid = threadIdx.x;
@@ -189,6 +202,7 @@
         if (mine) P.out[tid] = res[tid];
         if (P.host && tid >= P.host_lo && tid < P.host_lo + P.host_n) P.host[tid] = mine ? res[tid] : P.out[tid];
     }
+    finish_verdict(P, res, tid);
     if (P.host && P.seq != 0.0) {
         __threadfence_system();
         __syncthreads();
@@ -199,6 +213,7 @@
 }
 
 __global__ __launch_bounds__(256) void finish_serial_kernel(const FinishParams P) {
+    if (gate_shut(P.gate, P.expect)) return;
     __shared__ double red[256];
     __shared__ double res[RB_SLOTS];
     const int tid = threadIdx.x;
@@ -228,6 +243,7 @@
         if (mine) P.out[tid] = res[tid];
         if (P.host && tid >= P.host_lo && tid < P.host_lo + P.host_n) P.host[tid] = mine ? res[tid] : P.out[tid];
     }
+    finish_verdict(P, res, tid);
     if (P.host && P.seq != 0.0) {
         __threadfence_system();
         __syncthreads();
@@ -257,14 +273,15 @@
 
 void launch_vec_stats(const double* v, int64_t n, double* scratch, double* block, int32_t slot, hipStream_t st, const double* mask) {
     const int nb = reduce_blocks(n);
-    hipLaunchKernelGGL(block_reduce_kernel<1>, dim3(nb), dim3(256), 0, st, v, (const double*)nullptr, n, scratch, mask);
+    hipLaunchKernelGGL(block_reduce_kernel<1>, dim3(nb), dim3(256), 0, st, v, (const double*)nullptr, n, scratch, mask,
+                       (const int32_t*)nullptr, 0);
     launch_finish(finish_plain(scratch, nb, 2, block, slot), st);
 }
 
 void launch_dot(const double* a, const double* b, int64_t n, double* scratch, double* block, int32_t slot, hipStream_t st,
                 const double* mask) {
     const int nb = reduce_blocks(n);
-    hipLaunchKernelGGL(block_reduce_kernel<0>, dim3(nb), dim3(256), 0, st, a, b, n, scratch, mask);
+    hipLaunchKernelGGL(block_reduce_kernel<0>, dim3(nb), dim3(256), 0, st, a, b, n, scratch, mask, (const int32_t*)nullptr, 0);
     launch_finish(finish_plain(scratch, nb, 1, block, slot), st);
 }
 
@@ -289,18 +306,25 @@
 }
 
 void launch_trial_finish(const double* g, int64_t n, double* scratch, const double* f0_partials, int64_t f0_count, double* scal,
-                         int32_t* moved, double* host, hipStream_t st, const double* mask, double seq, bool partials_ready) {
+                         int32_t* moved, double* host, hipStream_t st, const double* mask, double seq, bool partials_ready, Gate gate,
+                         const TrialVerdict* verdict) {
     const int nb = reduce_blocks(n);
-    if (!partials_ready) hipLaunchKernelGGL(block_reduce_kernel<1>, dim3(nb), dim3(256), 0, st, g, (const double*)nullptr, n, scratch, mask);
-    launch_finish(finish_trial_params(f0_partials, f0_count, scratch, nb, scal, moved, host, seq), st);
+    if (!partials_ready)
+        hipLaunchKernelGGL(block_reduce_kernel<1>, dim3(nb), dim3(256), 0, st, g, (const double*)nullptr, n, scratch, mask, gate.word,
+                           gate.expect);
+    FinishParams F = finish_trial_params(f0_partials, f0_count, scratch, nb, scal, moved, host, seq);
+    F.gate = gate.word; F.expect = gate.expect;
+    if (verdict) { F.verdict = verdict->word; F.stamp = verdict->stamp; F.thr = verdict->thr; }
+    launch_finish(F, st);
 }
 
 void launch_restrict_trial(int64_t rows, const int32_t* ptr, const int32_t* col, const double* val, const double* ret, double* g,
                             double* scratch, const double* x, const double* nn, double s, double* xn, int32_t* moved, int32_t stamp,
-                            hipStream_t st) {
+                            hipStream_t st, Gate gate) {
     if (rows == 0) return;
     const int nb = reduce_blocks(rows);
-    hipLaunchKernelGGL(restrict_trial_kernel, dim3(nb), dim3(256), 0, st, rows, ptr, col, val, ret, g, scratch, x, nn, s, xn, moved, stamp);
+    hipLaunchKernelGGL(restrict_trial_kernel, dim3(nb), dim3(256), 0, st, rows, ptr, col, val, ret, g, scratch, x, nn, s, xn, moved, stamp,
+                       gate.word, gate.expect);
     MGB_HIP_CHECK(hipGetLastError());
 }
 
diff --git a/multigridbarrier.jl_amd/csrc/vector_kernels.hpp b/multigridbarrier.jl_amd/csrc/vector_kernels.hpp
--- a/multigridbarrier.jl_amd/csrc/vector_kernels.hpp
+++ b/multigridbarrier.jl_amd/csrc/vector_kernels.hpp
@@ -10,7 +10,9 @@
 __global__ __launch_bounds__(256) void csr_matvec_row_kernel(int64_t rows, const int32_t* __restrict__ ptr,
                                                              const int32_t* __restrict__ col,
                                                              const double* __restrict__ val,
-                                                             const double* __restrict__ x, double* __restrict__ y) {
+                                                             const double* __restrict__ x, double* __restrict__ y,
+                                                             const int32_t* gate, int32_t expect) {
+    if (gate_shut(gate, expect)) return;
     const int64_t i = (int64_t)blockIdx.x * 256 + threadIdx.x;
     if (i >= rows) return;
     double s = 0.0;
@@ -22,7 +24,9 @@
 __global__ __launch_bounds__(256) void csr_matvec_wave_kernel(int64_t rows, const int32_t* __restrict__ ptr,
                                                               const int32_t* __restrict__ col,
                                                               const double* __restrict__ val,
-                                                              const double* __restrict__ x, double* __restrict__ y) {
+                                                              const double* __restrict__ x, double* __restrict__ y,
+                                                              const int32_t* gate, int32_t expect) {
+    if (gate_shut(gate, expect)) return;
     const int lane = threadIdx.x & 63;
     const int64_t i = (int64_t)blockIdx.x * 4 + (threadIdx.x >> 6);
     if (i >= rows) return;
@@ -37,7 +41,9 @@
                                                                const int32_t* __restrict__ col,
                                                                const double* __restrict__ val,
                                                                const double* __restrict__ x,
-                                                               double* __restrict__ partial, int nchunk) {
+                                                               double* __restrict__ partial, int nchunk,
+                                                               const int32_t* gate, int32_t expect) {
+    if (gate_shut(gate, expect)) return;
     __shared__ double red[256];
     const int row = blockIdx.y, ch = blockIdx.x, tid = threadIdx.x;
     const int32_t q0 = ptr[row] + ch * CHUNK;
@@ -64,7 +70,9 @@
 }
 
 __global__ __launch_bounds__(256) void csr_matvec_chunk_sum_kernel(int64_t rows, const double* __restrict__ partial,
-                                                                   int nchunk, double* __restrict__ y) {
+                                                                   int nchunk, double* __restrict__ y,
+                                                                   const int32_t* gate, int32_t expect) {
+    if (gate_shut(gate, expect)) return;
     const int lane = threadIdx.x & 63;
     const int64_t i = (int64_t)blockIdx.x * 4 + (threadIdx.x >> 6);
     if (i >= rows) return;
@@ -78,7 +86,8 @@
                                                       const int32_t* __restrict__ col,
                                                       const double* __restrict__ val,
                                                       const double* __restrict__ s, const double* __restrict__ z0,
-                                                      double* __restrict__ zfull) {
+                                                      double* __restrict__ zfull, const int32_t* gate, int32_t expect) {
+    if (gate_shut(gate, expect)) return;
     const int64_t i = (int64_t)blockIdx.x * 256 + threadIdx.x;
     if (i >= rows) return;
     double v = z0[i];
@@ -88,7 +97,8 @@
 
 __global__ __launch_bounds__(256) void step_kernel(const double* __restrict__ x, const double* __restrict__ nn,
                                                    double s, double* __restrict__ xn, int64_t len,
-                                                   int32_t* __restrict__ moved, int32_t stamp) {
+                                                   int32_t* __restrict__ moved, int32_t stamp, const int32_t* gate, int32_t expect) {
+    if (gate_shut(gate, expect)) return;
     const int64_t i = (int64_t)blockIdx.x * 256 + threadIdx.x;
     bool m = false;
     if (i < len) {
@@ -111,6 +121,13 @@
     if (i < len) dst[i] = alpha * src[i];
 }
 
+__global__ __launch_bounds__(256) void gated_copy_kernel(const double* __restrict__ src, double* __restrict__ dst, int64_t len,
+                                                         const int32_t* gate, int32_t expect) {
+    if (gate_shut(gate, expect)) return;
+    const int64_t i = (int64_t)blockIdx.x * 256 + threadIdx.x;
+    if (i < len) dst[i] = src[i];
+}
+
 __global__ __launch_bounds__(256) void border_tail_kernel(const double* __restrict__ g, double* __restrict__ tail, int64_t m,
                                                           double* __restrict__ x_one) {
     const int64_t i = (int64_t)blockIdx.x * 256 + threadIdx.x;
@@ -156,16 +173,16 @@
 }
 
 void launch_csr_matvec(int64_t rows, const int32_t* ptr, const int32_t* col, const double* val,
-                       const double* x, double* y, bool add, bool long_rows, hipStream_t st) {
+                       const double* x, double* y, bool add, bool long_rows, hipStream_t st, Gate gate) {
     if (rows == 0) return;
     if (long_rows) {
         const dim3 grid((unsigned)((rows + 3) / 4));
-        if (add) hipLaunchKernelGGL(csr_matvec_wave_kernel<true>, grid, dim3(256), 0, st, rows, ptr, col, val, x, y);
-        else hipLaunchKernelGGL(csr_matvec_wave_kernel<false>, grid, dim3(256), 0, st, rows, ptr, col, val, x, y);
+        if (add) hipLaunchKernelGGL(csr_matvec_wave_kernel<true>, grid, dim3(256), 0, st, rows, ptr, col, val, x, y, gate.word, gate.expect);
+        else hipLaunchKernelGGL(csr_matvec_wave_kernel<false>, grid, dim3(256), 0, st, rows, ptr, col, val, x, y, gate.word, gate.expect);
     } else {
         const dim3 grid((unsigned)((rows + 255) / 256));
-        if (add) hipLaunchKernelGGL(csr_matvec_row_kernel<true>, grid, dim3(256), 0, st, rows, ptr, col, val, x, y);
-        else hipLaunchKernelGGL(csr_matvec_row_kernel<false>, grid, dim3(256), 0, st, rows, ptr, col, val, x, y);
+        if (add) hipLaunchKernelGGL(csr_matvec_row_kernel<true>, grid, dim3(256), 0, st, rows, ptr, col, val, x, y, gate.word, gate.expect);
+        else hipLaunchKernelGGL(csr_matvec_row_kernel<false>, grid, dim3(256), 0, st, rows, ptr, col, val, x, y, gate.word, gate.expect);
     }
     MGB_HIP_CHECK(hipGetLastError());
 }
@@ -173,27 +190,34 @@
 int csr_chunks(int64_t max_row_len) { return (int)((max_row_len + CHUNK - 1) / CHUNK); }
 
 void launch_csr_matvec_chunked(int64_t rows, const int32_t* ptr, const int32_t* col, const double* val,
-                               const double* x, double* y, double* scratch, int nchunk, hipStream_t st) {
+                               const double* x, double* y, double* scratch, int nchunk, hipStream_t st, Gate gate) {
     if (rows == 0) return;
     hipLaunchKernelGGL(csr_matvec_chunk_kernel, dim3((unsigned)nchunk, (unsigned)rows), dim3(256), 0, st, ptr, col, val, x,
-                       scratch, nchunk);
+                       scratch, nchunk, gate.word, gate.expect);
     hipLaunchKernelGGL(csr_matvec_chunk_sum_kernel, dim3((unsigned)((rows + 3) / 4)), dim3(256), 0, st, rows, scratch,
-                       nchunk, y);
+                       nchunk, y, gate.word, gate.expect);
     MGB_HIP_CHECK(hipGetLastError());
 }
 
 void launch_prolong(int64_t rows, const int32_t* ptr, const int32_t* col, const double* val, const double* s,
-                    const double* z0, double* zfull, hipStream_t st) {
+                    const double* z0, double* zfull, hipStream_t st, Gate gate) {
     if (rows == 0) return;
     hipLaunchKernelGGL(prolong_kernel, dim3((unsigned)((rows + 255) / 256)), dim3(256), 0, st, rows, ptr, col, val, s,
-                       z0, zfull);
+                       z0, zfull, gate.word, gate.expect);
     MGB_HIP_CHECK(hipGetLastError());
 }
 
 void launch_step(const double* x, const double* n, double s, double* xn, int64_t len, int32_t* moved, int32_t stamp,
-                 hipStream_t st) {
-    if (len == 0) return;
-    hipLaunchKernelGGL(step_kernel, dim3((unsigned)((len + 255) / 256)), dim3(256), 0, st, x, n, s, xn, len, moved, stamp);
+                 hipStream_t st, Gate gate) {
+    if (len == 0) return;
+    hipLaunchKernelGGL(step_kernel, dim3((unsigned)((len + 255) / 256)), dim3(256), 0, st, x, n, s, xn, len, moved, stamp, gate.word,
+                       gate.expect);
+    MGB_HIP_CHECK(hipGetLastError());
+}
+
+void launch_gated_copy(const double* src, double* dst, int64_t len, hipStream_t st, Gate gate) {
+    if (len == 0) return;
+    hipLaunchKernelGGL(gated_copy_kernel, dim3((unsigned)((len + 255) / 256)), dim3(256), 0, st, src, dst, len, gate.word, gate.expect);
     MGB_HIP_CHECK(hipGetLastError());
 }
 
diff --git a/multigridbarrier.jl_amd/device.py b/multigridbarrier.jl_amd/device.py
--- a/multigridbarrier.jl_amd/device.py
+++ b/multigridbarrier.jl_amd/device.py
@@ -101,7 +101,7 @@
     "mgbhip_vec_alloc", "mgbhip_vec_free", "mgbhip_vec_len", "mgbhip_vec_upload", "mgbhip_vec_download",
     "mgbhip_vec_fill", "mgbhip_vec_copy", "mgbhip_vec_axpy", "mgbhip_vec_scale", "mgbhip_vec_dot",
     "mgbhip_vec_norm", "mgbhip_vec_isfinite", "mgbhip_f0_d", "mgbhip_f1_d", "mgbhip_f2_d", "mgbhip_solve_d",
-    "mgbhip_prolong_add", "mgbhip_level_plan", "mgbhip_elem_plan", "mgbhip_trial_values", "mgbhip_solver_launches", "mgbhip_interpolate", "mgbhip_interpolate_grad",
+    "mgbhip_prolong_add", "mgbhip_level_plan", "mgbhip_elem_plan", "mgbhip_trial_values", "mgbhip_linesearch", "mgbhip_trial_counters", "mgbhip_solver_launches", "mgbhip_interpolate", "mgbhip_interpolate_grad",
     "mgbhip_locator_create", "mgbhip_locator_elements", "mgbhip_locator_evaluate", "mgbhip_locator_destroy",
     "mgbhip_closest_create", "mgbhip_closest_fetch", "mgbhip_closest_evaluate", "mgbhip_closest_destroy",
     "mgbhip_quadrature_create", "mgbhip_quadrature_points", "mgbhip_quadrature_weights", "mgbhip_quadrature_integrate",
@@ -174,6 +174,10 @@
     lib.mgbhip_level_plan.argtypes = [C.c_void_p, C.c_int32, _ip]
     lib.mgbhip_elem_plan.argtypes = [C.c_void_p, C.c_int32, _ip]
     lib.mgbhip_trial_values.argtypes = [C.c_void_p, C.c_int32, _dp, _dp, C.c_double, _dp, _dp, _dp, _dp, _dp, _ip, _ip, _ip]
+    if hasattr(lib, "mgbhip_linesearch"):
+        lib.mgbhip_linesearch.argtypes = [C.c_void_p, C.c_int32, _dp, _dp, _dp, _dp, C.c_double, C.c_double, C.c_double, C.c_double, _dp,
+                                          _dp, _dp, _dp, _dp]
+        lib.mgbhip_trial_counters.argtypes = [C.c_void_p, C.POINTER(C.c_int64)]
     lib.mgbhip_solver_launches.argtypes = [C.c_void_p, C.c_int32, _ip, C.c_int64]
     lib.mgbhip_solver_launches.restype = C.c_int64
     vp = C.c_void_p
@@ -737,6 +741,22 @@
         return dict(y=y.value, g=g, xn=xn, moved=int(moved.value), finite=int(finite.value), on_the_fly=bool(path.value & 1),
                     fused_restrict=bool(path.value & 2))
 
+    def linesearch(self, level: int, x, direction, y: float, inc: float, c, z0, ls_c1: float, ls_beta: float) -> dict:
+        x, direction, c, z0 = _f64(x), _f64(direction), np.asfortranarray(c, dtype=np.float64), _f64(z0)
+        m = self.level_sizes[level]
+        g, xn, zfull, out, blocks = np.empty(m), np.empty(m), np.empty(z0.size), np.zeros(8), np.zeros(48)
+        _check(self.lib, self.lib.mgbhip_linesearch(self.handle, level, _ptr(x), _ptr(direction), _ptr(c), _ptr(z0), float(y), float(inc),
+                                                    float(ls_c1), float(ls_beta), _ptr(out), _ptr(g), _ptr(xn), _ptr(zfull), _ptr(blocks)))
+        return dict(have=bool(out[0]), y=float(out[1]), gnorm=float(out[2]), zfull_is_xn=bool(out[3]), last_block=int(out[4]),
+                    g=g, xn=xn, zfull=zfull, scal=blocks[:16].copy(), blocks=blocks[16:].reshape(2, 16).copy())
+
+    TRIAL_COUNTER_KEYS = ("spec_queued", "spec_ran", "spec_skipped", "plain_trials", "f0_evals", "f1_evals", "step_stamp", "result_seq")
+
+    def trial_counters(self) -> dict:
+        out = (C.c_int64 * 8)()
+        _check(self.lib, self.lib.mgbhip_trial_counters(self.handle, out))
+        return dict(zip(self.TRIAL_COUNTER_KEYS, (int(v) for v in out)))
+
     LAUNCH_KEYS = ("level", "first", "count", "cls", "max_m", "max_k", "max_child", "tiny", "wave", "inv", "iface", "packed",
                    "assembly", "block0", "backward")
     ASSEMBLY = ("none", "gather", "columns")
```

After: 713.0. No clear change (-0.5%).
